# hamptus/mlx-swift-qwen3-tts

Hardware: NVIDIA B200
Metric: audio-sec generated per sec (RTFx) (higher is better)
Workload: dtype u4 g64 weights dequantised at load to f16 operands x f32 accumulate, f32 residual stream

## Files before the change

### mlx-swift-qwen3-tts_b200/csrc/engine.h

```cpp
#pragma once
#include <map>
#include <memory>
#include <mutex>
#include <string>
#include <vector>

#include "frame_kernel.h"
#include "kernels.h"

namespace q3 {

class CodecDecoder;
class AudioEncoder;
class SpeakerEncoderDev;

struct EngineOptions {
  int device = 0;
  cudaStream_t stream = nullptr;
  int max_batch = 1, kv_capacity = 512, max_frames = 2400, use_cuda_graph = 1;
  int load_codec = 1, load_talker = 1, codec_max_frames = 2400, codec_max_batch = 8;
  int lanes = 1;
  int max_trailing = 1024;
  int packed_gemm = 0;
  int runtime_quantization = 0;
};

struct Admission {
  bool too_short = false;
  int prefill_len = 0;
};

struct TalkerShared {
  DeviceArena arena;
  TalkerWeights w;
  int weight_dtype = Q3TTS_BF16, eff_bits = 0, eff_group = 64;
  std::mutex mu;
};

class TalkerEngine {
 public:
  TalkerEngine(const std::string& model_dir, const TalkerConfig& cfg, const EngineOptions& opt, cudaStream_t stream,
               LaunchCounter* counter, std::shared_ptr<TalkerShared> shared = nullptr);
  ~TalkerEngine();

  Admission admit(int slot, const q3tts_request& req);
  struct AdmitItem { int slot; const q3tts_request* req; };
  void admit_batch(const std::vector<AdmitItem>& items, std::vector<Admission>& out);
  int max_prefill_rows() const { return max_rows_; }
  int step_slots(int hi) const {
    if (!handle_tc_) return hi;
    int b = hi <= 32 ? 32 : (hi <= 64 ? 64 : (hi + 127) / 128 * 128);
    return b < opt_.max_batch ? b : opt_.max_batch;
  }
  void run_frames(int n_slots, int n);
  void fetch_states(int n_slots, std::vector<SlotState>& out);
  void fetch_frames(int slot, int first, int count, int32_t* dst);
  void fetch_logits(int frames, float* code0_out, float* cp_out);
  int dump_slot() const { return dump_enabled_ ? dump_slot_ : -1; }
  void release(int slot);
  void drop_graphs();

  const TalkerConfig& config() const { return cfg_; }
  const TalkerWeights& weights() const { return w_; }
  int max_batch() const { return opt_.max_batch; }
  int kv_capacity() const { return opt_.kv_capacity; }
  int max_frames() const { return opt_.max_frames; }
  int weight_dtype() const { return shared_->weight_dtype; }
  int quant_bits() const { return shared_->eff_bits; }
  int checkpoint_quant_bits() const { return w_.checkpoint_bits; }
  int quant_group() const { return shared_->eff_group; }
  size_t device_bytes() const { return arena_.total() + (owns_weights_ ? shared_->arena.total() : 0); }
  const std::shared_ptr<TalkerShared>& shared() const { return shared_; }
  size_t weight_bytes_per_frame() const { return w_.talker_step_bytes + 15 * w_.cp_pass_bytes; }
  int64_t graph_replays = 0, graph_nodes_replayed = 0, mega_launches = 0;
  bool megakernel_enabled() const { return mega_.ok; }
  double last_prefill_ms = 0;

  double profile_linears(int which, int m, int iters, int64_t& launches, int64_t& bytes_per_iter);
  int sample_probe(const float* logits, int vocab, float temperature, int top_k, float top_p, float rep_penalty,
                   const int32_t* token_set, int n_set, uint64_t seed, uint64_t counter);

 private:
  void forward_stack(const StackWeights& S, float* x, int m, const int* row_slot, const int* row_pos, const int* win_start,
                     const float* inv_freq, void* kbase, void* vbase, int kv_f16, size_t slot_stride, size_t layer_stride, int capacity,
                     bool one_row_per_slot, bool decode_step, bool x16_ready);
  void issue_frame(int n_slots);
  void build_tc_weights();
  void build_mega_plan();
  TcLinear make_tc(const Linear& L, bool interleave_halves, const float* fold = nullptr);
  bool use_tc(int) const { return handle_tc_; }
  bool use_tc_step(int) const { return handle_tc_; }
  bool use_mega(int n_slots) const { return mega_.ok && !handle_tc_ && opt_.max_batch <= mega_.max_slots && n_slots <= mega_.max_slots; }
  void linear_tc(const TcLinear& L, const void* x16, int m, float* out32, int ld32, void* out16, int ld16, const float* res, int act, int swiglu, bool row_count_invariant = false);
  LaunchCtx ctx() { return LaunchCtx{stream_, counter_}; }

  TalkerConfig cfg_;
  EngineOptions opt_;
  cudaStream_t stream_;
  LaunchCounter* counter_;
  DeviceArena arena_;
  std::shared_ptr<TalkerShared> shared_;
  bool owns_weights_ = false;
  TalkerWeights& w_;

  int max_rows_ = 0, max_tp_rows_ = 0, set_words_ = 0;
  int tc_min_rows_ = 3;
  bool step_tc_ = false;
  bool handle_tc_ = false;
  bool packed_gemm_ = false;
  void attach_packed(struct TcGemm& g, const TcLinear& L) const;
  float* d_rs_ = nullptr;
  static constexpr float kX16Div = 16.0f;
  void *d_h16_ = nullptr, *d_attn16_ = nullptr, *d_act16_ = nullptr, *d_tpe16_ = nullptr, *d_tph16_ = nullptr;
  void *kcache_ = nullptr, *vcache_ = nullptr;
  int kv_f16_ = 0;
  float *cp_k_ = nullptr, *cp_v_ = nullptr;
  size_t kv_slot_stride_ = 0, kv_layer_stride_ = 0, cpkv_slot_stride_ = 0, cpkv_layer_stride_ = 0;
  static constexpr int kCpCapacity = 32;
  SlotState* d_state_ = nullptr;
  int *d_step_slot_ = nullptr, *d_step_pos_ = nullptr, *d_win_ = nullptr;
  int *d_cp_slot2_ = nullptr, *d_cp_pos2_ = nullptr, *d_iota_ = nullptr, *d_cp_pos_ = nullptr;
  int *d_pf_slot_ = nullptr, *d_pf_pos_ = nullptr, *d_pf_win_ = nullptr;
  float *d_x_ = nullptr, *d_qkv_ = nullptr, *d_attn_ = nullptr, *d_act_ = nullptr;
  float *d_hlast_ = nullptr, *d_logits0_ = nullptr, *d_cplogits_ = nullptr, *d_cpin_ = nullptr, *d_cpx_ = nullptr, *d_xstep_ = nullptr;
  int *d_cur_codes_ = nullptr, *d_frames_ = nullptr, *d_forced_ = nullptr;
  unsigned* d_sets_ = nullptr;
  float *d_trailing_ = nullptr, *d_tts_ = nullptr;
  float *d_tpe_ = nullptr, *d_tph_ = nullptr, *d_tp_ = nullptr, *d_spk_ = nullptr;
  int *d_ids_ = nullptr, *d_desc_ = nullptr;
  Embedding* d_cp_emb_ = nullptr;
  float *d_inv_freq_ = nullptr, *d_cp_inv_freq_ = nullptr;
  float *d_dump0_ = nullptr, *d_dumpcp_ = nullptr;
  int dump_cap_ = 0, dump_slot_ = 0;
  bool dump_enabled_ = false;
  float* d_probe_logits_ = nullptr;
  unsigned* d_probe_set_ = nullptr;
  int* d_probe_out_ = nullptr;
  int* h_stage_ = nullptr;
  size_t h_stage_ints_ = 0;
  SlotState* h_state_ = nullptr;
  cudaEvent_t ev_a_ = nullptr, ev_b_ = nullptr;

  struct Graph {
    cudaGraphExec_t exec = nullptr;
    int64_t nodes = 0;
  };
  std::map<long long, Graph> graphs_;
  MegaPlan mega_;
};

struct Handle {
  std::mutex mu;
  std::string model_dir;
  std::string last_error;
  bool poisoned = false;
  EngineOptions opt;
  cudaStream_t stream = nullptr;
  bool own_stream = false;
  LaunchCounter counter;
  TalkerConfig cfg;
  bool has_talker = false;
  std::unique_ptr<TalkerEngine> talker;
  std::unique_ptr<CodecDecoder> codec;
  std::unique_ptr<AudioEncoder> audio_encoder;
  std::unique_ptr<SpeakerEncoderDev> speaker_encoder;
  q3tts_timing timing{};
  cudaEvent_t ev_start = nullptr, ev_stop = nullptr;
  float* h_pcm = nullptr;
  size_t h_pcm_floats = 0;
  int32_t* h_codes = nullptr;
  size_t h_codes_ints = 0;
  int32_t* d_codes = nullptr;
  size_t d_codes_ints = 0;
  float* d_pcm = nullptr;
  size_t d_pcm_floats = 0;
  void* open_stream = nullptr;
  std::mutex lanes_mu;
  std::vector<Handle*> lanes;
  ~Handle();
};

}
```

### mlx-swift-qwen3-tts_b200/csrc/gemm_skinny.cu

```cuda
#include <cuda.h>

#include <algorithm>

#include "skinny_common.cuh"

namespace q3 {

namespace {

using namespace skinny;

template <int ACT, bool SWIGLU>
__global__ void __launch_bounds__(kThreads, 1)
tc_skinny_kernel(const __grid_constant__ CUtensorMap tmW, const __grid_constant__ CUtensorMap tmX, const SkParams p) {
  extern __shared__ uint8_t smem_raw[];
  uint8_t* smem = reinterpret_cast<uint8_t*>((reinterpret_cast<uintptr_t>(smem_raw) + 1023) & ~(uintptr_t)1023);
  const int x_bytes = p.m_pad * kBlockK * 2;
  uint8_t* sW = smem;
  uint8_t* sX = smem + (size_t)p.stages * kWBytes;
  float* red = reinterpret_cast<float*>(sX + (size_t)p.stages * x_bytes);
  uint64_t* full = reinterpret_cast<uint64_t*>(red + (size_t)kRowsW * p.m_pad);
  uint64_t* empty = full + p.stages;
  uint64_t* tmem_full = empty + p.stages;
  uint64_t* red_full = tmem_full + 1;
  uint64_t* ack = red_full + 1;
  uint32_t* tmem_slot = reinterpret_cast<uint32_t*>(ack + 1);
  float* rowscale_s = reinterpret_cast<float*>(tmem_slot + 2);

  const int warp = threadIdx.x >> 5, lane = threadIdx.x & 31;
  const uint32_t rank = p.split > 1 ? cluster_ctarank() : 0u;
  const int n0 = blockIdx.x * kRowsW;
  const int kb0 = (int)((rank * (uint32_t)p.num_kb) >> p.split_shift);
  const int kb1 = (int)(((rank + 1u) * (uint32_t)p.num_kb) >> p.split_shift);
  const int nkb = kb1 - kb0;

  pdl_launch_dependents();
  if (threadIdx.x == 32) {
    asm volatile("prefetch.tensormap [%0];" ::"l"(&tmW) : "memory");
    asm volatile("prefetch.tensormap [%0];" ::"l"(&tmX) : "memory");
  }
  if (threadIdx.x == 0) {
    if (p.trace) p.trace[((size_t)blockIdx.y * gridDim.x + blockIdx.x) * 16 + 0] = sk_globaltimer();
    SK_STAMP(1);
    for (int s = 0; s < p.stages; ++s) { mbar_init(&full[s], 1); mbar_init(&empty[s], 1); }
    mbar_init(tmem_full, 1);
    mbar_init(red_full, 1);
    mbar_init(ack, p.split > 1 ? p.split - 1 : 1);
    asm volatile("fence.mbarrier_init.release.cluster;" ::: "memory");
    asm volatile("fence.proxy.async.shared::cta;" ::: "memory");
  }
  if (warp == 1) {
    asm volatile("tcgen05.alloc.cta_group::1.sync.aligned.shared::cta.b32 [%0], %1;" ::"r"(smem_u32(tmem_slot)), "r"(p.tmem_cols) : "memory");
    asm volatile("tcgen05.relinquish_alloc_permit.cta_group::1.sync.aligned;" ::: "memory");
  }
  tc_fence_before();
  __syncthreads();
  tc_fence_after();
  const uint32_t tmem_base = *tmem_slot;
  if (threadIdx.x == 0) SK_STAMP(2);
  if (p.split > 1) cluster_arrive_release();

  if (warp == 0) {
    {
      const bool lead = elect_one();
      const int pre = nkb < p.stages ? nkb : p.stages;
      if (lead) {
        for (int i = 0; i < pre; ++i) {
          mbar_expect_tx(&full[i], (uint32_t)(kWBytes + x_bytes));
          tma_load_2d(sW + (size_t)i * kWBytes, &tmW, &full[i], (kb0 + i) * kBlockK, n0);
        }
        for (int i = pre; i < nkb; ++i) tma_prefetch_2d(&tmW, (kb0 + i) * kBlockK, n0);
      }
      pdl_wait();
      int s = 0;
      uint32_t ph = 0;
      for (int i = 0; i < nkb; ++i) {
        if (i >= pre) mbar_wait(&empty[s], ph ^ 1u);
        if (lead) {
          if (i >= pre) {
            mbar_expect_tx(&full[s], (uint32_t)(kWBytes + x_bytes));
            tma_load_2d(sW + (size_t)s * kWBytes, &tmW, &full[s], (kb0 + i) * kBlockK, n0);
          }
          tma_load_2d(sX + (size_t)s * x_bytes, &tmX, &full[s], (kb0 + i) * kBlockK, 0);
        }
        if (++s == p.stages) { s = 0; ph ^= 1u; }
      }
    }
    __syncwarp();
  } else if (warp == 1) {
    {
      const bool lead = elect_one();
      const uint32_t idesc = (1u << 4) | ((uint32_t)(p.m_pad >> 3) << 17) | ((uint32_t)(kRowsW >> 4) << 24);
      int s = 0;
      uint32_t ph = 0;
      for (int i = 0; i < nkb; ++i) {
        mbar_wait(&full[s], ph);
        tc_fence_after();
        if (lead && i == 0) SK_STAMP(3);
        const uint64_t ad = umma_desc(smem_u32(sW + (size_t)s * kWBytes));
        const uint64_t bd = umma_desc(smem_u32(sX + (size_t)s * x_bytes));
        if (lead) {
#pragma unroll
          for (int k = 0; k < kBlockK / 16; ++k)
            umma_f16(tmem_base, ad + (uint64_t)(2 * k), bd + (uint64_t)(2 * k), idesc, (i | k) != 0 ? 1u : 0u);
          umma_commit(&empty[s]);
        }
        if (++s == p.stages) { s = 0; ph ^= 1u; }
      }
      if (lead) umma_commit(tmem_full);
    }
    __syncwarp();
  } else {
    pdl_wait();
    if (p.rms_x) sk_row_factors(p, rowscale_s, rank);
    if (p.split > 1) cluster_wait_acquire();
    mbar_wait(tmem_full, 0);
    tc_fence_after();
    if (threadIdx.x == 64) SK_STAMP(4);
    sk_reduce_epilogue<ACT, SWIGLU>(p, reinterpret_cast<float*>(smem), red, red_full, ack, rowscale_s, tmem_base, rank, n0);
  }
  if (p.split > 1 && warp < 2) cluster_wait_acquire();
  tc_fence_before();
  __syncthreads();
  if (threadIdx.x == 0 && p.trace) {
    SK_STAMP(8);
    p.trace[((size_t)blockIdx.y * gridDim.x + blockIdx.x) * 16 + 9] = sk_globaltimer();
  }
  if (warp == 1) {
    tc_fence_after();
    asm volatile("tcgen05.dealloc.cta_group::1.sync.aligned.b32 %0, %1;" ::"r"(tmem_base), "r"(p.tmem_cols) : "memory");
  }
}

constexpr int kSmemKB = 108;

struct SkPlan {
  int m_pad, split, stages, num_kb, tiles;
  size_t smem;
};

SkPlan plan(const TcGemm& g) {
  SkPlan s{};
  const int M = g.Bt * g.T;
  s.m_pad = M <= 32 ? 32 : (M <= 64 ? 64 : 128);
  s.tiles = (g.N + kRowsW - 1) / kRowsW;
  s.num_kb = (g.cin + kBlockK - 1) / kBlockK;
  s.split = k_split(s.tiles, s.num_kb, s.m_pad);
  const int stage_bytes = kWBytes + s.m_pad * kBlockK * 2;
  const int red_bytes = kRowsW * s.m_pad * 4;
  const int nkb_max = (s.num_kb + s.split - 1) / s.split;
  s.stages = std::max(2, (kSmemKB * 1024 - red_bytes) / stage_bytes);
  s.stages = std::max(1, std::min(s.stages, nkb_max));
  while (s.stages * stage_bytes < red_bytes) ++s.stages;
  s.smem = (size_t)s.stages * stage_bytes + red_bytes + 1024 + (2 * s.stages + 4) * 8 + 16 + 128 * 4;
  return s;
}

}

bool tc_skinny_supported(const TcGemm& g) {
  const long long M = (long long)g.Bt * g.T;
  return g.allow_skinny && !g.res16 && !g.outr16 && g.ntap == 1 && M >= 1 && M <= 128 && !g.snake_ea && !g.pcm && !(g.swiglu && g.act != TC_ACT_NONE) && tc_gemm_supported(g);
}

using SkKernel = void (*)(const CUtensorMap, const CUtensorMap, const SkParams);
static SkKernel pick_kernel(int act, int swiglu) {
  if (swiglu) return tc_skinny_kernel<TC_ACT_NONE, true>;
  if (act == TC_ACT_GELU) return tc_skinny_kernel<TC_ACT_GELU, false>;
  if (act == TC_ACT_SILU) return tc_skinny_kernel<TC_ACT_SILU, false>;
  return tc_skinny_kernel<TC_ACT_NONE, false>;
}

void init_tc_skinny() {
  tc_resolve_encode();
  for (SkKernel k : {pick_kernel(0, 1), pick_kernel(TC_ACT_GELU, 0), pick_kernel(TC_ACT_SILU, 0), pick_kernel(0, 0)})
    Q3_CUDA(cudaFuncSetAttribute(k, cudaFuncAttributeMaxDynamicSharedMemorySize, 220 * 1024));
  for (SkKernel k : {pick_kernel(0, 1), pick_kernel(TC_ACT_GELU, 0), pick_kernel(TC_ACT_SILU, 0), pick_kernel(0, 0)})
    Q3_CUDA(cudaFuncSetAttribute(k, cudaFuncAttributeNonPortableClusterSizeAllowed, 1));
  init_tc_skinny_q();
}

unsigned long long* g_sk_trace = nullptr;

void tc_skinny_set_trace(unsigned long long* dev_buf) { g_sk_trace = dev_buf; }
unsigned long long* tc_skinny_trace_buf() { return g_sk_trace; }
void tc_skinny_grid(const TcGemm& g, int* tiles, int* split, int* stages) {
  const SkPlan s = plan(g);
  *tiles = s.tiles; *split = s.split; *stages = s.stages;
}

void launch_tc_skinny(const LaunchCtx& c, const TcGemm& g) {
  if (tc_skinny_q_supported(g)) return launch_tc_skinny_q(c, g);
  Q3_CHECK(tc_skinny_supported(g), Q3TTS_ERR_INVALID_ARG, "tc_skinny: unsupported shape (rows %d, cin %d, N %d)", g.Bt * g.T, g.cin, g.N);
  tc_resolve_encode();
  const SkPlan s = plan(g);
  SkParams p{};
  p.M = g.Bt * g.T; p.N = g.N; p.K = g.cin;
  p.m_pad = s.m_pad; p.split = s.split; p.mc = s.m_pad / s.split; p.stages = s.stages; p.num_kb = s.num_kb;
  p.mc_shift = 0;
  while ((1 << p.mc_shift) < p.mc) ++p.mc_shift;
  p.split_shift = 0;
  while ((1 << p.split_shift) < p.split) ++p.split_shift;
  p.tmem_cols = std::max(32, s.m_pad);
  p.bias = g.bias; p.res = g.res; p.ld_res = g.ld_res; p.scale = g.scale; p.act = g.act; p.swiglu = g.swiglu;
  p.out32 = g.out32; p.ld32 = g.ld32; p.out16 = g.out16; p.ld16 = g.ld16;
  p.out16_scale = g.out16_scale;
  p.rms_x = g.rms_in ? g.a : nullptr;
  p.rms_a = 1.0f / (g.in_scale * g.in_scale * (float)g.cin); p.rms_eps = g.rms_eps; p.rms_mult = 1.0f / g.in_scale;
  Q3_CHECK(!g.row_scale, Q3TTS_ERR_INVALID_ARG, "tc_skinny: pass rms_in instead of precomputed row factors");
  p.trace = g_sk_trace;

  const uint64_t wdims[2] = {(uint64_t)g.cin, (uint64_t)g.N};
  const uint64_t wstr[1] = {(uint64_t)g.cin * 2};
  const uint32_t wbox[2] = {(uint32_t)kBlockK, (uint32_t)kRowsW};
  const CUtensorMap mw = tc_make_map(g.w, 2, wdims, wstr, wbox);
  const uint64_t xdims[2] = {(uint64_t)g.cin, (uint64_t)p.M};
  const uint64_t xstr[1] = {(uint64_t)g.cin * 2};
  const uint32_t xbox[2] = {(uint32_t)kBlockK, (uint32_t)s.m_pad};
  const CUtensorMap mx = tc_make_map(g.a, 2, xdims, xstr, xbox);

  Q3_CHECK(s.smem <= 220 * 1024, Q3TTS_ERR_CAPACITY, "tc_skinny: shared memory request %zu too large", s.smem);
  cudaLaunchConfig_t cfg{};
  cfg.gridDim = dim3((unsigned)s.tiles, (unsigned)s.split);
  cfg.blockDim = dim3(kThreads);
  cfg.dynamicSmemBytes = s.smem;
  cfg.stream = c.stream;
  cudaLaunchAttribute attr[2];
  int na = 0;
  if (s.split > 1) {
    attr[na].id = cudaLaunchAttributeClusterDimension;
    attr[na].val.clusterDim.x = 1; attr[na].val.clusterDim.y = (unsigned)s.split; attr[na].val.clusterDim.z = 1;
    ++na;
  }
  if (pdl_enabled()) {
    attr[na].id = cudaLaunchAttributeProgrammaticStreamSerialization;
    attr[na].val.programmaticStreamSerializationAllowed = 1;
    ++na;
  }
  cfg.attrs = attr;
  cfg.numAttrs = na;
  Q3_CUDA(cudaLaunchKernelEx(&cfg, pick_kernel(g.act, g.swiglu), mw, mx, p));
  c.tick();
}

}
```

### mlx-swift-qwen3-tts_b200/csrc/skinny_common.cuh

```cuda
#pragma once
#include <cuda.h>

#include "gemm_tc.h"
#include "tc_ptx.cuh"

namespace q3 {
namespace skinny {

using namespace tcptx;

constexpr int kRowsW = 128;
constexpr int kBlockK = 64;
constexpr int kWBytes = kRowsW * kBlockK * 2;
constexpr int kThreads = 192;
constexpr int kMaxSplit = 8;
constexpr int kCtaTarget = 200;

inline int k_split(int tiles, int num_kb, int m_pad) {
  int split = 1;
  while (split * 2 <= kMaxSplit && tiles * split * 2 <= kCtaTarget && split * 2 <= num_kb && m_pad / (split * 2) >= 4) split *= 2;
  return split;
}

struct SkParams {
  int M, N, K;
  int m_pad, mc, mc_shift, split, stages, num_kb, tmem_cols;
  const float* bias;
  const float* res;
  int ld_res;
  const float* scale;
  int act, swiglu;
  float* out32;
  int ld32;
  __half* out16;
  int ld16;
  float out16_scale;
  const __half* rms_x;
  float rms_a, rms_eps, rms_mult;
  unsigned long long* trace;
  const void* q_scales;
  const void* q_biases;
  const float* q_fold;
  int q_group, q_sdt;
  int q_pstages;
  int q_xstages, q_xown;
  int q_half_rows;
  int split_shift;
};

__device__ __forceinline__ unsigned long long sk_globaltimer() {
  unsigned long long t;
  asm volatile("mov.u64 %0, %%globaltimer;" : "=l"(t));
  return t;
}
#define SK_STAMP(slot)                                                                                        \
  do {                                                                                                        \
    if (p.trace) p.trace[((size_t)blockIdx.y * gridDim.x + blockIdx.x) * 16 + (slot)] = (unsigned long long)clock64(); \
  } while (0)

__device__ __forceinline__ float sk_gelu_erf(float v) { return 0.5f * v * (1.0f + erff(v * 0.70710678118654752440f)); }
__device__ __forceinline__ float sk_silu(float v) { return v / (1.0f + expf(-v)); }
__device__ __forceinline__ float sk_silu_fast(float v) { return __fdividef(v, 1.0f + __expf(-v)); }

__device__ __forceinline__ float4 lds_f4(uint32_t saddr) {
  float4 v;
  asm volatile("ld.shared.v4.f32 {%0, %1, %2, %3}, [%4];" : "=f"(v.x), "=f"(v.y), "=f"(v.z), "=f"(v.w) : "r"(saddr));
  return v;
}

template <int NC>
__device__ __forceinline__ void sk_load_res(const SkParams& p, float (&r)[NC], int valid, int m0, int ob) {
  if (p.res) {
    const float* rp = p.res + (size_t)m0 * p.ld_res + ob;
#pragma unroll
    for (int e = 0; e < NC; ++e, rp += p.ld_res) r[e] = e < valid ? *rp : 0.f;
  }
}
template <int NC, int ACT, bool SWIGLU>
__device__ __forceinline__ void sk_finish(const SkParams& p, float (&acc)[NC], const float (&r)[NC], int valid, int m0, int ob, float bias,
                                          float scale, const float* rowscale) {
#pragma unroll
  for (int e = 0; e < NC; ++e) {
    float v = acc[e];
    if (rowscale) v *= rowscale[e];
    v += bias;
    if (ACT == TC_ACT_GELU) v = sk_gelu_erf(v);
    else if (ACT == TC_ACT_SILU) v = sk_silu(v);
    if (SWIGLU) {
      const float up = __shfl_xor_sync(0xffffffffu, v, 1);
      v = sk_silu_fast(v) * up;
    }
    if (p.res) v = r[e] + scale * v;
    acc[e] = v;
  }
  if (p.out32) {
    float* op = p.out32 + (size_t)m0 * p.ld32 + ob;
#pragma unroll
    for (int e = 0; e < NC; ++e, op += p.ld32)
      if (e < valid) *op = acc[e];
  }
  if (p.out16) {
    __half* hp = p.out16 + (size_t)m0 * p.ld16 + ob;
#pragma unroll
    for (int e = 0; e < NC; ++e, hp += p.ld16)
      if (e < valid) *hp = __float2half_rn(acc[e] * p.out16_scale);
  }
}

template <int ACT, bool SWIGLU>
__device__ __forceinline__ void sk_reduce_epilogue(const SkParams& p, float* stage_out, float* red, uint64_t* red_full, uint64_t* ack, const float* rowscale_s,
                                                   uint32_t tmem_base, uint32_t rank, int n0) {
  const int warp = threadIdx.x >> 5, lane = threadIdx.x & 31;
  const int q = warp & 3;
  const int row = q * 32 + lane;
  const int n = n0 + row;
  const bool n_ok = n < p.N;
  const uint32_t taddr = tmem_base + ((uint32_t)(q * 32) << 16);
  const float bias = (p.bias && n_ok) ? p.bias[n] : 0.f;
  const int so = SWIGLU ? (n >> 1) : n;
  const float scale = (p.scale && n_ok) ? p.scale[so] : 1.f;
  for (int c0 = 0; c0 < p.m_pad; c0 += 32) {
    uint32_t raw[32];
    tmem_ld32(taddr + (uint32_t)c0, raw);
#pragma unroll
    for (int j = 0; j < 32; j += 4) {
      const int col = c0 + j;
      const int dst = col >> p.mc_shift;
      const int off = col & (p.mc - 1);
      *reinterpret_cast<float4*>(stage_out + (size_t)dst * kRowsW * p.mc + ((size_t)(off >> 2) * kRowsW + row) * 4) =
          make_float4(__uint_as_float(raw[j]), __uint_as_float(raw[j + 1]), __uint_as_float(raw[j + 2]), __uint_as_float(raw[j + 3]));
    }
  }
  asm volatile("fence.proxy.async.shared::cta;" ::: "memory");
  asm volatile("bar.sync 1, 128;" ::: "memory");
  const uint32_t slice_bytes = (uint32_t)(kRowsW * p.mc * 4);
  if (threadIdx.x == 64 && p.split > 1) {
    mbar_expect_tx(red_full, slice_bytes * (uint32_t)(p.split - 1));
    for (int i = 1; i < p.split; ++i) {
      const uint32_t d = (rank + (uint32_t)i) & (uint32_t)(p.split - 1);
      bulk_copy_to_rank(map_to_rank(smem_u32(red + (size_t)rank * kRowsW * p.mc), d), smem_u32(stage_out + (size_t)d * kRowsW * p.mc), slice_bytes,
                        map_to_rank(smem_u32(red_full), d));
    }
  }
  if (threadIdx.x == 64) SK_STAMP(5);
  const int m_base = (int)rank * p.mc;
  const bool lane_out = n_ok && (!SWIGLU || (n & 1) == 0);
  float r16[16];
  {
    int valid0 = p.M - m_base;
    valid0 = valid0 < 16 ? valid0 : 16;
    valid0 = valid0 < p.mc ? valid0 : p.mc;
    sk_load_res<16>(p, r16, lane_out ? valid0 : 0, m_base, so);
  }
  if (p.split > 1) mbar_wait(red_full, 0);
  if (threadIdx.x == 96) SK_STAMP(10);
  if (threadIdx.x == 64) {
    SK_STAMP(6);
    for (int i = 1; i < p.split; ++i) mbar_arrive_remote_relaxed(map_to_rank(smem_u32(ack), (rank + (uint32_t)i) & (uint32_t)(p.split - 1)));
  }
  const uint32_t own_s = smem_u32(stage_out), red_s = smem_u32(red);
  for (int cb = 0; cb < p.mc; cb += 16) {
    const int nc = p.mc - cb < 16 ? p.mc - cb : 16;
    float a16[16];
#pragma unroll
    for (int j = 0; j < 16; ++j) a16[j] = 0.f;
    for (int s = 0; s < p.split; ++s) {
      const uint32_t base = (s == (int)rank ? own_s : red_s) + (uint32_t)s * slice_bytes + (uint32_t)row * 16u;
#pragma unroll
      for (int c = 0; c < 16; c += 4) {
        if (c < nc) {
          const float4 v = lds_f4(base + (uint32_t)((cb + c) >> 2) * (uint32_t)(kRowsW * 16));
          a16[c] += v.x; a16[c + 1] += v.y; a16[c + 2] += v.z; a16[c + 3] += v.w;
        }
      }
    }
    if (threadIdx.x == 96 && cb == 0) SK_STAMP(11);
    int valid = p.M - (m_base + cb);
    valid = valid < nc ? valid : nc;
    if (!lane_out) valid = 0;
    if (cb > 0) sk_load_res<16>(p, r16, valid, m_base + cb, so);
    sk_finish<16, ACT, SWIGLU>(p, a16, r16, valid, m_base + cb, so, bias, scale, p.rms_x ? rowscale_s + cb : nullptr);
    if (threadIdx.x == 96 && cb == 0) SK_STAMP(12);
  }
  if (threadIdx.x == 96) SK_STAMP(13);
  if (threadIdx.x == 64 && p.split > 1) {
    SK_STAMP(7);
    mbar_wait(ack, 0);
  }
}

__device__ __forceinline__ void sk_row_factors(const SkParams& p, float* rowscale_s, uint32_t rank) {
  const int warp = threadIdx.x >> 5, lane = threadIdx.x & 31;
  const int q = warp & 3;
  const int m_lo = (int)rank * p.mc, j = lane & 7;
  for (int r0 = 0; r0 < p.mc; r0 += 16) {
    const int r = r0 + q * 4 + (lane >> 3), m = m_lo + r;
    float ss = (r < p.mc && m < p.M) ? tc_row_sumsq_f16(p.rms_x + (size_t)m * p.K, p.K, j) : 0.f;
    ss = tc_group8_sum(ss);
    if (j == 0 && r < p.mc) rowscale_s[r] = p.rms_mult * rsqrtf(ss * p.rms_a + p.rms_eps);
  }
}

}
}
```

### mlx-swift-qwen3-tts_b200/csrc/talker_engine.cu

```cuda
#include <algorithm>
#include <cmath>

#include "engine.h"
#include "frame_kernel.h"
#include "gemm_tc.h"

namespace q3 {

void init_talker_kernels();
int mega_max_blocks_per_sm(int fmt, int slots, size_t smem);

TalkerEngine::TalkerEngine(const std::string& model_dir, const TalkerConfig& cfg, const EngineOptions& opt, cudaStream_t stream,
                           LaunchCounter* counter, std::shared_ptr<TalkerShared> shared)
    : cfg_(cfg), opt_(opt), stream_(stream), counter_(counter), shared_(shared ? shared : std::make_shared<TalkerShared>()),
      owns_weights_(!shared), w_(shared_->w) {
  init_talker_kernels();
  if (owns_weights_)
    load_talker_weights(model_dir, cfg_, shared_->arena, stream_, w_, shared_->weight_dtype, shared_->eff_bits, shared_->eff_group,
                        opt_.runtime_quantization != 0);
  const int B = opt_.max_batch, C = opt_.kv_capacity, F = opt_.max_frames;
  const int H = cfg_.hidden_size, Hcp = cfg_.cp.hidden_size;
  Q3_CHECK(B >= 1 && C >= 208 && F >= 1, Q3TTS_ERR_INVALID_ARG, "bad options: max_batch %d kv_capacity %d max_frames %d", B, C, F);
  const StackWeights &T = w_.talker, &P = w_.cp;
  max_rows_ = std::max(std::max(2 * B, C), std::min(B * 96, 8192));
  max_tp_rows_ = std::max(C + opt_.max_trailing + 8, std::min(B * 128, 16384));
  set_words_ = (std::max(cfg_.vocab_size, cfg_.cp.vocab_size) + 31) / 32;

  kv_layer_stride_ = (size_t)T.kv_heads * C * 128;
  kv_slot_stride_ = kv_layer_stride_ * T.layers;
  if (const char* e = getenv("Q3TTS_TC_MIN_ROWS")) tc_min_rows_ = atoi(e);
  {
    const char* e16 = getenv("Q3TTS_KV_F16");
    kv_f16_ = (tc_min_rows_ > 0 && B >= tc_min_rows_ && !(e16 && atoi(e16) == 0)) ? 1 : 0;
  }
  const size_t kv_elem = kv_f16_ ? 2 : 4;
  kcache_ = arena_.alloc(kv_slot_stride_ * B * kv_elem);
  vcache_ = arena_.alloc(kv_slot_stride_ * B * kv_elem);
  cpkv_layer_stride_ = (size_t)P.kv_heads * kCpCapacity * 128;
  cpkv_slot_stride_ = cpkv_layer_stride_ * P.layers;
  cp_k_ = arena_.alloc_n<float>(cpkv_slot_stride_ * B);
  cp_v_ = arena_.alloc_n<float>(cpkv_slot_stride_ * B);

  d_state_ = arena_.alloc_n<SlotState>(B);
  Q3_CUDA(cudaMemsetAsync(d_state_, 0, sizeof(SlotState) * B, stream_));
  d_step_slot_ = arena_.alloc_n<int>(B); d_step_pos_ = arena_.alloc_n<int>(B); d_win_ = arena_.alloc_n<int>(B);
  d_cp_slot2_ = arena_.alloc_n<int>(2 * B); d_cp_pos2_ = arena_.alloc_n<int>(2 * B);
  d_iota_ = arena_.alloc_n<int>(B); d_cp_pos_ = arena_.alloc_n<int>(16 * B);
  d_pf_slot_ = arena_.alloc_n<int>(max_rows_); d_pf_pos_ = arena_.alloc_n<int>(max_rows_); d_pf_win_ = arena_.alloc_n<int>(B);
  Q3_CUDA(cudaMemsetAsync(d_pf_win_, 0, sizeof(int) * B, stream_));
  Q3_CUDA(cudaMemsetAsync(d_win_, 0, sizeof(int) * B, stream_));

  const int wide_h = std::max(H, Hcp);
  const int qkv_w = std::max((T.heads + 2 * T.kv_heads) * 128, (P.heads + 2 * P.kv_heads) * 128);
  const int attn_w = std::max(T.heads, P.heads) * 128;
  const int act_w = std::max(T.inter, P.inter);
  d_x_ = arena_.alloc_n<float>((size_t)max_rows_ * wide_h);
  d_qkv_ = arena_.alloc_n<float>((size_t)max_rows_ * qkv_w);
  d_attn_ = arena_.alloc_n<float>((size_t)max_rows_ * attn_w);
  d_act_ = arena_.alloc_n<float>((size_t)max_rows_ * act_w);
  d_hlast_ = arena_.alloc_n<float>((size_t)B * H);
  d_logits0_ = arena_.alloc_n<float>((size_t)B * cfg_.vocab_size);
  d_cplogits_ = arena_.alloc_n<float>((size_t)B * cfg_.cp.vocab_size);
  d_cpin_ = arena_.alloc_n<float>((size_t)2 * B * H);
  d_cpx_ = arena_.alloc_n<float>((size_t)2 * B * Hcp);
  d_xstep_ = arena_.alloc_n<float>((size_t)B * H);
  d_cur_codes_ = arena_.alloc_n<int>((size_t)B * 16);
  Q3_CUDA(cudaMemsetAsync(d_cur_codes_, 0, sizeof(int) * B * 16, stream_));
  d_frames_ = arena_.alloc_n<int>((size_t)B * F * 16);
  d_forced_ = arena_.alloc_n<int>((size_t)B * F * 16);
  d_sets_ = arena_.alloc_n<unsigned>((size_t)B * 16 * set_words_);
  d_trailing_ = arena_.alloc_n<float>((size_t)B * opt_.max_trailing * H);
  d_tts_ = arena_.alloc_n<float>((size_t)3 * H);
  d_tpe_ = arena_.alloc_n<float>((size_t)max_tp_rows_ * cfg_.text_hidden_size);
  d_tph_ = arena_.alloc_n<float>((size_t)max_tp_rows_ * cfg_.text_hidden_size);
  d_tp_ = arena_.alloc_n<float>((size_t)max_tp_rows_ * H);
  d_spk_ = arena_.alloc_n<float>((size_t)B * H);
  d_ids_ = arena_.alloc_n<int>(max_tp_rows_);
  d_desc_ = arena_.alloc_n<int>((size_t)3 * max_rows_);
  if (tc_min_rows_ > 0 && B >= tc_min_rows_) {
    init_tc_gemm();
    {
      std::lock_guard<std::mutex> lk(shared_->mu);
      if (!w_.has_tc) build_tc_weights();
    }
    d_h16_ = arena_.alloc((size_t)max_rows_ * std::max(wide_h, cfg_.text_hidden_size) * 2);
    d_attn16_ = arena_.alloc((size_t)max_rows_ * attn_w * 2);
    d_act16_ = arena_.alloc((size_t)max_rows_ * act_w * 2);
    d_rs_ = arena_.alloc_n<float>((size_t)max_rows_);
    d_tpe16_ = arena_.alloc((size_t)max_tp_rows_ * cfg_.text_hidden_size * 2);
    d_tph16_ = arena_.alloc((size_t)max_tp_rows_ * cfg_.text_hidden_size * 2);
  }
  handle_tc_ = w_.has_tc && tc_min_rows_ > 0 && B >= tc_min_rows_;
  {
    const char* e = getenv("Q3TTS_SKINNY_Q");
    packed_gemm_ = opt_.packed_gemm == 1 || (opt_.packed_gemm == 0 && e && atoi(e) != 0);
  }
  Q3_CHECK(!kv_f16_ || handle_tc_ || !w_.has_tc, Q3TTS_ERR_BAD_CONFIG, "internal: fp16 KV rings on a handle without the tensor-core step");
  d_probe_logits_ = arena_.alloc_n<float>(4096);
  d_probe_set_ = arena_.alloc_n<unsigned>(128);
  d_probe_out_ = arena_.alloc_n<int>(1);

  std::vector<int> slot2(2 * B), pos2(2 * B), iota(B), cpos(16 * B);
  for (int s = 0; s < B; ++s) {
    slot2[2 * s] = slot2[2 * s + 1] = s;
    pos2[2 * s] = 0; pos2[2 * s + 1] = 1;
    iota[s] = s;
    for (int g = 0; g < 16; ++g) cpos[g * B + s] = g + 1;
  }
  Q3_CUDA(cudaMemcpy(d_cp_slot2_, slot2.data(), slot2.size() * 4, cudaMemcpyHostToDevice));
  Q3_CUDA(cudaMemcpy(d_cp_pos2_, pos2.data(), pos2.size() * 4, cudaMemcpyHostToDevice));
  Q3_CUDA(cudaMemcpy(d_iota_, iota.data(), iota.size() * 4, cudaMemcpyHostToDevice));
  Q3_CUDA(cudaMemcpy(d_cp_pos_, cpos.data(), cpos.size() * 4, cudaMemcpyHostToDevice));

  std::vector<float> f(64), fc(64);
  for (int i = 0; i < 64; ++i) {
    f[i] = 1.0f / powf(cfg_.rope_theta, (float)(2 * i) / 128.0f);
    fc[i] = 1.0f / powf(cfg_.cp.rope_theta, (float)(2 * i) / 128.0f);
  }
  d_inv_freq_ = arena_.alloc_n<float>(64); d_cp_inv_freq_ = arena_.alloc_n<float>(64);
  Q3_CUDA(cudaMemcpy(d_inv_freq_, f.data(), 256, cudaMemcpyHostToDevice));
  Q3_CUDA(cudaMemcpy(d_cp_inv_freq_, fc.data(), 256, cudaMemcpyHostToDevice));

  d_cp_emb_ = arena_.alloc_n<Embedding>(15);
  Q3_CUDA(cudaMemcpy(d_cp_emb_, w_.cp_codec_embedding.data(), sizeof(Embedding) * 15, cudaMemcpyHostToDevice));

  h_stage_ints_ = (size_t)max_tp_rows_ + 3 * (size_t)C + 64;
  Q3_CUDA(cudaMallocHost(&h_stage_, h_stage_ints_ * sizeof(int)));
  Q3_CUDA(cudaMallocHost(&h_state_, sizeof(SlotState) * B));
  Q3_CUDA(cudaEventCreate(&ev_a_));
  Q3_CUDA(cudaEventCreate(&ev_b_));

  h_stage_[0] = cfg_.tts_bos_token_id; h_stage_[1] = cfg_.tts_eos_token_id; h_stage_[2] = cfg_.tts_pad_token_id;
  for (int i = 0; i < 3; ++i)
    Q3_CHECK(h_stage_[i] >= 0 && h_stage_[i] < cfg_.text_vocab_size, Q3TTS_ERR_BAD_CONFIG, "tts special token id %d outside text vocab", h_stage_[i]);
  Q3_CUDA(cudaMemcpyAsync(d_ids_, h_stage_, 12, cudaMemcpyHostToDevice, stream_));
  LaunchCtx c{stream_, nullptr};
  launch_gather_rows(c, w_.text_embedding, d_ids_, 3, d_tpe_, cfg_.text_hidden_size, false);
  launch_linear(c, w_.fc1, d_tpe_, cfg_.text_hidden_size, 3, d_tph_, cfg_.text_hidden_size, nullptr, 0.f, EPI_SILU);
  launch_linear(c, w_.fc2, d_tph_, cfg_.text_hidden_size, 3, d_tts_, H, nullptr, 0.f, EPI_STORE);
  Q3_CUDA(cudaStreamSynchronize(stream_));
  build_mega_plan();
}

void TalkerEngine::build_mega_plan() {
  mega_ = MegaPlan{};
  if (const char* e = getenv("Q3TTS_MEGAKERNEL"))
    if (atoi(e) == 0) return;
  if (!opt_.use_cuda_graph) return;
  const StackWeights &T = w_.talker, &P = w_.cp;
  std::vector<const Linear*> order;
  std::vector<int> swiglu;
  struct Norms { const float *norm_w, *q_norm, *k_norm; };
  struct PhaseInfo { int in_kind, pass, epi, out_sel, flags, layer, unit, tkind; };
  std::vector<Norms> norms;
  std::vector<PhaseInfo> phase;
  enum { IN_GX = 0, IN_GX_LAST, IN_CP0, IN_CPG, IN_TALKER, IN_ATTN, IN_ACT };
  enum { E_STORE = 0, E_ADD_RAW = 1, E_SWIGLU = 2 };
  auto push = [&](const Linear& L, bool sw, PhaseInfo ph, const float* nw = nullptr, const float* qn = nullptr, const float* kn = nullptr) {
    order.push_back(&L); swiglu.push_back(sw ? 1 : 0); norms.push_back({nw, qn, kn}); phase.push_back(ph);
  };
  for (int u = 0; u < 16; ++u) {
    const bool talker = (u == 15);
    const StackWeights& S = talker ? T : P;
    const int base = (talker ? MF_TALKER : 0) | (u == 0 ? MF_ROWS2 : 0);
    const int first_kind = talker ? IN_TALKER : (u == 0 ? IN_CP0 : IN_CPG);
    bool first = true;
    auto flags_of = [&](int extra) { const int f = base | extra | (first ? MF_UNIT_START : 0); first = false; return f; };
    const bool mtp = !talker && w_.has_mtp;
    if (mtp) push(w_.small_to_mtp, false, {first_kind, u, E_STORE, 0, flags_of(0), 0, u, 0});
    for (int l = 0; l < S.layers; ++l) {
      const LayerWeights& lw = S.layer[l];
      const int qkv_in = (l == 0 && !mtp) ? first_kind : IN_GX;
      push(lw.qkv, false, {qkv_in, u, E_STORE, 1, flags_of(MF_ATTN | MF_KEEP_RAW | ((talker && l == 0) ? MF_FINALIZE : 0)), l, u, 1}, lw.in_norm, lw.q_norm, lw.k_norm);
      push(lw.o, false, {IN_ATTN, u, E_ADD_RAW, 0, flags_of(0), l, u, 2});
      push(lw.gate_up, true, {IN_GX, u, E_SWIGLU, 2, flags_of(MF_KEEP_RAW), l, u, 3}, lw.post_norm);
      push(lw.down, false, {IN_ACT, u, E_ADD_RAW, 0, flags_of(0), l, u, 4});
    }
    if (talker) push(w_.codec_head, false, {IN_GX, u, E_STORE, 3, flags_of(MF_HEAD | MF_KEEP_RAW), 0, u, 5}, T.final_norm);
    else push(w_.lm_head[u], false, {IN_GX_LAST, u == 0 ? 2 : 1, E_STORE, 3, flags_of(MF_HEAD), 0, u, 5}, P.final_norm);
  }
  const Linear& L0 = *order[0];
  int fmt = -1;
  if (L0.bits == 4) fmt = 0; else if (L0.bits == 8) fmt = 1;
  else if (L0.bits == 0) fmt = L0.sdt == Q3TTS_BF16 ? 2 : (L0.sdt == Q3TTS_F16 ? 3 : 4);
  if (fmt < 0) return;
  const int vpl = fmt == 0 ? 32 : (fmt == 1 ? 16 : (fmt == 4 ? 4 : 8));
  const int kc = 32 * vpl;
  std::vector<MegaLinear> lin;
  int kmax = 0, need_slot = 0;
  for (size_t i = 0; i < order.size(); ++i) {
    const Linear& L = *order[i];
    if (L.bits != L0.bits || (L.bits == 0 && L.sdt != L0.sdt)) return;
    if (L.bits && (L.group % vpl != 0 || L.in % L.group != 0)) return;
    if (L.in % vpl != 0 || L.in % 4 != 0) return;
    MegaLinear m{};
    m.w = L.bits ? (const void*)L.qw : L.w; m.scales = L.scales; m.biases = L.biases; m.bias = L.bias;
    m.nsub = swiglu[i] ? 2 : 1;
    m.out_eff = L.out / m.nsub;
    m.in = L.in;
    m.row_bytes = L.bits ? L.in * L.bits / 8 : L.in * (int)dtype_size(L.sdt);
    m.srow_bytes = L.bits ? (L.in / L.group) * (int)dtype_size(L.sdt) : 0;
    m.sdt = L.sdt; m.group = L.bits ? L.group : 1;
    if (m.group & (m.group - 1)) return;
    m.group_shift = 0;
    while ((1 << m.group_shift) < m.group) ++m.group_shift;
    int u = 1;
    while (u <= 16 && ((u * m.row_bytes) % 16 != 0 || (u * m.srow_bytes) % 16 != 0)) u <<= 1;
    if (u > 16 || m.out_eff % u != 0) return;
    m.unit = u;
    m.norm_w = norms[i].norm_w; m.q_norm = norms[i].q_norm; m.k_norm = norms[i].k_norm;
    m.in_kind = phase[i].in_kind; m.pass = phase[i].pass; m.epi = phase[i].epi; m.out_sel = phase[i].out_sel; m.flags = phase[i].flags;
    m.layer = phase[i].layer; m.uidx = phase[i].unit; m.tkind = phase[i].tkind;
    need_slot = std::max(need_slot, u * m.nsub * (m.row_bytes + 2 * m.srow_bytes));
    kmax = std::max(kmax, L.in);
    lin.push_back(m);
  }
  const int G_tk = T.heads / T.kv_heads, G_cp = P.heads / P.kv_heads;
  auto g_ok = [](int g) { return g == 1 || g == 2 || g == 4; };
  if (!g_ok(G_tk) || !g_ok(G_cp) || T.head_dim != 128 || P.head_dim != 128) return;
  if (T.heads % T.kv_heads || P.heads % P.kv_heads) return;
  if (cfg_.vocab_size > 4096 || cfg_.cp.vocab_size > 4096) return;
  if (T.hidden % 4 || P.hidden % 4 || T.inter % 4 || P.inter % 4) return;
  int slot_bytes = 32 * 1024;
  while (slot_bytes < need_slot) slot_bytes += 8 * 1024;
  const int nchunk = (kmax + kc - 1) / kc;
  const int hmax = std::max(T.hidden, P.hidden);
  auto up = [](int v, int a) { return (v + a - 1) / a * a; };
  const bool mma = (fmt == 0 || fmt == 1);
  int gmin = 1 << 30, gmax = 0, max_tiles = 0;
  for (const MegaLinear& m : lin) {
    gmin = std::min(gmin, m.group); gmax = std::max(gmax, m.group);
    const int rch = (slot_bytes / (m.nsub * (m.row_bytes + 2 * m.srow_bytes))) / m.unit * m.unit;
    max_tiles = std::max(max_tiles, ((rch + 15) / 16) * m.nsub);
  }
  if (mma && (gmin < 32 || gmax > 128 || kmax % 32 != 0)) return;
  const int budget = 226 * 1024;
  int NS = 0, MT = 0, n_ring = 0, xs_bytes = 0, xsum_bytes = 0, xraw_bytes = 0, red_bytes = 0, hl_bytes = 0, rope_bytes = 0, part_bytes = 0;
  const int scratch = (4096 + 64 + 4096) * 4;
  for (int cand : {kMegaMaxSlots, 1}) {
    if (cand > 1 && (!mma || opt_.max_batch < 2)) continue;
    NS = cand; MT = 2 * NS;
    const bool tc = mma && cand > 1;
    xs_bytes = up(std::max(tc ? 8 * (kmax * 2 + 64) : MT * nchunk * kc * 4, scratch), 128);
    xsum_bytes = up(tc ? MT * (kmax / gmin) * 4 : MT * nchunk * 32 * 4, 128);
    xraw_bytes = up(MT * hmax * 4, 128);
    red_bytes = up(MT * 16 * 4, 128);
    hl_bytes = up(NS * hmax * 4, 128);
    rope_bytes = up(NS * 128 * 2 * 4, 128);
    part_bytes = tc ? up(std::max(32, max_tiles) * 128 * 4, 128) : 0;
    const int fixed = xs_bytes + xsum_bytes + xraw_bytes + red_bytes + 256 + 512 + hl_bytes + rope_bytes + part_bytes + 128;
    n_ring = std::min(8, (budget - fixed) / slot_bytes);
    if (n_ring >= 3 || (cand == 1 && n_ring >= 2)) break;
    NS = 0;
  }
  if (NS == 0) return;
  mega_.max_slots = NS;
  MegaParams& p = mega_.p;
  p.slot_bytes = slot_bytes; p.n_ring = n_ring;
  p.off_xs = n_ring * slot_bytes;
  p.off_xsum = p.off_xs + xs_bytes;
  p.off_xraw = p.off_xsum + xsum_bytes;
  p.off_red = p.off_xraw + xraw_bytes;
  p.off_bar = p.off_red + red_bytes;
  p.off_dsc = p.off_bar + 256;
  static_assert(2 * sizeof(MegaLinear) <= 512, "descriptor slots");
  p.off_hl = p.off_dsc + 512;
  p.raw_ld = hmax;
  p.off_rope = p.off_hl + hl_bytes;
  p.off_part = p.off_rope + rope_bytes;
  p.xh_stride = kmax + 32;
  mega_.smem = (size_t)p.off_part + part_bytes + 128;
  mega_.fmt = fmt; mega_.G_cp = G_cp; mega_.G_tk = G_tk;
  int dev = 0, sms = 0, coop = 0;
  Q3_CUDA(cudaGetDevice(&dev));
  Q3_CUDA(cudaDeviceGetAttribute(&sms, cudaDevAttrMultiProcessorCount, dev));
  Q3_CUDA(cudaDeviceGetAttribute(&coop, cudaDevAttrCooperativeLaunch, dev));
  if (!coop || sms < 1) return;
  init_mega_kernels();
  if (mega_max_blocks_per_sm(fmt, mega_.max_slots, mega_.smem) < 1) return;
  int min_units = 1 << 30;
  for (const MegaLinear& m : lin) min_units = std::min(min_units, m.out_eff / m.unit);
  mega_.grid = std::min(sms, min_units);
  if (mega_.grid < 1 || opt_.kv_capacity > 4 * 128) return;
  for (MegaLinear& m : lin) {
    const int U = m.out_eff / m.unit;
    m.ubase = U / mega_.grid; m.urem = U % mega_.grid;
    m.rch = (slot_bytes / (m.nsub * (m.row_bytes + 2 * m.srow_bytes))) / m.unit * m.unit;
  }
  MegaLinear* d_lin = arena_.alloc_n<MegaLinear>(lin.size());
  Q3_CUDA(cudaMemcpy(d_lin, lin.data(), sizeof(MegaLinear) * lin.size(), cudaMemcpyHostToDevice));
  auto stack_of = [&](const StackWeights& S, const float* inv_freq, float* k, float* v, size_t slot_stride, size_t layer_stride, int cap, int nsplit) {
    MegaStack s{};
    s.hidden = S.hidden; s.layers = S.layers; s.heads = S.heads; s.kv_heads = S.kv_heads; s.inter = S.inter; s.eps = S.eps;
    s.final_norm = S.final_norm; s.inv_freq = inv_freq; s.k = k; s.v = v;
    s.slot_stride = slot_stride; s.layer_stride = layer_stride; s.capacity = cap; s.nsplit = nsplit;
    return s;
  };
  const int nsplit_tk = 4;
  p.lin = d_lin; p.n_lin = (int)lin.size();
  p.cp = stack_of(P, d_cp_inv_freq_, cp_k_, cp_v_, cpkv_slot_stride_, cpkv_layer_stride_, kCpCapacity, 1);
  if (kv_f16_) return;
  p.tk = stack_of(T, d_inv_freq_, (float*)kcache_, (float*)vcache_, kv_slot_stride_, kv_layer_stride_, opt_.kv_capacity, nsplit_tk);
  p.has_mtp = w_.has_mtp ? 1 : 0; p.H = cfg_.hidden_size; p.Hcp = cfg_.cp.hidden_size; p.V = cfg_.vocab_size; p.Vc = cfg_.cp.vocab_size;
  p.codec = w_.codec_embedding; p.cp_emb = d_cp_emb_;
  p.st = d_state_; p.cur_codes = d_cur_codes_; p.frames = d_frames_; p.forced = d_forced_; p.max_frames = opt_.max_frames;
  p.sets = d_sets_; p.set_words = set_words_;
  p.trailing = d_trailing_; p.max_trailing = opt_.max_trailing; p.tts_pad = d_tts_ + (size_t)2 * cfg_.hidden_size;
  p.hlast = d_hlast_; p.logits0 = d_logits0_; p.cplogits = d_cplogits_;
  p.part_stride = up(std::max(T.heads, P.heads) * 130, 4);
  p.ld_x = up(hmax, 4);
  p.ld_qkv = up(std::max((T.heads + 2 * T.kv_heads) * 128, (P.heads + 2 * P.kv_heads) * 128), 4);
  p.ld_act = up(std::max(T.inter, P.inter), 4);
  p.ld_logit = up(std::max(cfg_.vocab_size, cfg_.cp.vocab_size), 4);
  const size_t n_x = (size_t)MT * p.ld_x, n_qkv = (size_t)MT * p.ld_qkv, n_part = (size_t)MT * nsplit_tk * p.part_stride;
  const size_t n_act = (size_t)MT * p.ld_act, n_logit = (size_t)NS * p.ld_logit, n_msg = (size_t)2 * 16 * kMegaMaxSlots * 4;
  p.ex_bytes = (n_x + n_qkv + n_part + n_act + n_logit + n_msg) * sizeof(unsigned long long);
  unsigned long long* ex = arena_.alloc_n<unsigned long long>(n_x + n_qkv + n_part + n_act + n_logit + n_msg);
  p.ex_base = ex;
  p.ex_x = ex; ex += n_x;
  p.ex_qkv = ex; ex += n_qkv;
  p.ex_part = ex; ex += n_part;
  p.ex_act = ex; ex += n_act;
  p.ex_logit = ex; ex += n_logit;
  p.ex_msg = ex;
  p.window = 192;
  p.eos_id = cfg_.codec_eos_token_id; p.pad_id = cfg_.codec_pad_id;
  if (getenv("Q3TTS_MEGA_TRACE")) {
    p.trace_stride = 8 * 1024 * 8;
    p.trace = arena_.alloc_n<long long>((size_t)2 * p.trace_stride);
  }
  mega_.ok = true;
}

TalkerEngine::~TalkerEngine() {
  drop_graphs();
  if (h_stage_) cudaFreeHost(h_stage_);
  if (h_state_) cudaFreeHost(h_state_);
  if (ev_a_) cudaEventDestroy(ev_a_);
  if (ev_b_) cudaEventDestroy(ev_b_);
  if (d_dump0_) cudaFree(d_dump0_);
  if (d_dumpcp_) cudaFree(d_dumpcp_);
}

void TalkerEngine::drop_graphs() {
  for (auto& g : graphs_)
    if (g.second.exec) cudaGraphExecDestroy(g.second.exec);
  graphs_.clear();
}

TcLinear TalkerEngine::make_tc(const Linear& L, bool interleave_halves, const float* fold) {
  const LaunchCtx c{stream_, nullptr};
  TcLinear t;
  t.out = L.out; t.in = L.in; t.bias = L.bias;
  if (L.bits) { t.qw = L.qw; t.qscales = L.scales; t.qbiases = L.biases; t.qbits = L.bits; t.qgroup = L.group; t.qsdt = L.sdt; t.fold = fold; t.halves = interleave_halves; }
  __half* dst = (__half*)shared_->arena.alloc((size_t)L.out * L.in * 2);
  if (L.bits && fold) {
    float* tmp = nullptr;
    Q3_CUDA(cudaMalloc(&tmp, (size_t)L.out * L.in * 4));
    launch_dequantize(c, L.qw, L.scales, L.biases, L.sdt, L.out, L.in, L.group, L.bits, Q3TTS_F32, tmp);
    launch_weight_to_f16(c, tmp, Q3TTS_F32, L.out, L.in, interleave_halves, dst, fold);
    Q3_CUDA(cudaStreamSynchronize(stream_));
    cudaFree(tmp);
  } else if (L.bits) {
    if (!interleave_halves) {
      launch_dequantize(c, L.qw, L.scales, L.biases, L.sdt, L.out, L.in, L.group, L.bits, Q3TTS_F16, dst);
    } else {
      __half* tmp = nullptr;
      Q3_CUDA(cudaMalloc(&tmp, (size_t)L.out * L.in * 2));
      launch_dequantize(c, L.qw, L.scales, L.biases, L.sdt, L.out, L.in, L.group, L.bits, Q3TTS_F16, tmp);
      launch_weight_to_f16(c, tmp, Q3TTS_F16, L.out, L.in, true, dst);
      Q3_CUDA(cudaStreamSynchronize(stream_));
      cudaFree(tmp);
    }
  } else {
    launch_weight_to_f16(c, L.w, L.sdt, L.out, L.in, interleave_halves, dst, fold);
  }
  t.w = dst;
  return t;
}

void TalkerEngine::build_tc_weights() {
  auto ok = [](const Linear& L) { return L.in % 8 == 0 && L.out % 32 == 0; };
  bool all = ok(w_.fc1) && ok(w_.fc2) && ok(w_.codec_head) && (!w_.has_mtp || ok(w_.small_to_mtp));
  for (StackWeights* S : {&w_.talker, &w_.cp})
    for (auto& l : S->layer) all = all && ok(l.qkv) && ok(l.o) && ok(l.gate_up) && ok(l.down) && (l.gate_up.out / 2) % 16 == 0;
  for (auto& h : w_.lm_head) all = all && ok(h);
  if (!all) return;
  for (StackWeights* S : {&w_.talker, &w_.cp}) {
    S->tc.resize(S->layers);
    for (int l = 0; l < S->layers; ++l) {
      S->tc[l].qkv = make_tc(S->layer[l].qkv, false, S->layer[l].in_norm);
      S->tc[l].o = make_tc(S->layer[l].o, false);
      S->tc[l].gate_up_il = make_tc(S->layer[l].gate_up, true, S->layer[l].post_norm);
      S->tc[l].down = make_tc(S->layer[l].down, false);
    }
  }
  w_.fc1_tc = make_tc(w_.fc1, false);
  w_.fc2_tc = make_tc(w_.fc2, false);
  w_.codec_head_tc = make_tc(w_.codec_head, false);
  for (auto& h : w_.lm_head) w_.lm_head_tc.push_back(make_tc(h, false, w_.cp.final_norm));
  if (w_.has_mtp) w_.small_to_mtp_tc = make_tc(w_.small_to_mtp, false);
  Q3_CUDA(cudaStreamSynchronize(stream_));
  w_.has_tc = true;
}

void TalkerEngine::attach_packed(TcGemm& g, const TcLinear& L) const {
  if (!L.qbits || !packed_gemm_) return;
  g.q_w = L.qw; g.q_scales = L.qscales; g.q_biases = L.qbiases; g.q_fold = L.fold;
  g.q_bits = L.qbits; g.q_group = L.qgroup; g.q_sdt = L.qsdt; g.q_halves = L.halves ? 1 : 0;
}

void TalkerEngine::linear_tc(const TcLinear& L, const void* x16, int m, float* out32, int ld32, void* out16, int ld16, const float* res,
                             int act, int swiglu, bool row_count_invariant) {
  TcGemm g;
  if (row_count_invariant) { g.allow_skinny = 0; g.k_rotate = 0; }
  g.a = (const __half*)x16; g.w = (const __half*)L.w; g.Bt = 1; g.T = m; g.cin = L.in; g.N = L.out; g.ntap = 1; g.dil = 1;
  g.bias = L.bias; g.res = res; g.ld_res = ld32; g.act = act; g.swiglu = swiglu;
  g.out32 = out32; g.ld32 = ld32; g.out16 = (__half*)out16; g.ld16 = ld16;
  if (!row_count_invariant) attach_packed(g, L);
  launch_tc_gemm(ctx(), g);
}

void TalkerEngine::forward_stack(const StackWeights& S, float* x, int m, const int* row_slot, const int* row_pos,
                                 const int* win_start, const float* inv_freq, void* kbase, void* vbase, int kv_f16, size_t slot_stride,
                                 size_t layer_stride, int capacity, bool one_row_per_slot, bool decode_step, bool x16_ready) {
  const size_t kv_elem = kv_f16 ? 2 : 4;
  const LaunchCtx c = ctx();
  const int qkv_ld = (S.heads + 2 * S.kv_heads) * 128, attn_ld = S.heads * 128;
  if ((decode_step ? step_tc_ : use_tc(m)) && !S.tc.empty()) {
    const bool fused = decode_step && m <= 128;
    const bool pass0_pairs = decode_step && !one_row_per_slot && win_start == nullptr && row_pos == d_cp_pos2_ && (m % 2) == 0;
    const float inv16 = 1.0f / kX16Div;
    auto consumer = [&](const TcLinear& L, float* out32, int ld32, void* out16, int ld16, int swiglu) {
      TcGemm g;
      g.a = (const __half*)d_h16_; g.w = (const __half*)L.w; g.Bt = 1; g.T = m; g.cin = L.in; g.N = L.out;
      g.bias = L.bias; g.swiglu = swiglu; g.out32 = out32; g.ld32 = ld32; g.out16 = (__half*)out16; g.ld16 = ld16;
      g.rms_eps = S.eps; g.in_scale = inv16; g.allow_skinny = fused; g.k_rotate = fused;
      if (fused) {
        g.rms_in = 1;
        attach_packed(g, L);
      } else {
        launch_row_scale(c, (const __half*)d_h16_, m, S.hidden, inv16, S.eps, d_rs_);
        g.row_scale = d_rs_;
      }
      launch_tc_gemm(c, g);
    };
    auto producer = [&](const TcLinear& L, const void* a16) {
      TcGemm g;
      g.a = (const __half*)a16; g.w = (const __half*)L.w; g.Bt = 1; g.T = m; g.cin = L.in; g.N = L.out;
      g.bias = L.bias; g.res = x; g.ld_res = S.hidden; g.out32 = x; g.ld32 = S.hidden; g.allow_skinny = fused; g.k_rotate = fused;
      if (fused) {
        g.out16 = (__half*)d_h16_; g.ld16 = S.hidden; g.out16_scale = inv16;
        attach_packed(g, L);
        launch_tc_gemm(c, g);
      } else {
        launch_tc_gemm(c, g);
        launch_scale_to_f16(c, x, (size_t)m * S.hidden, inv16, (__half*)d_h16_);
      }
    };
    if (!x16_ready) launch_scale_to_f16(c, x, (size_t)m * S.hidden, inv16, (__half*)d_h16_);
    for (int l = 0; l < S.layers; ++l) {
      const LayerWeights& L = S.layer[l];
      const LayerTc& Tc = S.tc[l];
      KVLayout kv;
      kv.k = static_cast<char*>(kbase) + l * layer_stride * kv_elem; kv.v = static_cast<char*>(vbase) + l * layer_stride * kv_elem;
      kv.slot_stride = slot_stride; kv.capacity = capacity; kv.f16 = kv_f16;
      consumer(Tc.qkv, d_qkv_, qkv_ld, nullptr, 0, 0);
      if (one_row_per_slot) {
        launch_rope_attention_f16(c, d_qkv_, qkv_ld, m, S.heads, S.kv_heads, L.q_norm, L.k_norm, S.eps, inv_freq, row_slot, row_pos, win_start, kv,
                                  (__half*)d_attn16_, attn_ld);
      } else if (pass0_pairs) {
        launch_cp_pass0_attention_f16(c, d_qkv_, qkv_ld, m / 2, S.heads, S.kv_heads, L.q_norm, L.k_norm, S.eps, inv_freq, kv, (__half*)d_attn16_, attn_ld);
      } else {
        launch_qk_norm_rope_append(c, d_qkv_, qkv_ld, m, S.heads, S.kv_heads, S.head_dim, L.q_norm, L.k_norm, S.eps, inv_freq, row_slot,
                                   row_pos, kv);
        launch_attention_f16(c, d_qkv_, qkv_ld, m, S.heads, S.kv_heads, S.head_dim, row_slot, row_pos, win_start, kv, (__half*)d_attn16_, attn_ld);
      }
      producer(Tc.o, d_attn16_);
      consumer(Tc.gate_up_il, nullptr, 0, d_act16_, S.inter, 1);
      producer(Tc.down, d_act16_);
    }
    return;
  }
  for (int l = 0; l < S.layers; ++l) {
    const LayerWeights& L = S.layer[l];
    KVLayout kv;
    kv.k = static_cast<char*>(kbase) + l * layer_stride * kv_elem; kv.v = static_cast<char*>(vbase) + l * layer_stride * kv_elem;
    kv.slot_stride = slot_stride; kv.capacity = capacity; kv.f16 = kv_f16;
    launch_linear(c, L.qkv, x, S.hidden, m, d_qkv_, qkv_ld, L.in_norm, S.eps, EPI_STORE);
    if (one_row_per_slot) {
      launch_rope_attention(c, d_qkv_, qkv_ld, m, S.heads, S.kv_heads, L.q_norm, L.k_norm, S.eps, inv_freq, row_slot, row_pos, win_start, kv,
                            d_attn_, attn_ld);
    } else {
      launch_qk_norm_rope_append(c, d_qkv_, qkv_ld, m, S.heads, S.kv_heads, S.head_dim, L.q_norm, L.k_norm, S.eps, inv_freq, row_slot,
                                 row_pos, kv);
      launch_attention(c, d_qkv_, qkv_ld, m, S.heads, S.kv_heads, S.head_dim, row_slot, row_pos, win_start, kv, d_attn_, attn_ld);
    }
    launch_linear(c, L.o, d_attn_, attn_ld, m, x, S.hidden, nullptr, 0.f, EPI_ADD);
    launch_linear(c, L.gate_up, x, S.hidden, m, d_act_, S.inter, L.post_norm, S.eps, EPI_SWIGLU);
    launch_linear(c, L.down, d_act_, S.inter, m, x, S.hidden, nullptr, 0.f, EPI_ADD);
  }
}

Admission TalkerEngine::admit(int slot, const q3tts_request& r) {
  std::vector<AdmitItem> items{{slot, &r}};
  std::vector<Admission> out;
  admit_batch(items, out);
  return out[0];
}

void TalkerEngine::admit_batch(const std::vector<AdmitItem>& items, std::vector<Admission>& out) {
  const int H = cfg_.hidden_size, C = opt_.kv_capacity, F = opt_.max_frames, TH = cfg_.text_hidden_size;
  out.assign(items.size(), Admission{});
  std::vector<int> ids{cfg_.tts_bos_token_id, cfg_.tts_eos_token_id, cfg_.tts_pad_token_id};
  const int TP_BOS = 0, TP_EOS = 1, TP_PAD = 2;
  std::vector<int> desc, meta_slot, meta_pos;
  std::vector<float> spk_host;
  struct Plan { int slot, row0, P, tp_trailing, n_trailing; const q3tts_request* r; };
  std::vector<Plan> plans;
  auto check_text = [&](const int32_t* p, int n, const char* what) {
    for (int i = 0; i < n; ++i)
      Q3_CHECK(p[i] >= 0 && p[i] < cfg_.text_vocab_size, Q3TTS_ERR_INVALID_ARG, "%s id %d outside the text vocabulary", what, p[i]);
  };
  for (size_t it = 0; it < items.size(); ++it) {
    const int slot = items[it].slot;
    const q3tts_request& r = *items[it].req;
    Q3_CHECK(slot >= 0 && slot < opt_.max_batch, Q3TTS_ERR_INVALID_ARG, "slot %d out of range", slot);
    Q3_CHECK(r.text_ids != nullptr || r.n_text_ids == 0, Q3TTS_ERR_INVALID_ARG, "text_ids is NULL");
    if (r.n_text_ids < 9) {
      out[it].too_short = true;
      continue;
    }
    check_text(r.text_ids, r.n_text_ids, "text");
    const bool has_instruct = r.instruct_ids != nullptr && r.n_instruct_ids > 0;
    const bool use_icl = !has_instruct && r.ref_codes != nullptr && r.ref_text_ids != nullptr && r.n_ref_text_ids > 0;
    if (has_instruct) check_text(r.instruct_ids, r.n_instruct_ids, "instruct");
    if (use_icl) check_text(r.ref_text_ids, r.n_ref_text_ids, "reference transcript");
    const bool spk_by_id = r.speaker_id >= 0;
    const bool spk_by_vec = !spk_by_id && r.speaker_embedding != nullptr;
    if (spk_by_id) Q3_CHECK(r.speaker_id < cfg_.vocab_size, Q3TTS_ERR_INVALID_ARG, "speaker_id %d outside codec vocabulary", r.speaker_id);
    if (spk_by_vec) Q3_CHECK(r.speaker_embedding_dim == H, Q3TTS_ERR_INVALID_ARG, "speaker embedding has %d dims, model hidden size is %d", r.speaker_embedding_dim, H);
    const int n_front_text = has_instruct ? r.n_instruct_ids : (use_icl ? r.n_ref_text_ids : 0);
    const int n_ref_audio = (use_icl && r.ref_frames > 0) ? r.ref_frames : 0;
    const int trailing_len = r.n_text_ids - 4 - 5;
    const int n_trailing = trailing_len > 0 ? trailing_len : 0;
    Q3_CHECK(n_trailing + 1 <= opt_.max_trailing, Q3TTS_ERR_CAPACITY, "text too long: %d trailing tokens > %d", n_trailing + 1, opt_.max_trailing);
    const int n_codec = 5 + ((spk_by_id || spk_by_vec) ? 1 : 0);
    const int P = n_front_text + n_ref_audio + 3 + (n_codec - 1) + 1;
    Q3_CHECK(P <= C - 16, Q3TTS_ERR_CAPACITY, "prefill of %d positions exceeds kv_capacity %d - 16; raise q3tts_options.kv_capacity", P, C);
    Q3_CHECK((int)ids.size() + n_front_text + 4 + n_trailing <= max_tp_rows_ && (int)meta_slot.size() + P <= max_rows_, Q3TTS_ERR_CAPACITY,
             "prompt batch too large for this handle");
    const int tp_front = (int)ids.size();
    for (int i = 0; i < n_front_text; ++i) ids.push_back(has_instruct ? r.instruct_ids[i] : r.ref_text_ids[i]);
    const int tp_role = (int)ids.size();
    for (int i = 0; i < 3; ++i) ids.push_back(r.text_ids[i]);
    const int tp_first = (int)ids.size();
    ids.push_back(r.text_ids[3]);
    const int tp_trailing = (int)ids.size();
    for (int i = 0; i < n_trailing; ++i) ids.push_back(r.text_ids[4 + i]);
    int spk_ref = 0;
    if (spk_by_vec) {
      spk_host.insert(spk_host.end(), r.speaker_embedding, r.speaker_embedding + H);
      spk_ref = (int)(spk_host.size() / H);
    }
    const int row0 = (int)meta_slot.size();
    auto row = [&](int tp, int codec, int spk) {
      desc.push_back(tp); desc.push_back(codec); desc.push_back(spk);
      meta_slot.push_back(slot); meta_pos.push_back((int)meta_slot.size() - 1 - row0);
    };
    for (int i = 0; i < n_front_text; ++i) row(tp_front + i, -1, 0);
    for (int i = 0; i < n_ref_audio; ++i) {
      const int code = r.ref_codes[i];
      Q3_CHECK(code >= 0 && code < cfg_.vocab_size, Q3TTS_ERR_INVALID_ARG, "reference code %d outside codec vocabulary", code);
      row(-1, code, 0);
    }
    for (int i = 0; i < 3; ++i) row(tp_role + i, -1, 0);
    int codec_ids[6], codec_spk[6] = {0, 0, 0, 0, 0, 0};
    int k = 0;
    codec_ids[k++] = cfg_.codec_nothink_id; codec_ids[k++] = cfg_.codec_think_bos_id; codec_ids[k++] = cfg_.codec_think_eos_id;
    if (spk_by_id) codec_ids[k++] = r.speaker_id;
    else if (spk_by_vec) { codec_ids[k] = -1; codec_spk[k] = spk_ref; ++k; }
    codec_ids[k++] = cfg_.codec_pad_id; codec_ids[k++] = cfg_.codec_bos_id;
    for (int i = 0; i < n_codec - 1; ++i) row(i < n_codec - 2 ? TP_PAD : TP_BOS, codec_ids[i], codec_spk[i]);
    row(tp_first, codec_ids[n_codec - 1], 0);
    out[it].prefill_len = P;
    plans.push_back({slot, row0, P, tp_trailing, n_trailing, &r});
  }
  if (plans.empty()) return;
  const int n_tp = (int)ids.size(), R = (int)meta_slot.size();
  Q3_CHECK((int)(spk_host.size() / H) <= opt_.max_batch, Q3TTS_ERR_CAPACITY, "too many speaker embeddings in one admission batch");

  const LaunchCtx c = ctx();
  Q3_CUDA(cudaEventRecord(ev_a_, stream_));
  Q3_CUDA(cudaMemcpyAsync(d_ids_, ids.data(), sizeof(int) * n_tp, cudaMemcpyHostToDevice, stream_));
  Q3_CUDA(cudaMemcpyAsync(d_desc_, desc.data(), sizeof(int) * 3 * R, cudaMemcpyHostToDevice, stream_));
  Q3_CUDA(cudaMemcpyAsync(d_pf_slot_, meta_slot.data(), sizeof(int) * R, cudaMemcpyHostToDevice, stream_));
  Q3_CUDA(cudaMemcpyAsync(d_pf_pos_, meta_pos.data(), sizeof(int) * R, cudaMemcpyHostToDevice, stream_));
  if (!spk_host.empty()) Q3_CUDA(cudaMemcpyAsync(d_spk_, spk_host.data(), sizeof(float) * spk_host.size(), cudaMemcpyHostToDevice, stream_));
  if (use_tc(n_tp)) {
    launch_gather_rows_f16(c, w_.text_embedding, d_ids_, n_tp, (__half*)d_tpe16_, TH);
    linear_tc(w_.fc1_tc, d_tpe16_, n_tp, nullptr, 0, d_tph16_, TH, nullptr, TC_ACT_SILU, 0, true);
    linear_tc(w_.fc2_tc, d_tph16_, n_tp, d_tp_, H, nullptr, 0, nullptr, TC_ACT_NONE, 0, true);
  } else {
    launch_gather_rows(c, w_.text_embedding, d_ids_, n_tp, d_tpe_, TH, false);
    launch_linear(c, w_.fc1, d_tpe_, TH, n_tp, d_tph_, TH, nullptr, 0.f, EPI_SILU);
    launch_linear(c, w_.fc2, d_tph_, TH, n_tp, d_tp_, H, nullptr, 0.f, EPI_STORE);
  }
  launch_assemble_rows(c, d_tp_, H, w_.codec_embedding, d_spk_, d_desc_, R, d_x_);
  for (const Plan& p : plans) {
    float* tr = d_trailing_ + (size_t)p.slot * opt_.max_trailing * H;
    if (p.n_trailing > 0)
      Q3_CUDA(cudaMemcpyAsync(tr, d_tp_ + (size_t)p.tp_trailing * H, sizeof(float) * p.n_trailing * H, cudaMemcpyDeviceToDevice, stream_));
    Q3_CUDA(cudaMemcpyAsync(tr + (size_t)p.n_trailing * H, d_tp_ + (size_t)TP_EOS * H, sizeof(float) * H, cudaMemcpyDeviceToDevice, stream_));
  }
  forward_stack(w_.talker, d_x_, R, d_pf_slot_, d_pf_pos_, d_pf_win_, d_inv_freq_, kcache_, vcache_, kv_f16_, kv_slot_stride_, kv_layer_stride_, C, false, false, false);
  for (const Plan& p : plans) {
    launch_rmsnorm(c, d_x_ + (size_t)(p.row0 + p.P - 1) * H, H, 1, H, w_.talker.final_norm, w_.talker.eps, d_hlast_ + (size_t)p.slot * H, H);
    launch_linear(c, w_.codec_head, d_hlast_ + (size_t)p.slot * H, H, 1, d_logits0_ + (size_t)p.slot * cfg_.vocab_size, cfg_.vocab_size, nullptr, 0.f, EPI_STORE);
  }
  for (const Plan& p : plans) {
    const q3tts_request& r = *p.r;
    const int slot = p.slot;
    const bool forced = r.forced_codes != nullptr && r.n_forced_frames > 0;
    if (forced) {
      Q3_CHECK(r.n_forced_frames <= F, Q3TTS_ERR_CAPACITY, "n_forced_frames %d > max_frames %d", r.n_forced_frames, F);
      Q3_CUDA(cudaMemcpyAsync(d_forced_ + (size_t)slot * F * 16, r.forced_codes, sizeof(int) * 16 * r.n_forced_frames, cudaMemcpyHostToDevice, stream_));
    }
    int logits_cap = 0;
    if ((r.code0_logits_out != nullptr || r.cp_logits_out != nullptr) && r.logits_capacity_frames > 0) {
      Q3_CHECK(slot == 0 || !use_mega(opt_.max_batch), Q3TTS_ERR_INVALID_ARG, "logit dumps on a handle of <= 2 slots are only available for slot 0");
      Q3_CHECK(slot < 4096, Q3TTS_ERR_INVALID_ARG, "logit dumps are limited to slots < 4096");
      logits_cap = std::min(r.logits_capacity_frames, F);
      if (logits_cap > dump_cap_) {
        Q3_CUDA(cudaStreamSynchronize(stream_));
        if (d_dump0_) cudaFree(d_dump0_);
        if (d_dumpcp_) cudaFree(d_dumpcp_);
        Q3_CUDA(cudaMalloc(&d_dump0_, sizeof(float) * (size_t)logits_cap * cfg_.vocab_size));
        Q3_CUDA(cudaMalloc(&d_dumpcp_, sizeof(float) * (size_t)logits_cap * 15 * cfg_.cp.vocab_size));
        dump_cap_ = logits_cap;
        drop_graphs();
      }
      Q3_CUDA(cudaMemsetAsync(d_dump0_, 0, sizeof(float) * (size_t)logits_cap * cfg_.vocab_size, stream_));
      Q3_CUDA(cudaMemsetAsync(d_dumpcp_, 0, sizeof(float) * (size_t)logits_cap * 15 * cfg_.cp.vocab_size, stream_));
    }
    if (logits_cap > 0) { dump_slot_ = slot; dump_enabled_ = true; }
    else if (slot == dump_slot_) dump_enabled_ = false;
    SlotState s{};
    s.active = 1;
    s.pos = p.P;
    s.total_text = p.n_trailing + 1;
    s.max_tokens = forced ? r.n_forced_frames : std::min(std::max(r.max_tokens, 0), F);
    s.n_forced = forced ? r.n_forced_frames : 0;
    s.stream_variant = r.stream_variant ? 1 : 0;
    s.top_k = r.top_k;
    s.logits_cap = logits_cap;
    s.temperature = r.temperature;
    s.top_p = (r.top_p > 0.f) ? r.top_p : 1.0f;
    s.rep_penalty = (r.repetition_penalty > 0.f) ? r.repetition_penalty : 1.0f;
    s.seed = r.seed;
    if (s.max_tokens <= 0) s.finished = 1;
    h_state_[slot] = s;
    Q3_CUDA(cudaMemsetAsync(d_sets_ + (size_t)slot * 16 * set_words_, 0, sizeof(unsigned) * 16 * set_words_, stream_));
  }
  Q3_CUDA(cudaStreamSynchronize(stream_));
  for (const Plan& p : plans)
    Q3_CUDA(cudaMemcpyAsync(d_state_ + p.slot, h_state_ + p.slot, sizeof(SlotState), cudaMemcpyHostToDevice, stream_));
  Q3_CUDA(cudaEventRecord(ev_b_, stream_));
  Q3_CUDA(cudaStreamSynchronize(stream_));
  float ms = 0.f;
  cudaEventElapsedTime(&ms, ev_a_, ev_b_);
  last_prefill_ms += ms;
}

void TalkerEngine::release(int slot) {
  Q3_CUDA(cudaMemsetAsync(d_state_ + slot, 0, sizeof(SlotState), stream_));
}

void TalkerEngine::issue_frame(int n_slots) {
  step_tc_ = use_tc_step(n_slots);
  const LaunchCtx c = ctx();
  const int H = cfg_.hidden_size, Hcp = cfg_.cp.hidden_size, V = cfg_.vocab_size, Vc = cfg_.cp.vocab_size;
  const int B = opt_.max_batch, F = opt_.max_frames;
  SamplerParams p{};
  p.vocab = V; p.group = 0; p.codec_vocab = V; p.eos_id = cfg_.codec_eos_token_id; p.pad_id = cfg_.codec_pad_id;
  p.groups = 16; p.set_words = set_words_;
  float* dump0 = dump_enabled_ ? d_dump0_ : nullptr;
  float* dumpcp = dump_enabled_ ? d_dumpcp_ : nullptr;
  const bool x16_direct = step_tc_ && !w_.has_mtp;
  auto next_input = [&](int mode) {
    NextInput ni;
    ni.mode = mode; ni.H = H; ni.h_last = d_hlast_; ni.codec = w_.codec_embedding; ni.cp_emb = d_cp_emb_; ni.y32 = d_cpin_;
    if (step_tc_) { ni.y16 = (__half*)d_h16_; ni.y16_scale = w_.has_mtp ? 1.0f : 1.0f / kX16Div; }
    return ni;
  };
  launch_sample(c, d_logits0_, V, n_slots, d_state_, p, d_sets_, d_cur_codes_, d_forced_, F, dump0, V, 0, dump_slot_, next_input(1));
  for (int g = 0; g < 15; ++g) {
    const int m = g == 0 ? 2 * n_slots : n_slots;
    float* x = d_cpin_;
    if (w_.has_mtp) {
      if (step_tc_) {
        linear_tc(w_.small_to_mtp_tc, d_h16_, m, d_cpx_, Hcp, nullptr, 0, nullptr, TC_ACT_NONE, 0);
      } else {
        launch_linear(c, w_.small_to_mtp, d_cpin_, H, m, d_cpx_, Hcp, nullptr, 0.f, EPI_STORE);
      }
      x = d_cpx_;
    }
    forward_stack(w_.cp, x, m, g == 0 ? d_cp_slot2_ : d_iota_, g == 0 ? d_cp_pos2_ : d_cp_pos_ + (size_t)g * B, nullptr,
                  d_cp_inv_freq_, cp_k_, cp_v_, 0, cpkv_slot_stride_, cpkv_layer_stride_, kCpCapacity, g != 0, true, x16_direct);
    if (step_tc_ && g != 0 && n_slots <= 128) {
      TcGemm hg;
      hg.a = (const __half*)d_h16_; hg.w = (const __half*)w_.lm_head_tc[g].w; hg.Bt = 1; hg.T = n_slots; hg.cin = Hcp; hg.N = Vc;
      hg.bias = w_.lm_head_tc[g].bias; hg.out32 = d_cplogits_; hg.ld32 = Vc;
      hg.rms_in = 1; hg.rms_eps = w_.cp.eps; hg.in_scale = 1.0f / kX16Div;
      attach_packed(hg, w_.lm_head_tc[g]);
      launch_tc_gemm(c, hg);
    } else if (step_tc_) {
      launch_rmsnorm_f16(c, g == 0 ? x + Hcp : x, g == 0 ? 2 * Hcp : Hcp, n_slots, Hcp, nullptr, w_.cp.eps, (__half*)d_h16_, Hcp);
      linear_tc(w_.lm_head_tc[g], d_h16_, n_slots, d_cplogits_, Vc, nullptr, 0, nullptr, TC_ACT_NONE, 0);
    } else if (g == 0) {
      launch_linear(c, w_.lm_head[0], x + Hcp, 2 * Hcp, n_slots, d_cplogits_, Vc, w_.cp.final_norm, w_.cp.eps, EPI_STORE);
    } else {
      launch_linear(c, w_.lm_head[g], x, Hcp, n_slots, d_cplogits_, Vc, w_.cp.final_norm, w_.cp.eps, EPI_STORE);
    }
    SamplerParams pg = p;
    pg.vocab = Vc; pg.group = g + 1;
    launch_sample(c, d_cplogits_, Vc, n_slots, d_state_, pg, d_sets_, d_cur_codes_, d_forced_, F, dumpcp, 15 * Vc, g * Vc, dump_slot_,
                  g < 14 ? next_input(2) : NextInput());
  }
  launch_frame_finalize(c, n_slots, d_state_, d_cur_codes_, d_frames_, F, d_sets_, set_words_, d_trailing_, opt_.max_trailing,
                        d_tts_ + (size_t)2 * H, w_.codec_embedding, d_cp_emb_, H, d_xstep_, step_tc_ ? (__half*)d_h16_ : nullptr, 1.0f / kX16Div);
  launch_step_rows(c, n_slots, d_state_, d_step_slot_, d_step_pos_, d_win_);
  forward_stack(w_.talker, d_xstep_, n_slots, d_step_slot_, d_step_pos_, d_win_, d_inv_freq_, kcache_, vcache_, kv_f16_, kv_slot_stride_,
                kv_layer_stride_, opt_.kv_capacity, true, true, step_tc_);
  launch_rmsnorm(c, d_xstep_, H, n_slots, H, w_.talker.final_norm, w_.talker.eps, d_hlast_, H);
  if (step_tc_) {
    launch_f32_to_f16(c, d_hlast_, (size_t)n_slots * H, (__half*)d_h16_);
    linear_tc(w_.codec_head_tc, d_h16_, n_slots, d_logits0_, V, nullptr, 0, nullptr, TC_ACT_NONE, 0);
  } else {
    launch_linear(c, w_.codec_head, d_hlast_, H, n_slots, d_logits0_, V, nullptr, 0.f, EPI_STORE);
  }
  launch_step_advance(c, n_slots, d_state_, 192);
}

void TalkerEngine::run_frames(int n_slots, int n) {
  if (n <= 0 || n_slots <= 0) return;
  if (!opt_.use_cuda_graph) {
    for (int i = 0; i < n; ++i) issue_frame(n_slots);
    return;
  }
  if (use_mega(n_slots)) {
    if (mega_.p.trace) Q3_CUDA(cudaMemsetAsync(mega_.p.trace, 0, sizeof(long long) * 2 * mega_.p.trace_stride, stream_));
    launch_frame_megakernel(ctx(), mega_, n_slots, n, dump_enabled_ ? d_dump0_ : nullptr, dump_enabled_ ? d_dumpcp_ : nullptr);
    ++mega_launches;
    if (mega_.p.trace) {
      std::vector<long long> t((size_t)2 * mega_.p.trace_stride);
      Q3_CUDA(cudaMemcpyAsync(t.data(), mega_.p.trace, sizeof(long long) * t.size(), cudaMemcpyDeviceToHost, stream_));
      Q3_CUDA(cudaStreamSynchronize(stream_));
      if (FILE* f = fopen(getenv("Q3TTS_MEGA_TRACE"), "wb")) { fwrite(t.data(), sizeof(long long), t.size(), f); fclose(f); }
    }
    return;
  }
  const long long key = (long long)n_slots * 8192 + (dump_enabled_ ? 1 + dump_slot_ : 0);
  auto it = graphs_.find(key);
  if (it == graphs_.end()) {
    cudaGraph_t g = nullptr;
    if (counter_) { counter_->capturing = true; counter_->captured = 0; }
    Q3_CUDA(cudaStreamBeginCapture(stream_, cudaStreamCaptureModeThreadLocal));
    try {
      issue_frame(n_slots);
    } catch (...) {
      cudaStreamEndCapture(stream_, &g);
      if (g) cudaGraphDestroy(g);
      if (counter_) counter_->capturing = false;
      throw;
    }
    cudaError_t e = cudaStreamEndCapture(stream_, &g);
    if (counter_) counter_->capturing = false;
    if (e != cudaSuccess) fail(Q3TTS_ERR_CUDA, "graph capture failed: %s", cudaGetErrorString(e));
    Graph gr;
    gr.nodes = counter_ ? counter_->captured : 0;
    e = cudaGraphInstantiate(&gr.exec, g, 0);
    cudaGraphDestroy(g);
    if (e != cudaSuccess) fail(Q3TTS_ERR_CUDA, "graph instantiate failed: %s", cudaGetErrorString(e));
    it = graphs_.emplace(key, gr).first;
  }
  for (int i = 0; i < n; ++i) {
    Q3_CUDA(cudaGraphLaunch(it->second.exec, stream_));
    if (counter_) counter_->n += it->second.nodes;
    ++graph_replays;
  }
}

void TalkerEngine::fetch_states(int n_slots, std::vector<SlotState>& out) {
  Q3_CUDA(cudaMemcpyAsync(h_state_, d_state_, sizeof(SlotState) * n_slots, cudaMemcpyDeviceToHost, stream_));
  Q3_CUDA(cudaStreamSynchronize(stream_));
  out.assign(h_state_, h_state_ + n_slots);
}

void TalkerEngine::fetch_frames(int slot, int first, int count, int32_t* dst) {
  if (count <= 0) return;
  Q3_CUDA(cudaMemcpyAsync(dst, d_frames_ + ((size_t)slot * opt_.max_frames + first) * 16, sizeof(int) * 16 * count,
                          cudaMemcpyDeviceToHost, stream_));
  Q3_CUDA(cudaStreamSynchronize(stream_));
}

void TalkerEngine::fetch_logits(int frames, float* code0_out, float* cp_out) {
  frames = std::min(frames, dump_cap_);
  if (frames <= 0) return;
  if (code0_out) Q3_CUDA(cudaMemcpyAsync(code0_out, d_dump0_, sizeof(float) * (size_t)frames * cfg_.vocab_size, cudaMemcpyDeviceToHost, stream_));
  if (cp_out) Q3_CUDA(cudaMemcpyAsync(cp_out, d_dumpcp_, sizeof(float) * (size_t)frames * 15 * cfg_.cp.vocab_size, cudaMemcpyDeviceToHost, stream_));
  Q3_CUDA(cudaStreamSynchronize(stream_));
}

double TalkerEngine::profile_linears(int which, int m, int iters, int64_t& launches, int64_t& bytes_per_iter) {
  const StackWeights& S = which == 0 ? w_.talker : w_.cp;
  Q3_CHECK(m >= 1 && m <= max_rows_, Q3TTS_ERR_INVALID_ARG, "m %d out of range (1..%d)", m, max_rows_);
  const LaunchCtx c{stream_, nullptr};
  const int qkv_ld = (S.heads + 2 * S.kv_heads) * 128, attn_ld = S.heads * 128;
  Q3_CUDA(cudaMemsetAsync(d_x_, 0, sizeof(float) * (size_t)m * S.hidden, stream_));
  Q3_CUDA(cudaMemsetAsync(d_attn_, 0, sizeof(float) * (size_t)m * attn_ld, stream_));
  if (d_h16_) {
    Q3_CUDA(cudaMemsetAsync(d_h16_, 0, (size_t)m * S.hidden * 2, stream_));
    Q3_CUDA(cudaMemsetAsync(d_attn16_, 0, (size_t)m * attn_ld * 2, stream_));
    Q3_CUDA(cudaMemsetAsync(d_act16_, 0, (size_t)m * S.inter * 2, stream_));
  }
  launches = 0;
  bytes_per_iter = 0;
  const bool tc = handle_tc_ && m >= tc_min_rows_ && !S.tc.empty();
  auto pass = [&](bool count) {
    for (int l = 0; l < S.layers; ++l) {
      const LayerWeights& L = S.layer[l];
      if (tc) {
        const LayerTc& T = S.tc[l];
        linear_tc(T.qkv, d_h16_, m, d_qkv_, qkv_ld, nullptr, 0, nullptr, TC_ACT_NONE, 0);
        linear_tc(T.o, d_attn16_, m, d_x_, S.hidden, nullptr, 0, nullptr, TC_ACT_NONE, 0);
        linear_tc(T.gate_up_il, d_h16_, m, nullptr, 0, d_act16_, S.inter, nullptr, TC_ACT_NONE, 1);
        linear_tc(T.down, d_act16_, m, d_x_, S.hidden, nullptr, 0, nullptr, TC_ACT_NONE, 0);
        if (count) { launches += 4; bytes_per_iter += (int64_t)(L.qkv.weight_bytes() + L.o.weight_bytes() + L.gate_up.weight_bytes() + L.down.weight_bytes()); }
        continue;
      }
      launch_linear(c, L.qkv, d_x_, S.hidden, m, d_qkv_, qkv_ld, L.in_norm, S.eps, EPI_STORE);
      launch_linear(c, L.o, d_attn_, attn_ld, m, d_x_, S.hidden, nullptr, 0.f, EPI_ADD);
      launch_linear(c, L.gate_up, d_x_, S.hidden, m, d_act_, S.inter, L.post_norm, S.eps, EPI_SWIGLU);
      launch_linear(c, L.down, d_act_, S.inter, m, d_x_, S.hidden, nullptr, 0.f, EPI_ADD);
      if (count) { launches += 4; bytes_per_iter += (int64_t)(L.qkv.weight_bytes() + L.o.weight_bytes() + L.gate_up.weight_bytes() + L.down.weight_bytes()); }
    }
    if (tc) {
      const TcLinear& head = which == 0 ? w_.codec_head_tc : w_.lm_head_tc[0];
      linear_tc(head, d_h16_, m, which == 0 ? d_logits0_ : d_cplogits_, head.out, nullptr, 0, nullptr, TC_ACT_NONE, 0);
      if (count) { launches += 1; bytes_per_iter += (int64_t)(which == 0 ? w_.codec_head : w_.lm_head[0]).weight_bytes(); }
      return;
    }
    const Linear& head = which == 0 ? w_.codec_head : w_.lm_head[0];
    launch_linear(c, head, d_x_, S.hidden, m, which == 0 ? d_logits0_ : d_cplogits_, head.out, S.final_norm, S.eps, EPI_STORE);
    if (count) { launches += 1; bytes_per_iter += (int64_t)head.weight_bytes(); }
  };
  pass(true);
  cudaGraph_t graph = nullptr;
  cudaGraphExec_t exec = nullptr;
  Q3_CUDA(cudaStreamBeginCapture(stream_, cudaStreamCaptureModeThreadLocal));
  pass(false);
  Q3_CUDA(cudaStreamEndCapture(stream_, &graph));
  Q3_CUDA(cudaGraphInstantiate(&exec, graph, 0));
  Q3_CUDA(cudaGraphLaunch(exec, stream_));
  Q3_CUDA(cudaEventRecord(ev_a_, stream_));
  for (int i = 0; i < iters; ++i) Q3_CUDA(cudaGraphLaunch(exec, stream_));
  Q3_CUDA(cudaEventRecord(ev_b_, stream_));
  Q3_CUDA(cudaStreamSynchronize(stream_));
  float ms = 0.f;
  cudaEventElapsedTime(&ms, ev_a_, ev_b_);
  cudaGraphExecDestroy(exec);
  cudaGraphDestroy(graph);
  launches *= iters;
  return ms;
}

int TalkerEngine::sample_probe(const float* logits, int vocab, float temperature, int top_k, float top_p, float rep_penalty,
                               const int32_t* token_set, int n_set, uint64_t seed, uint64_t counter) {
  Q3_CHECK(vocab > 0 && vocab <= 4096, Q3TTS_ERR_INVALID_ARG, "vocab %d out of range", vocab);
  std::vector<unsigned> bm(128, 0u);
  for (int i = 0; i < n_set; ++i)
    if (token_set[i] >= 0 && token_set[i] < vocab) bm[token_set[i] >> 5] |= 1u << (token_set[i] & 31);
  Q3_CUDA(cudaMemcpyAsync(d_probe_logits_, logits, sizeof(float) * vocab, cudaMemcpyHostToDevice, stream_));
  Q3_CUDA(cudaMemcpyAsync(d_probe_set_, bm.data(), sizeof(unsigned) * 128, cudaMemcpyHostToDevice, stream_));
  launch_sample_probe(ctx(), d_probe_logits_, vocab, cfg_.vocab_size, temperature, top_k, top_p > 0.f ? top_p : 1.f,
                      rep_penalty > 0.f ? rep_penalty : 1.f, n_set > 0 ? d_probe_set_ : nullptr, seed, counter, d_probe_out_);
  int id = -1;
  Q3_CUDA(cudaMemcpyAsync(&id, d_probe_out_, sizeof(int), cudaMemcpyDeviceToHost, stream_));
  Q3_CUDA(cudaStreamSynchronize(stream_));
  return id;
}

}
```

### mlx-swift-qwen3-tts_b200/csrc/talker_kernels.cu

```cuda
#include <cuda_bf16.h>
#include <cuda_fp16.h>

#include "kernels.h"
#include "device_utils.cuh"
#include "sampler.cuh"

namespace q3 {

__global__ void dequantize_kernel(const uint32_t* __restrict__ qw, const void* __restrict__ scales,
                                  const void* __restrict__ biases, int sdt, int out, int in, int group, int bits,
                                  int out_dt, void* __restrict__ dst) {
  const int per = 32 / bits;
  const size_t words = (size_t)out * (in / per);
  const uint32_t mask = (1u << bits) - 1u;
  for (size_t wi = (size_t)blockIdx.x * blockDim.x + threadIdx.x; wi < words; wi += (size_t)gridDim.x * blockDim.x) {
    const size_t row = wi / (in / per);
    const int col0 = (int)(wi % (in / per)) * per;
    const uint32_t w = qw[wi];
    const size_t gi = row * (in / group) + col0 / group;
    const float s = load_as_f32(scales, gi, sdt), b = load_as_f32(biases, gi, sdt);
    for (int j = 0; j < per; ++j) {
      const float q = (float)((w >> (j * bits)) & mask);
      const float v = __fadd_rn(__fmul_rn(s, q), b);
      const size_t o = row * in + col0 + j;
      if (out_dt == Q3TTS_F32) reinterpret_cast<float*>(dst)[o] = v;
      else if (out_dt == Q3TTS_F16) reinterpret_cast<__half*>(dst)[o] = __float2half_rn(v);
      else reinterpret_cast<__nv_bfloat16*>(dst)[o] = __float2bfloat16_rn(v);
    }
  }
}

void launch_dequantize(const LaunchCtx& c, const uint32_t* qw, const void* scales, const void* biases, int sdt, int out,
                       int in, int group, int bits, int out_dt, void* dst) {
  const size_t words = (size_t)out * in * bits / 32;
  int blocks = (int)std::min<size_t>((words + 255) / 256, 148 * 16);
  if (blocks < 1) blocks = 1;
  dequantize_kernel<<<blocks, 256, 0, c.stream>>>(qw, scales, biases, sdt, out, in, group, bits, out_dt, dst);
  c.tick();
}

__global__ void widen_bits_kernel(const uint32_t* __restrict__ src, size_t rows, int in, int bits, int cbits, uint32_t* __restrict__ dst) {
  const int per = 32 / cbits;
  const int src_words = in / 32 * bits, dst_words = in / per;
  const uint32_t mask = (1u << bits) - 1u;
  const size_t total = rows * (size_t)dst_words;
  for (size_t wi = (size_t)blockIdx.x * blockDim.x + threadIdx.x; wi < total; wi += (size_t)gridDim.x * blockDim.x) {
    const size_t row = wi / dst_words;
    const int col0 = (int)(wi - row * dst_words) * per;
    const uint32_t* s = src + row * src_words;
    const int bit0 = col0 * bits, w0 = bit0 >> 5;
    uint64_t v = s[w0];
    if (w0 + 1 < src_words) v |= (uint64_t)s[w0 + 1] << 32;
    v >>= bit0 & 31;
    uint32_t out = 0;
    for (int j = 0; j < per; ++j) out |= (uint32_t)((v >> (j * bits)) & mask) << (j * cbits);
    dst[wi] = out;
  }
}

void launch_widen_bits(const LaunchCtx& c, const uint32_t* src, int rows, int in, int bits, uint32_t* dst) {
  const int cbits = container_bits(bits);
  Q3_CHECK((bits == 2 || bits == 3 || bits == 5 || bits == 6) && in > 0 && in % 32 == 0 && rows > 0, Q3TTS_ERR_INVALID_ARG,
           "widen_bits: bits %d / in %d unsupported (bits 2, 3, 5 or 6, in a multiple of 32)", bits, in);
  const size_t words = (size_t)rows * in * cbits / 32;
  const int blocks = (int)std::max<size_t>(1, std::min<size_t>((words + 255) / 256, 148 * 16));
  widen_bits_kernel<<<blocks, 256, 0, c.stream>>>(src, (size_t)rows, in, bits, cbits, dst);
  c.tick();
}

__global__ void mlx_quantize_kernel(const void* __restrict__ w, int wdt, size_t groups, int in, int bits, uint32_t* __restrict__ qw8,
                                    void* __restrict__ scales, void* __restrict__ biases, void* __restrict__ fake) {
  const size_t g = (size_t)blockIdx.x * blockDim.x + threadIdx.x;
  if (g >= groups) return;
  const int gpr = in / 64;
  const size_t row = g / gpr;
  const size_t e0 = row * (size_t)in + (size_t)(g - row * gpr) * 64;
  float v[64];
  float mx = -INFINITY, mn = INFINITY;
#pragma unroll 8
  for (int j = 0; j < 64; ++j) {
    v[j] = load_as_f32(w, e0 + j, wdt);
    mx = fmaxf(mx, v[j]);
    mn = fminf(mn, v[j]);
  }
  const float n_bins = (float)((1 << bits) - 1);
  const bool side = fabsf(mn) > fabsf(mx);
  float s = fmaxf(__fdiv_rn(__fsub_rn(mx, mn), n_bins), 1e-7f);
  s = side ? s : -s;
  const float edge = side ? mn : mx;
  const float q0 = rintf(__fdiv_rn(edge, s));
  if (q0 != 0.f) s = __fdiv_rn(edge, q0);
  float b = q0 == 0.f ? 0.f : edge;
  if (wdt == Q3TTS_BF16) { s = __bfloat162float(__float2bfloat16_rn(s)); b = __bfloat162float(__float2bfloat16_rn(b)); }
  else if (wdt == Q3TTS_F16) { s = __half2float(__float2half_rn(s)); b = __half2float(__float2half_rn(b)); }
  const float s_safe = s == 0.f ? 1e-7f : s;
  if (wdt == Q3TTS_F32) { reinterpret_cast<float*>(scales)[g] = s; reinterpret_cast<float*>(biases)[g] = b; }
  else if (wdt == Q3TTS_F16) { reinterpret_cast<__half*>(scales)[g] = __float2half_rn(s); reinterpret_cast<__half*>(biases)[g] = __float2half_rn(b); }
  else { reinterpret_cast<__nv_bfloat16*>(scales)[g] = __float2bfloat16_rn(s); reinterpret_cast<__nv_bfloat16*>(biases)[g] = __float2bfloat16_rn(b); }
#pragma unroll 4
  for (int j = 0; j < 64; j += 4) {
    uint32_t word = 0;
#pragma unroll
    for (int u = 0; u < 4; ++u) {
      const float q = fminf(fmaxf(rintf(__fdiv_rn(__fsub_rn(v[j + u], b), s_safe)), 0.f), n_bins);
      word |= (uint32_t)q << (8 * u);
      if (fake) {
        const float d = __fadd_rn(__fmul_rn(s, q), b);
        const size_t o = e0 + j + u;
        if (wdt == Q3TTS_F32) reinterpret_cast<float*>(fake)[o] = d;
        else if (wdt == Q3TTS_F16) reinterpret_cast<__half*>(fake)[o] = __float2half_rn(d);
        else reinterpret_cast<__nv_bfloat16*>(fake)[o] = __float2bfloat16_rn(d);
      }
    }
    if (qw8) qw8[(e0 + j) >> 2] = word;
  }
}

void launch_mlx_quantize(const LaunchCtx& c, const void* w, int wdt, int out, int in, int bits, uint32_t* qw8, void* scales, void* biases,
                         void* fake) {
  Q3_CHECK(in % 64 == 0 && (bits == 4 || bits == 6 || bits == 8), Q3TTS_ERR_INVALID_ARG, "mlx_quantize: in %d / bits %d unsupported", in, bits);
  const size_t groups = (size_t)out * (in / 64);
  mlx_quantize_kernel<<<(unsigned)((groups + 127) / 128), 128, 0, c.stream>>>(w, wdt, groups, in, bits, qw8, scales, biases, fake);
  c.tick();
}

struct LinearKArgs {
  const void* w;
  const void* scales;
  const void* biases;
  const float* bias;
  const float* x;
  float* y;
  const float* norm_w;
  float eps;
  int out, in, group, sdt, m, ldx, ldy, epi;
};

template <int FMT, int MT>
__global__ void __launch_bounds__(256, (MT <= 2 ? 3 : 1)) linear_kernel(const LinearKArgs a) {
  constexpr int VPL = FmtTraits<FMT>::VPL;
  constexpr int KC = 32 * VPL;
  constexpr bool QUANT = (FMT == W_Q4 || FMT == W_Q8);
  constexpr int LPG = VPL / 4;
  extern __shared__ __align__(16) unsigned char smem_raw[];
  const int nchunk = (a.in + KC - 1) / KC;
  const int xstride = nchunk * (KC / 4);
  float4* xs = reinterpret_cast<float4*>(smem_raw);
  float* xsum = reinterpret_cast<float*>(smem_raw + (size_t)MT * xstride * sizeof(float4));
  __shared__ float red[MT][8];

  const int tid = threadIdx.x, lane = tid & 31, warp = tid >> 5;
  const int m0 = blockIdx.y * MT;
  const int in4 = a.in >> 2;
  const int out_eff = (a.epi == EPI_SWIGLU) ? (a.out >> 1) : a.out;
  const int nsub = (a.epi == EPI_SWIGLU) ? 2 : 1;
  const size_t row_bytes = QUANT ? (size_t)a.in * (FMT == W_Q4 ? 4 : 8) / 8 : (size_t)a.in * (FMT == W_F32 ? 4 : 2);
  const int ngroups = QUANT ? a.in / a.group : 0;
  const int r_first = blockIdx.x * 8 + warp;

  if (r_first < out_eff) {
    for (int s = 0; s < nsub; ++s) {
      const int row = r_first + s * out_eff;
      const unsigned char* wr = reinterpret_cast<const unsigned char*>(a.w) + (size_t)row * row_bytes;
      for (size_t off = (size_t)lane * 128; off < row_bytes; off += 32 * 128) prefetch_l2(wr + off);
      if constexpr (QUANT) {
        if (lane == 0) prefetch_l2(reinterpret_cast<const unsigned char*>(a.scales) + (size_t)row * ngroups * (a.sdt == Q3TTS_F32 ? 4 : 2));
        if (lane == 1) prefetch_l2(reinterpret_cast<const unsigned char*>(a.biases) + (size_t)row * ngroups * (a.sdt == Q3TTS_F32 ? 4 : 2));
      }
    }
  }

  const int iters = (in4 + 255) / 256;
#pragma unroll
  for (int mi = 0; mi < MT; ++mi) {
    const bool valid = (m0 + mi) < a.m;
    const float4* xr = reinterpret_cast<const float4*>(a.x + (size_t)(valid ? m0 + mi : 0) * a.ldx);
    float ss = 0.f;
    for (int it = 0; it < iters; ++it) {
      const int f = tid + it * 256;
      float4 v = make_float4(0.f, 0.f, 0.f, 0.f);
      if (valid && f < in4) v = xr[f];
      ss += v.x * v.x + v.y * v.y + v.z * v.z + v.w * v.w;
      if (a.norm_w != nullptr && f < in4) {
        const float4 nw = reinterpret_cast<const float4*>(a.norm_w)[f];
        v.x *= nw.x; v.y *= nw.y; v.z *= nw.z; v.w *= nw.w;
      }
      const int e = f << 2;
      const int ch = e / KC, ec = e - ch * KC;
      const int l = ec / VPL, j = (ec - l * VPL) >> 2;
      if (f < in4) xs[(size_t)mi * xstride + ch * (KC / 4) + j * 32 + l] = v;
      if constexpr (QUANT) {
        float s4 = (v.x + v.y) + (v.z + v.w);
#pragma unroll
        for (int o = 1; o < LPG; o <<= 1) s4 += __shfl_xor_sync(0xffffffffu, s4, o);
        if ((tid & (LPG - 1)) == 0 && f < in4) xsum[mi * (nchunk * 32) + ch * 32 + l] = s4;
      }
    }
    if (a.norm_w != nullptr) {
      ss = warp_sum(ss);
      if (lane == 0) red[mi][warp] = ss;
    }
  }
  __syncthreads();
  float inv_rms[MT];
#pragma unroll
  for (int mi = 0; mi < MT; ++mi) {
    inv_rms[mi] = 1.0f;
    if (a.norm_w != nullptr) {
      float s = 0.f;
#pragma unroll
      for (int w = 0; w < 8; ++w) s += red[mi][w];
      inv_rms[mi] = rsqrtf(s / (float)a.in + a.eps);
    }
  }

  for (int r = r_first; r < out_eff; r += gridDim.x * 8) {
    float yold[MT];
#pragma unroll
    for (int mi = 0; mi < MT; ++mi) yold[mi] = (a.epi == EPI_ADD && lane == 0 && m0 + mi < a.m) ? a.y[(size_t)(m0 + mi) * a.ldy + r] : 0.f;
    float res[2][MT];
#pragma unroll
    for (int s = 0; s < 2; ++s) {
#pragma unroll
      for (int mi = 0; mi < MT; ++mi) res[s][mi] = 0.f;
    }
#pragma unroll
    for (int s = 0; s < 2; ++s) {
      if (s >= nsub) break;
      const int row = r + s * out_eff;
      const uint4* wr = reinterpret_cast<const uint4*>(reinterpret_cast<const unsigned char*>(a.w) + (size_t)row * row_bytes);
      float acc[MT];
#pragma unroll
      for (int mi = 0; mi < MT; ++mi) acc[mi] = 0.f;
      for (int c0 = 0; c0 < nchunk; c0 += 4) {
        uint4 wv[4];
        float scv[4], biv[4];
#pragma unroll
        for (int u = 0; u < 4; ++u) {
          if ((c0 + u) * KC + lane * VPL < a.in) {
            wv[u] = ldg_stream(wr + (size_t)(c0 + u) * 32 + lane);
            if constexpr (QUANT) {
              const size_t gi = (size_t)row * ngroups + ((c0 + u) * KC + lane * VPL) / a.group;
              scv[u] = load_as_f32(a.scales, gi, a.sdt);
              biv[u] = load_as_f32(a.biases, gi, a.sdt);
            }
          }
        }
#pragma unroll
        for (int u = 0; u < 4; ++u) {
          if ((c0 + u) * KC + lane * VPL < a.in) {
            const int ch = c0 + u;
            float wf[VPL];
            lane_expand<FMT>(wv[u], wf);
#pragma unroll
            for (int mi = 0; mi < MT; ++mi) {
              const float d = lane_dot<FMT>(wf, xs + (size_t)mi * xstride + ch * (KC / 4) + lane);
              if constexpr (QUANT) acc[mi] += scv[u] * d + biv[u] * xsum[mi * (nchunk * 32) + ch * 32 + lane];
              else acc[mi] += d;
            }
          }
        }
      }
#pragma unroll
      for (int mi = 0; mi < MT; ++mi) res[s][mi] = warp_sum(acc[mi]) * inv_rms[mi];
    }
    if (lane == 0) {
#pragma unroll
      for (int mi = 0; mi < MT; ++mi) {
        if (m0 + mi >= a.m) break;
        float v = res[0][mi];
        float* yp = a.y + (size_t)(m0 + mi) * a.ldy + r;
        if (a.epi == EPI_SWIGLU) {
          float g = v, u = res[1][mi];
          if (a.bias) { g += a.bias[r]; u += a.bias[r + out_eff]; }
          *yp = silu_f(g) * u;
        } else {
          if (a.bias) v += a.bias[r];
          if (a.epi == EPI_SILU) v = silu_f(v);
          if (a.epi == EPI_ADD) v += yold[mi];
          *yp = v;
        }
      }
    }
  }
}

template <int FMT, int MT>
static void launch_linear_t(const LaunchCtx& c, const LinearKArgs& a, int num_sms) {
  constexpr int VPL = FmtTraits<FMT>::VPL;
  constexpr bool QUANT = (FMT == W_Q4 || FMT == W_Q8);
  constexpr int KC = 32 * VPL;
  const int nchunk = (a.in + KC - 1) / KC;
  size_t smem = (size_t)MT * nchunk * KC * sizeof(float) + (QUANT ? (size_t)MT * nchunk * 32 * sizeof(float) : 0);
  const int out_eff = (a.epi == EPI_SWIGLU) ? a.out / 2 : a.out;
  int bx = (out_eff + 7) / 8;
  const int cap = num_sms * 8;
  if (bx > cap) bx = cap;
  dim3 grid(bx, (a.m + MT - 1) / MT);
  linear_kernel<FMT, MT><<<grid, 256, smem, c.stream>>>(a);
  c.tick();
}

template <int FMT>
static void launch_linear_f(const LaunchCtx& c, LinearKArgs a) {
  int mt = 8;
  while (mt > 1 && (mt > a.m * 2 - 1 || (size_t)mt * a.in * 5 > 96 * 1024)) mt >>= 1;
  if (a.m == 1) mt = 1;
  switch (mt) {
    case 8: launch_linear_t<FMT, 8>(c, a, 148); break;
    case 4: launch_linear_t<FMT, 4>(c, a, 148); break;
    case 2: launch_linear_t<FMT, 2>(c, a, 148); break;
    default: launch_linear_t<FMT, 1>(c, a, 148); break;
  }
}

void launch_linear(const LaunchCtx& c, const Linear& L, const float* x, int ldx, int m, float* y, int ldy,
                   const float* norm_w, float eps, int epilogue) {
  if (m <= 0) return;
  LinearKArgs a;
  a.w = L.bits ? (const void*)L.qw : L.w;
  a.scales = L.scales; a.biases = L.biases; a.bias = L.bias;
  a.x = x; a.y = y; a.norm_w = norm_w; a.eps = eps;
  a.out = L.out; a.in = L.in; a.group = L.group; a.sdt = L.sdt; a.m = m; a.ldx = ldx; a.ldy = ldy; a.epi = epilogue;
  Q3_CHECK((ldx % 4) == 0, Q3TTS_ERR_INVALID_ARG, "linear: activation stride %d not 16-byte aligned", ldx);
  if (L.bits == 4) {
    Q3_CHECK(L.in % 32 == 0 && L.group % 32 == 0, Q3TTS_ERR_BAD_CONFIG, "4-bit linear needs in %% 32 == 0 and group %% 32 == 0 (in=%d, group=%d)", L.in, L.group);
    launch_linear_f<W_Q4>(c, a);
  } else if (L.bits == 8) {
    Q3_CHECK(L.in % 16 == 0 && L.group % 16 == 0, Q3TTS_ERR_BAD_CONFIG, "8-bit linear needs in %% 16 == 0 (in=%d)", L.in);
    launch_linear_f<W_Q8>(c, a);
  } else if (L.bits == 0) {
    if (L.sdt == Q3TTS_BF16) { Q3_CHECK(L.in % 8 == 0, Q3TTS_ERR_BAD_CONFIG, "bf16 linear needs in %% 8 == 0 (in=%d)", L.in); launch_linear_f<W_BF16>(c, a); }
    else if (L.sdt == Q3TTS_F16) { Q3_CHECK(L.in % 8 == 0, Q3TTS_ERR_BAD_CONFIG, "f16 linear needs in %% 8 == 0 (in=%d)", L.in); launch_linear_f<W_F16>(c, a); }
    else { Q3_CHECK(L.in % 4 == 0, Q3TTS_ERR_BAD_CONFIG, "f32 linear needs in %% 4 == 0 (in=%d)", L.in); launch_linear_f<W_F32>(c, a); }
  } else {
    fail(Q3TTS_ERR_BAD_CONFIG, "unsupported quantisation bits %d (4 and 8 are in scope; 6-bit runtime quantisation is not)", L.bits);
  }
}

__global__ void __launch_bounds__(256) rmsnorm_kernel(const float* __restrict__ x, int ldx, int dim, const float* __restrict__ w,
                                                      float eps, float* __restrict__ y, int ldy) {
  __shared__ float red[8];
  const float* xr = x + (size_t)blockIdx.x * ldx;
  float ss = 0.f;
  for (int i = threadIdx.x; i < dim; i += 256) { const float v = xr[i]; ss += v * v; }
  ss = warp_sum(ss);
  if ((threadIdx.x & 31) == 0) red[threadIdx.x >> 5] = ss;
  __syncthreads();
  float tot = 0.f;
#pragma unroll
  for (int i = 0; i < 8; ++i) tot += red[i];
  const float inv = rsqrtf(tot / (float)dim + eps);
  float* yr = y + (size_t)blockIdx.x * ldy;
  for (int i = threadIdx.x; i < dim; i += 256) yr[i] = xr[i] * inv * w[i];
}
void launch_rmsnorm(const LaunchCtx& c, const float* x, int ldx, int m, int dim, const float* w, float eps, float* y, int ldy) {
  if (m <= 0) return;
  rmsnorm_kernel<<<m, 256, 0, c.stream>>>(x, ldx, dim, w, eps, y, ldy);
  c.tick();
}

__device__ __forceinline__ float4 kv_ld4(const float* p) { return *reinterpret_cast<const float4*>(p); }
__device__ __forceinline__ float4 kv_ld4(const __half* p) {
  const uint2 u = *reinterpret_cast<const uint2*>(p);
  const float2 a = __half22float2(*reinterpret_cast<const __half2*>(&u.x)), b = __half22float2(*reinterpret_cast<const __half2*>(&u.y));
  return make_float4(a.x, a.y, b.x, b.y);
}
__device__ __forceinline__ float kv_ld(const float* p) { return *p; }
__device__ __forceinline__ float kv_ld(const __half* p) { return __half2float(*p); }
__device__ __forceinline__ void kv_st(float* p, float v) { *p = v; }
__device__ __forceinline__ void kv_st(__half* p, float v) { *p = __float2half_rn(v); }
template <typename KvT>
__global__ void __launch_bounds__(128) qk_norm_rope_append_kernel(float* __restrict__ qkv, int ld, int m, int heads, int kv_heads,
                                                                  const float* __restrict__ q_norm, const float* __restrict__ k_norm,
                                                                  float eps, const float* __restrict__ inv_freq,
                                                                  const int* __restrict__ row_slot, const int* __restrict__ row_pos,
                                                                  KVLayout kv) {
  const int total_heads = heads + 2 * kv_heads;
  const int gw = blockIdx.x * 4 + (threadIdx.x >> 5);
  if (gw >= m * total_heads) return;
  const int row = gw / total_heads, head = gw - row * total_heads;
  const int lane = threadIdx.x & 31;
  float* p = qkv + (size_t)row * ld + (size_t)head * 128;
  const int slot = row_slot[row], pos = row_pos[row];
  const int ring = pos % kv.capacity;
  if (head >= heads + kv_heads) {
    KvT* dst = static_cast<KvT*>(kv.v) + (size_t)slot * kv.slot_stride + ((size_t)(head - heads - kv_heads) * kv.capacity + ring) * 128;
    const float4 v4 = reinterpret_cast<const float4*>(p)[lane];
    kv_st(dst + 4 * lane, v4.x); kv_st(dst + 4 * lane + 1, v4.y); kv_st(dst + 4 * lane + 2, v4.z); kv_st(dst + 4 * lane + 3, v4.w);
    return;
  }
  const float a0 = p[lane], a1 = p[lane + 32], b0 = p[lane + 64], b1 = p[lane + 96];
  const float ss = warp_sum(a0 * a0 + a1 * a1 + b0 * b0 + b1 * b1);
  const float inv = rsqrtf(ss * (1.0f / 128.0f) + eps);
  const float* nw = head < heads ? q_norm : k_norm;
  const float x0 = a0 * inv * nw[lane], x1 = a1 * inv * nw[lane + 32];
  const float y0 = b0 * inv * nw[lane + 64], y1 = b1 * inv * nw[lane + 96];
  const float fp = (float)pos;
  float s0, c0, s1, c1;
  sincosf(fp * inv_freq[lane], &s0, &c0);
  sincosf(fp * inv_freq[lane + 32], &s1, &c1);
  const float o0 = x0 * c0 - y0 * s0, o1 = x1 * c1 - y1 * s1;
  const float o2 = y0 * c0 + x0 * s0, o3 = y1 * c1 + x1 * s1;
  if (head >= heads) {
    KvT* dst = static_cast<KvT*>(kv.k) + (size_t)slot * kv.slot_stride + ((size_t)(head - heads) * kv.capacity + ring) * 128;
    kv_st(dst + lane, o0); kv_st(dst + lane + 32, o1); kv_st(dst + lane + 64, o2); kv_st(dst + lane + 96, o3);
  } else {
    p[lane] = o0; p[lane + 32] = o1; p[lane + 64] = o2; p[lane + 96] = o3;
  }
}
void launch_qk_norm_rope_append(const LaunchCtx& c, float* qkv, int ld, int m, int heads, int kv_heads, int head_dim,
                                const float* q_norm, const float* k_norm, float eps, const float* inv_freq,
                                const int* row_slot, const int* row_pos, const KVLayout& kv) {
  Q3_CHECK(head_dim == 128, Q3TTS_ERR_BAD_CONFIG, "talker kernels are specialised for head_dim 128 (got %d)", head_dim);
  const int warps = m * (heads + 2 * kv_heads);
  if (warps <= 0) return;
  if (kv.f16)
    qk_norm_rope_append_kernel<__half><<<(warps + 3) / 4, 128, 0, c.stream>>>(qkv, ld, m, heads, kv_heads, q_norm, k_norm, eps, inv_freq, row_slot, row_pos, kv);
  else
    qk_norm_rope_append_kernel<float><<<(warps + 3) / 4, 128, 0, c.stream>>>(qkv, ld, m, heads, kv_heads, q_norm, k_norm, eps, inv_freq, row_slot, row_pos, kv);
  c.tick();
}

__device__ __forceinline__ void store_act(float* p, float v) { *p = v; }
__device__ __forceinline__ void store_act(__half* p, float v) { *p = __float2half_rn(v); }

template <int G, typename OutT, typename KvT>
__global__ void __launch_bounds__(128) attention_kernel(const float* __restrict__ qkv, int ld, int heads, int kv_heads,
                                                        const int* __restrict__ row_slot, const int* __restrict__ row_pos,
                                                        const int* __restrict__ win_start, KVLayout kv, OutT* __restrict__ out,
                                                        int ldo, float scale) {
  extern __shared__ __align__(16) float sm[];
  float* q = sm;
  float* sc = sm + G * 128;
  __shared__ float red_max[G], red_sum[G];
  const int row = blockIdx.x, kvh = blockIdx.y, tid = threadIdx.x, lane = tid & 31, warp = tid >> 5;
  const int slot = row_slot[row], pos = row_pos[row];
  const int w0 = win_start ? win_start[slot] : 0;
  const int S = pos - w0 + 1;
  const int cap = kv.capacity;
  const int r0 = w0 % cap;
  const KvT* kb = static_cast<const KvT*>(kv.k) + (size_t)slot * kv.slot_stride + (size_t)kvh * cap * 128;
  const KvT* vb = static_cast<const KvT*>(kv.v) + (size_t)slot * kv.slot_stride + (size_t)kvh * cap * 128;
#pragma unroll
  for (int g = 0; g < G; ++g) q[g * 128 + tid] = qkv[(size_t)row * ld + (size_t)(kvh * G + g) * 128 + tid];
  __syncthreads();
  for (int j = tid; j < S; j += 128) {
    const int rj = r0 + j;
    const KvT* kr = kb + (size_t)(rj >= cap ? rj - cap : rj) * 128;
    float acc[G];
#pragma unroll
    for (int g = 0; g < G; ++g) acc[g] = 0.f;
#pragma unroll 8
    for (int d = 0; d < 32; ++d) {
      const float4 kk = kv_ld4(kr + 4 * d);
#pragma unroll
      for (int g = 0; g < G; ++g) {
        const float4 qq = reinterpret_cast<const float4*>(q + g * 128)[d];
        acc[g] += kk.x * qq.x + kk.y * qq.y + kk.z * qq.z + kk.w * qq.w;
      }
    }
#pragma unroll
    for (int g = 0; g < G; ++g) sc[g * S + j] = acc[g] * scale;
  }
  __syncthreads();
  for (int g = warp; g < G; g += 4) {
    float mx = -INFINITY;
    for (int j = lane; j < S; j += 32) mx = fmaxf(mx, sc[g * S + j]);
    mx = warp_max(mx);
    float sum = 0.f;
    for (int j = lane; j < S; j += 32) { const float e = expf(sc[g * S + j] - mx); sc[g * S + j] = e; sum += e; }
    sum = warp_sum(sum);
    if (lane == 0) { red_max[g] = mx; red_sum[g] = sum; }
  }
  __syncthreads();
  float o[G];
#pragma unroll
  for (int g = 0; g < G; ++g) o[g] = 0.f;
  for (int j = 0; j < S; ++j) {
    const int rj = r0 + j;
    const float vv = kv_ld(vb + (size_t)(rj >= cap ? rj - cap : rj) * 128 + tid);
#pragma unroll
    for (int g = 0; g < G; ++g) o[g] = fmaf(sc[g * S + j], vv, o[g]);
  }
#pragma unroll
  for (int g = 0; g < G; ++g) store_act(out + (size_t)row * ldo + (size_t)(kvh * G + g) * 128 + tid, o[g] / red_sum[g]);
}
template <int G, typename OutT, typename KvT>
__global__ void __launch_bounds__(128, 4) rope_attention_kernel(const float* __restrict__ qkv, int ld, int heads, int kv_heads,
                                                             const float* __restrict__ q_norm, const float* __restrict__ k_norm, float eps,
                                                             const float* __restrict__ inv_freq, const int* __restrict__ row_slot,
                                                             const int* __restrict__ row_pos, const int* __restrict__ win_start, KVLayout kv,
                                                             OutT* __restrict__ out, int ldo, float scale) {
  __shared__ __align__(16) float q[G * 128];
  __shared__ __align__(16) float part_o[4][G][128];
  __shared__ float part_m[4][G], part_l[4][G];
  pdl_launch_dependents();
  pdl_wait();
  const int row = blockIdx.x, kvh = blockIdx.y, tid = threadIdx.x, lane = tid & 31, warp = tid >> 5;
  const int slot = row_slot[row], pos = row_pos[row];
  const int w0 = win_start ? win_start[slot] : 0;
  const int S = pos - w0 + 1;
  const int cap = kv.capacity;
  const int r0 = w0 % cap;
  const int ring = (r0 + S - 1 >= cap) ? r0 + S - 1 - cap : r0 + S - 1;
  KvT* kb = static_cast<KvT*>(kv.k) + (size_t)slot * kv.slot_stride + (size_t)kvh * cap * 128;
  KvT* vb = static_cast<KvT*>(kv.v) + (size_t)slot * kv.slot_stride + (size_t)kvh * cap * 128;
  const float* rowp = qkv + (size_t)row * ld;
  for (int hh = warp; hh <= G; hh += 4) {
    const float* src = rowp + (size_t)(hh < G ? (kvh * G + hh) : (heads + kvh)) * 128;
    const float a0 = src[lane], a1 = src[lane + 32], b0 = src[lane + 64], b1 = src[lane + 96];
    const float ss = warp_sum(a0 * a0 + a1 * a1 + b0 * b0 + b1 * b1);
    const float inv = rsqrtf(ss * (1.0f / 128.0f) + eps);
    const float* nw = hh < G ? q_norm : k_norm;
    const float x0 = a0 * inv * nw[lane], x1 = a1 * inv * nw[lane + 32], y0 = b0 * inv * nw[lane + 64], y1 = b1 * inv * nw[lane + 96];
    float s0, c0, s1, c1;
    sincosf((float)pos * inv_freq[lane], &s0, &c0);
    sincosf((float)pos * inv_freq[lane + 32], &s1, &c1);
    const float o0 = x0 * c0 - y0 * s0, o1 = x1 * c1 - y1 * s1, o2 = y0 * c0 + x0 * s0, o3 = y1 * c1 + x1 * s1;
    if (hh < G) {
      float* dst = q + hh * 128;
      dst[lane] = o0; dst[lane + 32] = o1; dst[lane + 64] = o2; dst[lane + 96] = o3;
    } else {
      KvT* dst = kb + (size_t)ring * 128;
      kv_st(dst + lane, o0); kv_st(dst + lane + 32, o1); kv_st(dst + lane + 64, o2); kv_st(dst + lane + 96, o3);
    }
  }
  kv_st(vb + (size_t)ring * 128 + tid, rowp[(size_t)(heads + kv_heads + kvh) * 128 + tid]);
  __syncthreads();
  const int seg = lane & 7, grp = warp * 4 + (lane >> 3);
  float qf[G][16];
#pragma unroll
  for (int g = 0; g < G; ++g)
#pragma unroll
    for (int i = 0; i < 4; ++i) {
      const float4 t = *reinterpret_cast<const float4*>(q + g * 128 + i * 32 + seg * 4);
      qf[g][4 * i] = t.x * scale; qf[g][4 * i + 1] = t.y * scale; qf[g][4 * i + 2] = t.z * scale; qf[g][4 * i + 3] = t.w * scale;
    }
  float mx[G], l[G], o[G][16];
#pragma unroll
  for (int g = 0; g < G; ++g) {
    mx[g] = -INFINITY; l[g] = 0.f;
#pragma unroll
    for (int d = 0; d < 16; ++d) o[g][d] = 0.f;
  }
  for (int jb = 0; jb < S; jb += 32) {
    const int j0 = jb + grp;
    float4 kk[2][4], vv[2][4];
#pragma unroll
    for (int u = 0; u < 2; ++u) {
      const int j = j0 + 16 * u;
      const int rj = r0 + (j < S ? j : 0);
      const size_t base = (size_t)(rj >= cap ? rj - cap : rj) * 128 + seg * 4;
#pragma unroll
      for (int i = 0; i < 4; ++i) {
        kk[u][i] = kv_ld4(kb + base + i * 32);
        vv[u][i] = kv_ld4(vb + base + i * 32);
      }
    }
#pragma unroll
    for (int u = 0; u < 2; ++u) {
      const bool valid = j0 + 16 * u < S;
#pragma unroll
      for (int g = 0; g < G; ++g) {
        float sdot = 0.f;
#pragma unroll
        for (int i = 0; i < 4; ++i)
          sdot += kk[u][i].x * qf[g][4 * i] + kk[u][i].y * qf[g][4 * i + 1] + kk[u][i].z * qf[g][4 * i + 2] + kk[u][i].w * qf[g][4 * i + 3];
        sdot += __shfl_xor_sync(0xffffffffu, sdot, 1);
        sdot += __shfl_xor_sync(0xffffffffu, sdot, 2);
        sdot += __shfl_xor_sync(0xffffffffu, sdot, 4);
        if (!valid) sdot = -INFINITY;
        const float mn = fmaxf(mx[g], sdot);
        const bool none = mn == -INFINITY;
        const float corr = none ? 1.f : expf(mx[g] - mn), pr = none ? 0.f : expf(sdot - mn);
        mx[g] = mn;
        l[g] = l[g] * corr + pr;
#pragma unroll
        for (int i = 0; i < 4; ++i) {
          o[g][4 * i] = o[g][4 * i] * corr + pr * vv[u][i].x;
          o[g][4 * i + 1] = o[g][4 * i + 1] * corr + pr * vv[u][i].y;
          o[g][4 * i + 2] = o[g][4 * i + 2] * corr + pr * vv[u][i].z;
          o[g][4 * i + 3] = o[g][4 * i + 3] * corr + pr * vv[u][i].w;
        }
      }
    }
  }
#pragma unroll
  for (int g = 0; g < G; ++g) {
    float m_all = fmaxf(mx[g], __shfl_xor_sync(0xffffffffu, mx[g], 8));
    m_all = fmaxf(m_all, __shfl_xor_sync(0xffffffffu, m_all, 16));
    const float f = (mx[g] == -INFINITY) ? 0.f : expf(mx[g] - m_all);
    float lw = l[g] * f;
    lw += __shfl_xor_sync(0xffffffffu, lw, 8);
    lw += __shfl_xor_sync(0xffffffffu, lw, 16);
#pragma unroll
    for (int d = 0; d < 16; ++d) {
      float t = o[g][d] * f;
      t += __shfl_xor_sync(0xffffffffu, t, 8);
      t += __shfl_xor_sync(0xffffffffu, t, 16);
      o[g][d] = t;
    }
    if (lane < 8) {
#pragma unroll
      for (int i = 0; i < 4; ++i)
        *reinterpret_cast<float4*>(&part_o[warp][g][i * 32 + seg * 4]) = make_float4(o[g][4 * i], o[g][4 * i + 1], o[g][4 * i + 2], o[g][4 * i + 3]);
      if (lane == 0) { part_m[warp][g] = m_all; part_l[warp][g] = lw; }
    }
  }
  __syncthreads();
#pragma unroll
  for (int g = 0; g < G; ++g) {
    float m_all = fmaxf(fmaxf(part_m[0][g], part_m[1][g]), fmaxf(part_m[2][g], part_m[3][g]));
    float num = 0.f, den = 0.f;
#pragma unroll
    for (int w = 0; w < 4; ++w) {
      const float f = (part_m[w][g] == -INFINITY) ? 0.f : expf(part_m[w][g] - m_all);
      num += part_o[w][g][tid] * f;
      den += part_l[w][g] * f;
    }
    store_act(out + (size_t)row * ldo + (size_t)(kvh * G + g) * 128 + tid, num / den);
  }
}
template <int G>
__global__ void __launch_bounds__(128) cp_pass0_attention_kernel(const float* __restrict__ qkv, int ld, int heads, int kv_heads,
                                                                 const float* __restrict__ q_norm, const float* __restrict__ k_norm, float eps,
                                                                 const float* __restrict__ inv_freq, KVLayout kv, __half* __restrict__ out,
                                                                 int ldo, float scale) {
  __shared__ __align__(16) float q1[G * 128];
  __shared__ __align__(16) float kk[2][128];
  __shared__ __align__(16) float vv[2][128];
  __shared__ float w0[G], w1[G];
  pdl_launch_dependents();
  pdl_wait();
  const int slot = blockIdx.x, kvh = blockIdx.y, tid = threadIdx.x, lane = tid & 31, warp = tid >> 5;
  float* kb = static_cast<float*>(kv.k) + (size_t)slot * kv.slot_stride + (size_t)kvh * kv.capacity * 128;
  float* vb = static_cast<float*>(kv.v) + (size_t)slot * kv.slot_stride + (size_t)kvh * kv.capacity * 128;
  for (int item = warp; item < G + 2; item += 4) {
    const int pos = item < G ? 1 : item - G;
    const float* rowp = qkv + (size_t)(2 * slot + pos) * ld;
    const float* src = rowp + (size_t)(item < G ? (kvh * G + item) : (heads + kvh)) * 128;
    const float a0 = src[lane], a1 = src[lane + 32], b0 = src[lane + 64], b1 = src[lane + 96];
    const float ss = warp_sum(a0 * a0 + a1 * a1 + b0 * b0 + b1 * b1);
    const float inv = rsqrtf(ss * (1.0f / 128.0f) + eps);
    const float* nw = item < G ? q_norm : k_norm;
    const float x0 = a0 * inv * nw[lane], x1 = a1 * inv * nw[lane + 32], y0 = b0 * inv * nw[lane + 64], y1 = b1 * inv * nw[lane + 96];
    float s0 = 0.f, c0 = 1.f, s1 = 0.f, c1 = 1.f;
    if (pos == 1) {
      sincosf(inv_freq[lane], &s0, &c0);
      sincosf(inv_freq[lane + 32], &s1, &c1);
    }
    const float o0 = x0 * c0 - y0 * s0, o1 = x1 * c1 - y1 * s1, o2 = y0 * c0 + x0 * s0, o3 = y1 * c1 + x1 * s1;
    float* dst = item < G ? q1 + item * 128 : kk[pos];
    dst[lane] = o0; dst[lane + 32] = o1; dst[lane + 64] = o2; dst[lane + 96] = o3;
    if (item >= G) {
      float* kd = kb + (size_t)pos * 128;
      kd[lane] = o0; kd[lane + 32] = o1; kd[lane + 64] = o2; kd[lane + 96] = o3;
    }
  }
#pragma unroll
  for (int pos = 0; pos < 2; ++pos) {
    const float v = qkv[(size_t)(2 * slot + pos) * ld + (size_t)(heads + kv_heads + kvh) * 128 + tid];
    vv[pos][tid] = v;
    vb[(size_t)pos * 128 + tid] = v;
  }
  __syncthreads();
  for (int g = warp; g < G; g += 4) {
    float d0 = 0.f, d1 = 0.f;
#pragma unroll
    for (int i = 0; i < 4; ++i) {
      const float qv = q1[g * 128 + lane + 32 * i];
      d0 = fmaf(qv, kk[0][lane + 32 * i], d0);
      d1 = fmaf(qv, kk[1][lane + 32 * i], d1);
    }
    d0 = warp_sum(d0) * scale;
    d1 = warp_sum(d1) * scale;
    const float mx = fmaxf(d0, d1);
    const float e0 = expf(d0 - mx), e1 = expf(d1 - mx);
    if (lane == 0) { w0[g] = e0 / (e0 + e1); w1[g] = e1 / (e0 + e1); }
  }
  __syncthreads();
#pragma unroll
  for (int g = 0; g < G; ++g) {
    out[(size_t)(2 * slot) * ldo + (size_t)(kvh * G + g) * 128 + tid] = __float2half_rn(vv[0][tid]);
    out[(size_t)(2 * slot + 1) * ldo + (size_t)(kvh * G + g) * 128 + tid] = __float2half_rn(w0[g] * vv[0][tid] + w1[g] * vv[1][tid]);
  }
}
void launch_cp_pass0_attention_f16(const LaunchCtx& c, const float* qkv, int ld, int n_slots, int heads, int kv_heads, const float* q_norm,
                                   const float* k_norm, float eps, const float* inv_freq, const KVLayout& kv, __half* out, int ldo) {
  if (n_slots <= 0) return;
  const int G = heads / kv_heads;
  const float scale = 1.0f / sqrtf(128.0f);
  dim3 grid(n_slots, kv_heads);
  const bool pdl = pdl_enabled();
  Q3_CHECK(G == 1 || G == 2 || G == 4, Q3TTS_ERR_BAD_CONFIG, "unsupported GQA group size %d", G);
  if (G == 1) launch_kernel_pdl(cp_pass0_attention_kernel<1>, grid, dim3(128), 0, c.stream, pdl, qkv, ld, heads, kv_heads, q_norm, k_norm, eps, inv_freq, kv, out, ldo, scale);
  else if (G == 2) launch_kernel_pdl(cp_pass0_attention_kernel<2>, grid, dim3(128), 0, c.stream, pdl, qkv, ld, heads, kv_heads, q_norm, k_norm, eps, inv_freq, kv, out, ldo, scale);
  else launch_kernel_pdl(cp_pass0_attention_kernel<4>, grid, dim3(128), 0, c.stream, pdl, qkv, ld, heads, kv_heads, q_norm, k_norm, eps, inv_freq, kv, out, ldo, scale);
  c.tick();
}

template <typename OutT>
static void launch_rope_attention_t(const LaunchCtx& c, const float* qkv, int ld, int m, int heads, int kv_heads, const float* q_norm,
                                    const float* k_norm, float eps, const float* inv_freq, const int* row_slot, const int* row_pos,
                                    const int* win_start, const KVLayout& kv, OutT* out, int ldo) {
  if (m <= 0) return;
  const int G = heads / kv_heads;
  const float scale = 1.0f / sqrtf(128.0f);
  const size_t smem = 0;
  dim3 grid(m, kv_heads);
  const bool pdl = pdl_enabled();
  Q3_CHECK(G == 1 || G == 2 || G == 4, Q3TTS_ERR_BAD_CONFIG, "unsupported GQA group size %d", G);
#define RA_LAUNCH(GV)                                                                                                                              \
  {                                                                                                                                                \
    if (kv.f16) launch_kernel_pdl(rope_attention_kernel<GV, OutT, __half>, grid, dim3(128), smem, c.stream, pdl, qkv, ld, heads, kv_heads, q_norm, k_norm, eps, \
                                  inv_freq, row_slot, row_pos, win_start, kv, out, ldo, scale);                                                    \
    else launch_kernel_pdl(rope_attention_kernel<GV, OutT, float>, grid, dim3(128), smem, c.stream, pdl, qkv, ld, heads, kv_heads, q_norm, k_norm, eps,         \
                           inv_freq, row_slot, row_pos, win_start, kv, out, ldo, scale);                                                           \
  }
  if (G == 1) RA_LAUNCH(1)
  else if (G == 2) RA_LAUNCH(2)
  else RA_LAUNCH(4)
#undef RA_LAUNCH
  c.tick();
}
void launch_rope_attention(const LaunchCtx& c, const float* qkv, int ld, int m, int heads, int kv_heads, const float* q_norm,
                           const float* k_norm, float eps, const float* inv_freq, const int* row_slot, const int* row_pos,
                           const int* win_start, const KVLayout& kv, float* out, int ldo) {
  launch_rope_attention_t<float>(c, qkv, ld, m, heads, kv_heads, q_norm, k_norm, eps, inv_freq, row_slot, row_pos, win_start, kv, out, ldo);
}
void launch_rope_attention_f16(const LaunchCtx& c, const float* qkv, int ld, int m, int heads, int kv_heads, const float* q_norm,
                               const float* k_norm, float eps, const float* inv_freq, const int* row_slot, const int* row_pos,
                               const int* win_start, const KVLayout& kv, __half* out, int ldo) {
  launch_rope_attention_t<__half>(c, qkv, ld, m, heads, kv_heads, q_norm, k_norm, eps, inv_freq, row_slot, row_pos, win_start, kv, out, ldo);
}

template <typename OutT>
static void launch_attention_t(const LaunchCtx& c, const float* qkv, int ld, int m, int heads, int kv_heads, int head_dim,
                               const int* row_slot, const int* row_pos, const int* win_start, const KVLayout& kv, OutT* out, int ldo) {
  Q3_CHECK(head_dim == 128, Q3TTS_ERR_BAD_CONFIG, "talker kernels are specialised for head_dim 128 (got %d)", head_dim);
  if (m <= 0) return;
  const int G = heads / kv_heads;
  const float scale = 1.0f / sqrtf((float)head_dim);
  const size_t smem = (size_t)G * (128 + kv.capacity) * sizeof(float);
  dim3 grid(m, kv_heads);
#define Q3_ATT(GV)                                                                                                     \
  {                                                                                                                    \
    if (kv.f16) attention_kernel<GV, OutT, __half><<<grid, 128, smem, c.stream>>>(qkv, ld, heads, kv_heads, row_slot, row_pos, win_start, kv, out, ldo, scale); \
    else attention_kernel<GV, OutT, float><<<grid, 128, smem, c.stream>>>(qkv, ld, heads, kv_heads, row_slot, row_pos, win_start, kv, out, ldo, scale); \
  }
  Q3_CHECK(smem <= 160 * 1024, Q3TTS_ERR_CAPACITY, "kv_capacity %d too large for the attention kernel", kv.capacity);
  if (G == 1) Q3_ATT(1) else if (G == 2) Q3_ATT(2) else if (G == 4) Q3_ATT(4)
  else fail(Q3TTS_ERR_BAD_CONFIG, "unsupported GQA group size %d", G);
#undef Q3_ATT
  c.tick();
}
void launch_attention(const LaunchCtx& c, const float* qkv, int ld, int m, int heads, int kv_heads, int head_dim,
                      const int* row_slot, const int* row_pos, const int* win_start, const KVLayout& kv, float* out, int ldo) {
  launch_attention_t<float>(c, qkv, ld, m, heads, kv_heads, head_dim, row_slot, row_pos, win_start, kv, out, ldo);
}
void launch_attention_f16(const LaunchCtx& c, const float* qkv, int ld, int m, int heads, int kv_heads, int head_dim,
                          const int* row_slot, const int* row_pos, const int* win_start, const KVLayout& kv, __half* out, int ldo) {
  launch_attention_t<__half>(c, qkv, ld, m, heads, kv_heads, head_dim, row_slot, row_pos, win_start, kv, out, ldo);
}

__global__ void weight_to_f16_kernel(const void* __restrict__ w, int dt, int rows, int cols, int interleave, const float* __restrict__ col_scale,
                                     __half* __restrict__ dst) {
  const size_t total = (size_t)rows * cols;
  for (size_t i = (size_t)blockIdx.x * blockDim.x + threadIdx.x; i < total; i += (size_t)gridDim.x * blockDim.x) {
    const int r = (int)(i / cols), cidx = (int)(i - (size_t)r * cols);
    int dr = r;
    if (interleave) dr = r < rows / 2 ? 2 * r : 2 * (r - rows / 2) + 1;
    const float v = load_as_f32(w, i, dt);
    dst[(size_t)dr * cols + cidx] = __float2half_rn(col_scale ? v * col_scale[cidx] : v);
  }
}
void launch_weight_to_f16(const LaunchCtx& c, const void* w, int dt, int rows, int cols, bool interleave_halves, __half* dst,
                          const float* col_scale) {
  const size_t total = (size_t)rows * cols;
  if (total == 0) return;
  const int blocks = (int)std::min<size_t>((total + 255) / 256, 148 * 32);
  weight_to_f16_kernel<<<blocks, 256, 0, c.stream>>>(w, dt, rows, cols, interleave_halves ? 1 : 0, col_scale, dst);
  c.tick();
}

__global__ void gather_rows_f16_kernel(Embedding e, const int* __restrict__ ids, __half* __restrict__ y, int ldy) {
  const int row = blockIdx.x;
  const int id = ids[row];
  for (int d = threadIdx.x; d < e.dim; d += blockDim.x)
    y[(size_t)row * ldy + d] = (id >= 0 && id < e.rows) ? __float2half_rn(load_as_f32(e.w, (size_t)id * e.dim + d, e.dt)) : __float2half_rn(0.f);
}
void launch_gather_rows_f16(const LaunchCtx& c, const Embedding& e, const int* ids, int n, __half* y, int ldy) {
  if (n <= 0) return;
  gather_rows_f16_kernel<<<n, 256, 0, c.stream>>>(e, ids, y, ldy);
  c.tick();
}

__global__ void gather_rows_kernel(Embedding e, const int* __restrict__ ids, int n, float* __restrict__ y, int ldy, int accumulate) {
  const int row = blockIdx.x;
  const int id = ids[row];
  if (id < 0 || id >= e.rows) return;
  for (int d = threadIdx.x; d < e.dim; d += blockDim.x) {
    const float v = load_as_f32(e.w, (size_t)id * e.dim + d, e.dt);
    float* p = y + (size_t)row * ldy + d;
    *p = accumulate ? (*p + v) : v;
  }
}
void launch_gather_rows(const LaunchCtx& c, const Embedding& e, const int* ids, int n, float* y, int ldy, bool accumulate) {
  if (n <= 0) return;
  gather_rows_kernel<<<n, 256, 0, c.stream>>>(e, ids, n, y, ldy, accumulate ? 1 : 0);
  c.tick();
}

__global__ void assemble_rows_kernel(const float* __restrict__ tp_rows, int H, Embedding codec, const float* __restrict__ spk,
                                     const int* __restrict__ desc, float* __restrict__ y) {
  const int row = blockIdx.x;
  const int tp = desc[row * 3 + 0], cd = desc[row * 3 + 1], sp = desc[row * 3 + 2];
  for (int d = threadIdx.x; d < H; d += blockDim.x) {
    float v = 0.f;
    if (tp >= 0) v += tp_rows[(size_t)tp * H + d];
    if (cd >= 0) v += load_as_f32(codec.w, (size_t)cd * H + d, codec.dt);
    if (sp > 0) v += spk[(size_t)(sp - 1) * H + d];
    y[(size_t)row * H + d] = v;
  }
}
void launch_assemble_rows(const LaunchCtx& c, const float* tp_rows, int H, const Embedding& codec, const float* spk,
                          const int* desc, int n, float* y) {
  if (n <= 0) return;
  assemble_rows_kernel<<<n, 256, 0, c.stream>>>(tp_rows, H, codec, spk, desc, y);
  c.tick();
}

__global__ void __launch_bounds__(kSampleThreads) sample_kernel(const float* __restrict__ logits, int ld, SlotState* __restrict__ st,
                                                               SamplerParams p, unsigned* __restrict__ token_sets,
                                                               int* __restrict__ cur_codes, const int* __restrict__ forced,
                                                               int max_frames, float* __restrict__ dump, int dump_stride_frame,
                                                               int dump_offset, int dump_slot, NextInput ni) {
  __shared__ float sl[kMaxVocab];
  __shared__ BlockRed br;
  sample_slot<0, kSampleThreads>(blockIdx.x, logits, ld, st, p, token_sets, cur_codes, forced, max_frames, dump, dump_stride_frame, dump_offset, dump_slot, sl, br);
  if (ni.mode == 0) return;
  __syncthreads();
  const int slot = blockIdx.x, H = ni.H;
  const int code = cur_codes[slot * p.groups + p.group];
  if (ni.mode == 1) {
    const bool ok = code >= 0 && code < ni.codec.rows;
    for (int d = threadIdx.x; d < H; d += kSampleThreads) {
      const float a = ni.h_last[(size_t)slot * H + d];
      const float b = ok ? load_as_f32(ni.codec.w, (size_t)code * H + d, ni.codec.dt) : 0.f;
      ni.y32[(size_t)(2 * slot) * H + d] = a;
      ni.y32[(size_t)(2 * slot + 1) * H + d] = b;
      if (ni.y16) {
        ni.y16[(size_t)(2 * slot) * H + d] = __float2half_rn(a * ni.y16_scale);
        ni.y16[(size_t)(2 * slot + 1) * H + d] = __float2half_rn(b * ni.y16_scale);
      }
    }
  } else {
    const Embedding e = ni.cp_emb[p.group - 1];
    const bool ok = code >= 0 && code < e.rows;
    for (int d = threadIdx.x; d < H; d += kSampleThreads) {
      const float v = ok ? load_as_f32(e.w, (size_t)code * H + d, e.dt) : 0.f;
      ni.y32[(size_t)slot * H + d] = v;
      if (ni.y16) ni.y16[(size_t)slot * H + d] = __float2half_rn(v * ni.y16_scale);
    }
  }
}
void launch_sample(const LaunchCtx& c, const float* logits, int ld, int n_slots, SlotState* st, const SamplerParams& p,
                   unsigned* token_sets, int* cur_codes, const int* forced, int max_frames, float* logits_dump,
                   int dump_stride_frame, int dump_offset, int dump_slot, const NextInput& ni) {
  Q3_CHECK(p.vocab <= kMaxVocab, Q3TTS_ERR_BAD_CONFIG, "sampler supports vocab <= %d (got %d)", kMaxVocab, p.vocab);
  sample_kernel<<<n_slots, kSampleThreads, 0, c.stream>>>(logits, ld, st, p, token_sets, cur_codes, forced, max_frames, logits_dump,
                                                          dump_stride_frame, dump_offset, dump_slot, ni);
  c.tick();
}

__global__ void __launch_bounds__(kSampleThreads) sample_probe_kernel(const float* __restrict__ logits, int V, int codec_vocab,
                                                                     float temperature, int top_k, float top_p, float rep_penalty,
                                                                     const unsigned* __restrict__ set_bitmap, unsigned long long seed,
                                                                     unsigned long long counter, int* __restrict__ id_out) {
  __shared__ float sl[kMaxVocab];
  __shared__ BlockRed br;
  for (int i = threadIdx.x; i < V; i += kSampleThreads) sl[i] = logits[i];
  __syncthreads();
  const int tok = sample_block<0, kSampleThreads>(sl, V, codec_vocab, temperature, top_k, top_p, rep_penalty, set_bitmap, seed, counter, br);
  if (threadIdx.x == 0) *id_out = tok;
}
void launch_sample_probe(const LaunchCtx& c, const float* logits, int vocab, int codec_vocab, float temperature, int top_k,
                         float top_p, float rep_penalty, const unsigned* set_bitmap, unsigned long long seed,
                         unsigned long long counter, int* id_out) {
  Q3_CHECK(vocab <= kMaxVocab, Q3TTS_ERR_INVALID_ARG, "sampler supports vocab <= %d (got %d)", kMaxVocab, vocab);
  sample_probe_kernel<<<1, kSampleThreads, 0, c.stream>>>(logits, vocab, codec_vocab, temperature, top_k, top_p, rep_penalty,
                                                          set_bitmap, seed, counter, id_out);
  c.tick();
}

template <int FORM>
constexpr int probe_threads() { return FORM == 0 ? kSampleThreads : kFrameSampleThreads; }

template <int FORM, bool DUMP>
__global__ void __launch_bounds__(kSampleThreads) sampler_probe_kernel(const float* __restrict__ logits, int ld, int V, int codec_vocab,
                                                                      SamplerProbeRows rows, int* __restrict__ ids,
                                                                      float* __restrict__ processed) {
  constexpr int NT = probe_threads<FORM>();
  __shared__ float sl[kMaxVocab];
  __shared__ BlockRed br;
  if (threadIdx.x >= NT) return;
  const int r = blockIdx.x;
  for (int i = threadIdx.x; i < V; i += NT) sl[i] = logits[(size_t)r * ld + i];
  block_sync<FORM, NT>();
  const int tok = sample_block<FORM, NT, DUMP>(sl, V, codec_vocab, rows.temperature[r], rows.top_k[r], rows.top_p[r], rows.rep_penalty[r],
                                               rows.sets ? rows.sets + (size_t)r * (kMaxVocab / 32) : nullptr, rows.seed[r], rows.counter[r],
                                               br, DUMP ? processed + (size_t)r * V : nullptr);
  if (threadIdx.x == 0) ids[r] = tok;
}
void launch_sampler_probe(const LaunchCtx& c, int form, const float* logits, int ld, int n_rows, int V, int codec_vocab,
                          const SamplerProbeRows& rows, int* ids, float* processed) {
  Q3_CHECK(V >= 1 && V <= kMaxVocab && n_rows >= 1 && (form == 0 || form == 1), Q3TTS_ERR_INVALID_ARG, "sampler probe: bad V %d / rows %d / form %d",
           V, n_rows, form);
  auto k = form == 0 ? (processed ? sampler_probe_kernel<0, true> : sampler_probe_kernel<0, false>)
                     : (processed ? sampler_probe_kernel<1, true> : sampler_probe_kernel<1, false>);
  k<<<n_rows, kSampleThreads, 0, c.stream>>>(logits, ld, V, codec_vocab, rows, ids, processed);
  c.tick();
}

__global__ void __launch_bounds__(kSampleThreads) sample_slot_frame_form_kernel(const float* __restrict__ logits, int ld, SlotState* __restrict__ st,
                                                                               SamplerParams p, unsigned* __restrict__ token_sets,
                                                                               int* __restrict__ cur_codes, const int* __restrict__ forced,
                                                                               int max_frames, float* __restrict__ dump, int dump_stride_frame,
                                                                               int dump_offset, int dump_slot) {
  __shared__ float sl[kMaxVocab];
  __shared__ BlockRed br;
  if (threadIdx.x >= kFrameSampleThreads) return;
  sample_slot<1, kFrameSampleThreads>(blockIdx.x, logits, ld, st, p, token_sets, cur_codes, forced, max_frames, dump, dump_stride_frame,
                                      dump_offset, dump_slot, sl, br);
}
void launch_sample_frame_form(const LaunchCtx& c, const float* logits, int ld, int n_slots, SlotState* st, const SamplerParams& p,
                              unsigned* token_sets, int* cur_codes, const int* forced, int max_frames, float* logits_dump,
                              int dump_stride_frame, int dump_offset, int dump_slot) {
  Q3_CHECK(p.vocab <= kMaxVocab, Q3TTS_ERR_BAD_CONFIG, "sampler supports vocab <= %d (got %d)", kMaxVocab, p.vocab);
  sample_slot_frame_form_kernel<<<n_slots, kSampleThreads, 0, c.stream>>>(logits, ld, st, p, token_sets, cur_codes, forced, max_frames,
                                                                          logits_dump, dump_stride_frame, dump_offset, dump_slot);
  c.tick();
}

__global__ void cp_input_kernel(int pass, const float* __restrict__ h_last, int H, Embedding codec, const Embedding* __restrict__ cp_emb,
                                const int* __restrict__ cur_codes, float* __restrict__ y, int groups) {
  const int slot = blockIdx.x;
  if (pass == 0) {
    const int code0 = cur_codes[slot * groups];
    const bool ok = code0 >= 0 && code0 < codec.rows;
    for (int d = threadIdx.x; d < H; d += blockDim.x) {
      y[(size_t)(2 * slot) * H + d] = h_last[(size_t)slot * H + d];
      y[(size_t)(2 * slot + 1) * H + d] = ok ? load_as_f32(codec.w, (size_t)code0 * H + d, codec.dt) : 0.f;
    }
  } else {
    const Embedding e = cp_emb[pass - 1];
    const int code = cur_codes[slot * groups + pass];
    const bool ok = code >= 0 && code < e.rows;
    for (int d = threadIdx.x; d < H; d += blockDim.x)
      y[(size_t)slot * H + d] = ok ? load_as_f32(e.w, (size_t)code * H + d, e.dt) : 0.f;
  }
}
void launch_cp_input(const LaunchCtx& c, int pass, int n_slots, const float* h_last, int H, const Embedding& codec,
                     const Embedding* cp_emb_dev, const int* cur_codes, float* y) {
  cp_input_kernel<<<n_slots, 256, 0, c.stream>>>(pass, h_last, H, codec, cp_emb_dev, cur_codes, y, 16);
  c.tick();
}

__global__ void frame_finalize_kernel(SlotState* __restrict__ st, const int* __restrict__ cur_codes, int* __restrict__ frames_out,
                                      int max_frames, unsigned* __restrict__ token_sets, int set_words,
                                      const float* __restrict__ trailing, int max_trailing, const float* __restrict__ tts_pad,
                                      Embedding codec, const Embedding* __restrict__ cp_emb, int H, float* __restrict__ x_next,
                                      __half* __restrict__ x16_next, float x16_scale) {
  const int slot = blockIdx.x;
  SlotState& s = st[slot];
  if (!s.frame_alive) return;
  constexpr int G = 16;
  __shared__ int codes[G];
  __shared__ const void* rowp[G];
  __shared__ int rowdt[G];
  if (threadIdx.x < G) {
    const int g = threadIdx.x, code = cur_codes[slot * G + g];
    codes[g] = code;
    const Embedding e = g == 0 ? codec : cp_emb[g - 1];
    const bool ok = code >= 0 && code < e.rows;
    rowp[g] = ok ? static_cast<const char*>(e.w) + (size_t)code * H * (e.dt == Q3TTS_F32 ? 4 : 2) : nullptr;
    rowdt[g] = e.dt;
  }
  __syncthreads();
  const int ti = s.trailing_idx;
  const float* text = (ti < s.total_text) ? trailing + ((size_t)slot * max_trailing + ti) * H : tts_pad;
  for (int d = threadIdx.x; d < H; d += blockDim.x) {
    float v[G];
#pragma unroll
    for (int g = 0; g < G; ++g) v[g] = rowp[g] ? load_as_f32(rowp[g], (size_t)d, rowdt[g]) : 0.f;
    float sum = v[0];
#pragma unroll
    for (int g = 1; g < G; ++g) sum += v[g];
    const float x = text[d] + sum;
    x_next[(size_t)slot * H + d] = x;
    if (x16_next) x16_next[(size_t)slot * H + d] = __float2half_rn(x * x16_scale);
  }
  __syncthreads();
  if (threadIdx.x == 0) {
    if (s.n_frames < max_frames) {
      for (int g = 0; g < G; ++g) frames_out[((size_t)slot * max_frames + s.n_frames) * G + g] = codes[g];
      s.n_frames += 1;
    }
    if (codes[0] >= 0 && codes[0] < set_words * 32) {
      unsigned* set0 = token_sets + (size_t)slot * G * set_words;
      set0[codes[0] >> 5] |= 1u << (codes[0] & 31);
    }
    if (ti < s.total_text) s.trailing_idx = ti + 1;
  }
}
void launch_frame_finalize(const LaunchCtx& c, int n_slots, SlotState* st, const int* cur_codes, int* frames_out,
                           int max_frames, unsigned* token_sets, int set_words, const float* trailing, int max_trailing,
                           const float* tts_pad, const Embedding& codec, const Embedding* cp_emb_dev, int H, float* x_next,
                           __half* x16_next, float x16_scale) {
  frame_finalize_kernel<<<n_slots, 256, 0, c.stream>>>(st, cur_codes, frames_out, max_frames, token_sets, set_words, trailing,
                                                       max_trailing, tts_pad, codec, cp_emb_dev, H, x_next, x16_next, x16_scale);
  c.tick();
}

__global__ void step_advance_kernel(int n_slots, SlotState* __restrict__ st, int window) {
  const int slot = blockIdx.x * blockDim.x + threadIdx.x;
  if (slot >= n_slots) return;
  SlotState& s = st[slot];
  if (!s.frame_alive) return;
  s.pos += 1;
  s.step += 1;
  if (s.step % 15 == 0 && s.pos - s.win_start > window) s.win_start = s.pos - window;
  if (s.step >= s.max_tokens) s.finished = 1;
  s.frame_alive = 0;
}
void launch_step_advance(const LaunchCtx& c, int n_slots, SlotState* st, int window) {
  step_advance_kernel<<<(n_slots + 63) / 64, 64, 0, c.stream>>>(n_slots, st, window);
  c.tick();
}

__global__ void step_rows_kernel(int n_slots, const SlotState* __restrict__ st, int* __restrict__ row_slot, int* __restrict__ row_pos,
                                 int* __restrict__ win_start) {
  const int slot = blockIdx.x * blockDim.x + threadIdx.x;
  if (slot >= n_slots) return;
  row_slot[slot] = slot;
  row_pos[slot] = st[slot].pos;
  win_start[slot] = st[slot].win_start;
}
void launch_step_rows(const LaunchCtx& c, int n_slots, const SlotState* st, int* row_slot, int* row_pos, int* win_start) {
  step_rows_kernel<<<(n_slots + 63) / 64, 64, 0, c.stream>>>(n_slots, st, row_slot, row_pos, win_start);
  c.tick();
}

template <int FMT>
static void init_linear_fmt() {
  Q3_CUDA(cudaFuncSetAttribute(linear_kernel<FMT, 1>, cudaFuncAttributeMaxDynamicSharedMemorySize, 200 * 1024));
  Q3_CUDA(cudaFuncSetAttribute(linear_kernel<FMT, 2>, cudaFuncAttributeMaxDynamicSharedMemorySize, 200 * 1024));
  Q3_CUDA(cudaFuncSetAttribute(linear_kernel<FMT, 4>, cudaFuncAttributeMaxDynamicSharedMemorySize, 200 * 1024));
  Q3_CUDA(cudaFuncSetAttribute(linear_kernel<FMT, 8>, cudaFuncAttributeMaxDynamicSharedMemorySize, 200 * 1024));
}
void init_talker_kernels() {
  init_linear_fmt<W_Q4>();
  init_linear_fmt<W_Q8>();
  init_linear_fmt<W_BF16>();
  init_linear_fmt<W_F16>();
  init_linear_fmt<W_F32>();
#define Q3_ATT_ATTR(GV, OT, KT) Q3_CUDA(cudaFuncSetAttribute(attention_kernel<GV, OT, KT>, cudaFuncAttributeMaxDynamicSharedMemorySize, 160 * 1024));
#define Q3_ATT_ATTR_G(OT, KT) Q3_ATT_ATTR(1, OT, KT) Q3_ATT_ATTR(2, OT, KT) Q3_ATT_ATTR(4, OT, KT)
  Q3_ATT_ATTR_G(float, float) Q3_ATT_ATTR_G(float, __half) Q3_ATT_ATTR_G(__half, float) Q3_ATT_ATTR_G(__half, __half)
#undef Q3_ATT_ATTR_G
#undef Q3_ATT_ATTR
}

}
```

Baseline: 1122.

## Fuse code-predictor pass into one persistent cooperative tcgen05 kernel

Adds a persistent cooperative kernel that runs every GEMM and attention phase of a code-predictor pass in a single launch. Warp 0 issues TMA loads, warp 1 issues UMMA into tensor memory, and the consumer warps do the split-K reductions and the RoPE attention, with global counters acting as grid-wide barriers between phases. Weight tiles for the next phase are prefetched before the barrier so loads overlap with the previous phase. The aim is to remove per-kernel launch and drain gaps across the fifteen small passes per frame, at the cost of spin-wait grid synchronisation, timeout error handling and heavy use of shared memory.

```diff
diff --git a/mlx-swift-qwen3-tts_b200/csrc/cp_pass.h b/mlx-swift-qwen3-tts_b200/csrc/cp_pass.h
--- /dev/null
+++ b/mlx-swift-qwen3-tts_b200/csrc/cp_pass.h
@@ -0,0 +1,55 @@
+#pragma once
+#include <cuda.h>
+
+#include "kernels.h"
+#include "skinny_common.cuh"
+
+namespace q3 {
+
+enum CpPhaseKind { CP_GEMM = 0, CP_ATTN = 1 };
+
+struct alignas(64) CpPhase {
+  CUtensorMap tmW;
+  CUtensorMap tmX;
+  skinny::SkParams p;
+  int kind;
+  int items;
+  const float* qkv;
+  int ld, ldo;
+  const float *q_norm, *k_norm;
+  KVLayout kv;
+  __half* out;
+};
+
+struct CpPassParams {
+  const CpPhase* phases;
+  int n_phases;
+  int max_tiles;
+  int heads, kv_heads;
+  float eps, attn_scale;
+  const float* inv_freq;
+  const int* row_slot;
+  const int* row_pos;
+  int row_pos_stride;
+  unsigned* sync;
+  int* error;
+  float* part;
+  int ring_stages, stage_bytes, attn_bytes;
+};
+
+struct CpPassPlan {
+  bool ok = false;
+  int grid = 0, G = 0;
+  size_t smem = 0;
+  CpPassParams p{};
+  CpPhase* d_phases = nullptr;
+};
+
+constexpr int kCpPassThreads = 320;
+constexpr int kCpAttnGroups = 2;
+
+size_t cp_pass_smem(int G, int m_pad, int* stages, int* stage_bytes, int* attn_bytes);
+int cp_pass_max_blocks_per_sm(int G, size_t smem);
+void launch_cp_pass(const LaunchCtx& c, const CpPassPlan& plan, int g);
+
+}
diff --git a/mlx-swift-qwen3-tts_b200/csrc/cp_pass_kernel.cu b/mlx-swift-qwen3-tts_b200/csrc/cp_pass_kernel.cu
--- /dev/null
+++ b/mlx-swift-qwen3-tts_b200/csrc/cp_pass_kernel.cu
@@ -0,0 +1,322 @@
+#include <algorithm>
+
+#include "cp_pass.h"
+#include "rope_attention.cuh"
+
+namespace q3 {
+
+namespace {
+
+using namespace skinny;
+
+constexpr unsigned long long kWaitNs = 2000000000ull;
+
+__device__ __forceinline__ bool cp_failed(const int* err) { return *reinterpret_cast<const volatile int*>(err) != 0; }
+__device__ __forceinline__ unsigned ld_acquire_u32(const unsigned* p) {
+  unsigned v;
+  asm volatile("ld.acquire.gpu.global.u32 %0, [%1];" : "=r"(v) : "l"(p) : "memory");
+  return v;
+}
+
+__device__ bool wait_count(const unsigned* cnt, unsigned target, int* err, int phase) {
+  unsigned long long t0 = 0;
+  for (uint32_t i = 0;; ++i) {
+    if (ld_acquire_u32(cnt) >= target) return true;
+    if ((i & 15) == 15) {
+      if (cp_failed(err)) return false;
+      const unsigned long long t = sk_globaltimer();
+      if (t0 == 0) t0 = t;
+      else if (t - t0 > kWaitNs) { atomicCAS(err, 0, 1 + phase); return false; }
+    }
+  }
+}
+__device__ bool mbar_wait_bounded(uint64_t* bar, uint32_t parity, int* err, int phase) {
+  unsigned long long t0 = 0;
+  for (uint32_t i = 0;; ++i) {
+    if (mbar_try_wait(bar, parity)) return true;
+    if ((i & 15) == 15) {
+      if (cp_failed(err)) return false;
+      const unsigned long long t = sk_globaltimer();
+      if (t0 == 0) t0 = t;
+      else if (t - t0 > kWaitNs) { atomicCAS(err, 0, 1 + phase); return false; }
+    }
+  }
+}
+__device__ __forceinline__ void group_bar(int id) { asm volatile("bar.sync %0, 128;" ::"r"(id) : "memory"); }
+__device__ __forceinline__ void consumer_bar() { asm volatile("bar.sync 5, %0;" ::"n"(kCpPassThreads - 64) : "memory"); }
+
+template <bool SWIGLU>
+__device__ __forceinline__ void reduce_rows(const CpPassParams& P, const SkParams& p, int item, const float* rowscale_s, int row) {
+  const int tile = item >> p.split_shift, r = item & (p.split - 1);
+  const int n = tile * kRowsW + row;
+  const bool n_ok = n < p.N;
+  const float bias = (p.bias && n_ok) ? p.bias[n] : 0.f;
+  const int so = SWIGLU ? (n >> 1) : n;
+  const float scale = (p.scale && n_ok) ? p.scale[so] : 1.f;
+  const bool lane_out = n_ok && (!SWIGLU || (n & 1) == 0);
+  const int m_base = r * p.mc;
+  const float* src0 = P.part + (size_t)tile * p.split * p.m_pad * kRowsW + (size_t)m_base * kRowsW + row;
+  for (int cb = 0; cb < p.mc; cb += 16) {
+    const int nc = p.mc - cb < 16 ? p.mc - cb : 16;
+    int valid = p.M - (m_base + cb);
+    valid = valid < nc ? valid : nc;
+    float a16[16];
+#pragma unroll
+    for (int j = 0; j < 16; ++j) a16[j] = 0.f;
+    for (int s = 0; s < p.split; ++s) {
+      const float* src = src0 + ((size_t)s * p.m_pad + cb) * kRowsW;
+#pragma unroll
+      for (int c = 0; c < 16; ++c)
+        if (c < valid) a16[c] += __ldcg(src + (size_t)c * kRowsW);
+    }
+    if (!lane_out) valid = 0;
+    float r16[16];
+    sk_load_res<16>(p, r16, valid, m_base + cb, so);
+    sk_finish<16, TC_ACT_NONE, SWIGLU>(p, a16, r16, valid, m_base + cb, so, bias, scale, p.rms_x ? rowscale_s + cb : nullptr);
+  }
+}
+
+template <int G>
+__global__ void __launch_bounds__(kCpPassThreads, 1) cp_pass_kernel(const CpPassParams P) {
+  extern __shared__ uint8_t smem_raw[];
+  uint8_t* smem = reinterpret_cast<uint8_t*>((reinterpret_cast<uintptr_t>(smem_raw) + 1023) & ~(uintptr_t)1023);
+  uint8_t* ring = smem;
+  uint8_t* attn = ring + (size_t)P.ring_stages * P.stage_bytes;
+  uint64_t* full = reinterpret_cast<uint64_t*>(attn + (size_t)kCpAttnGroups * P.attn_bytes);
+  uint64_t* empty = full + P.ring_stages;
+  uint64_t* tfull = empty + P.ring_stages;
+  uint64_t* tempty = tfull + 2;
+  uint32_t* tmem_slot = reinterpret_cast<uint32_t*>(tempty + 2);
+  int* flag = reinterpret_cast<int*>(tmem_slot + 1);
+  int* last = flag + 1;
+  float* rowscale_s = reinterpret_cast<float*>(tmem_slot + 4);
+
+  const int warp = threadIdx.x >> 5, lane = threadIdx.x & 31;
+  const int m_pad = P.phases[0].p.m_pad;
+  const uint32_t x_bytes = (uint32_t)m_pad * kBlockK * 2;
+  const int grid = gridDim.x;
+  if (threadIdx.x == 0) {
+    for (int s = 0; s < P.ring_stages; ++s) { mbar_init(&full[s], 1); mbar_init(&empty[s], 1); }
+    for (int i = 0; i < 2; ++i) { mbar_init(&tfull[i], 1); mbar_init(&tempty[i], 128); }
+    asm volatile("fence.mbarrier_init.release.cluster;" ::: "memory");
+    asm volatile("fence.proxy.async.shared::cta;" ::: "memory");
+  }
+  if (warp == 1) {
+    asm volatile("tcgen05.alloc.cta_group::1.sync.aligned.shared::cta.b32 [%0], %1;" ::"r"(smem_u32(tmem_slot)), "r"(256) : "memory");
+    asm volatile("tcgen05.relinquish_alloc_permit.cta_group::1.sync.aligned;" ::: "memory");
+  }
+  tc_fence_before();
+  __syncthreads();
+  tc_fence_after();
+  const uint32_t tmem_base = *tmem_slot;
+
+  if (warp == 0) {
+    const bool lead = elect_one();
+    bool ok = true;
+    int s = 0;
+    uint32_t ph = 0;
+    for (int k = 0; k < P.n_phases; ++k) {
+      const CpPhase& F = P.phases[k];
+      if (F.kind != CP_GEMM) continue;
+      const SkParams& p = F.p;
+      int s1 = s, j = 0;
+      uint32_t ph1 = ph;
+      for (int i = blockIdx.x; i < F.items; i += grid) {
+        const int tile = i >> p.split_shift, sl = i & (p.split - 1);
+        const int kb0 = (sl * p.num_kb) >> p.split_shift, kb1 = ((sl + 1) * p.num_kb) >> p.split_shift;
+        for (int kb = kb0; kb < kb1; ++kb, ++j) {
+          if (j < P.ring_stages) {
+            ok = ok && mbar_wait_bounded(&empty[s1], ph1 ^ 1u, P.error, k);
+            if (lead && ok) {
+              mbar_expect_tx(&full[s1], (uint32_t)kWBytes + x_bytes);
+              tma_load_2d(ring + (size_t)s1 * P.stage_bytes, &F.tmW, &full[s1], kb * kBlockK, tile * kRowsW);
+            }
+            if (++s1 == P.ring_stages) { s1 = 0; ph1 ^= 1u; }
+          } else if (lead) {
+            tma_prefetch_2d(&F.tmW, kb * kBlockK, tile * kRowsW);
+          }
+        }
+      }
+      const int pre = j < P.ring_stages ? j : P.ring_stages;
+      if (k > 0) ok = ok && wait_count(&P.sync[k - 1], (unsigned)grid, P.error, k);
+      asm volatile("fence.proxy.async.global;" ::: "memory");
+      j = 0;
+      for (int i = blockIdx.x; i < F.items; i += grid) {
+        const int tile = i >> p.split_shift, sl = i & (p.split - 1);
+        const int kb0 = (sl * p.num_kb) >> p.split_shift, kb1 = ((sl + 1) * p.num_kb) >> p.split_shift;
+        for (int kb = kb0; kb < kb1; ++kb, ++j) {
+          if (j >= pre) {
+            ok = ok && mbar_wait_bounded(&empty[s], ph ^ 1u, P.error, k);
+            if (lead && ok) {
+              mbar_expect_tx(&full[s], (uint32_t)kWBytes + x_bytes);
+              tma_load_2d(ring + (size_t)s * P.stage_bytes, &F.tmW, &full[s], kb * kBlockK, tile * kRowsW);
+            }
+          }
+          if (lead && ok) tma_load_2d(ring + (size_t)s * P.stage_bytes + kWBytes, &F.tmX, &full[s], kb * kBlockK, 0);
+          if (++s == P.ring_stages) { s = 0; ph ^= 1u; }
+        }
+      }
+    }
+    __syncwarp();
+  } else if (warp == 1) {
+    const bool lead = elect_one();
+    const uint32_t idesc = (1u << 4) | ((uint32_t)(m_pad >> 3) << 17) | ((uint32_t)(kRowsW >> 4) << 24);
+    bool ok = true;
+    int s = 0;
+    uint32_t ph = 0, uses[2] = {0u, 0u};
+    for (int k = 0; k < P.n_phases; ++k) {
+      const CpPhase& F = P.phases[k];
+      if (F.kind != CP_GEMM) continue;
+      const SkParams& p = F.p;
+      int it = 0;
+      for (int i = blockIdx.x; i < F.items; i += grid, ++it) {
+        if (uses[it] > 0) ok = ok && mbar_wait_bounded(&tempty[it], (uses[it] - 1u) & 1u, P.error, k);
+        tc_fence_after();
+        const uint32_t dcol = tmem_base + (uint32_t)(it * m_pad);
+        const int sl = i & (p.split - 1);
+        const int kb0 = (sl * p.num_kb) >> p.split_shift, kb1 = ((sl + 1) * p.num_kb) >> p.split_shift;
+        for (int kb = kb0; kb < kb1; ++kb) {
+          ok = ok && mbar_wait_bounded(&full[s], ph, P.error, k);
+          tc_fence_after();
+          const uint64_t ad = umma_desc(smem_u32(ring + (size_t)s * P.stage_bytes));
+          const uint64_t bd = umma_desc(smem_u32(ring + (size_t)s * P.stage_bytes + kWBytes));
+          if (lead && ok) {
+#pragma unroll
+            for (int kk = 0; kk < kBlockK / 16; ++kk)
+              umma_f16(dcol, ad + (uint64_t)(2 * kk), bd + (uint64_t)(2 * kk), idesc, ((kb - kb0) | kk) != 0 ? 1u : 0u);
+            umma_commit(&empty[s]);
+          }
+          if (++s == P.ring_stages) { s = 0; ph ^= 1u; }
+        }
+        if (lead) umma_commit(&tfull[it]);
+        ++uses[it];
+      }
+    }
+    __syncwarp();
+  } else {
+    const int ctid = threadIdx.x - 64, group = ctid >> 7, gtid = ctid & 127;
+    const int row = (warp & 3) * 32 + lane;
+    float* aq = reinterpret_cast<float*>(attn + (size_t)group * P.attn_bytes);
+    float* apo = aq + G * 128;
+    float* apm = apo + 4 * G * 128;
+    float* apl = apm + 4 * G;
+    uint32_t uses[2] = {0u, 0u};
+    for (int k = 0; k < P.n_phases; ++k) {
+      const CpPhase& F = P.phases[k];
+      if (F.kind == CP_GEMM) {
+        if (group == 0) {
+          const SkParams& p = F.p;
+          int it = 0;
+          for (int i = blockIdx.x; i < F.items; i += grid, ++it) {
+            const bool got = mbar_wait_bounded(&tfull[it], uses[it] & 1u, P.error, k);
+            ++uses[it];
+            tc_fence_after();
+            float* dst = P.part + (size_t)i * m_pad * kRowsW + row;
+            const uint32_t taddr = tmem_base + ((uint32_t)((warp & 3) * 32) << 16) + (uint32_t)(it * m_pad);
+            for (int c0 = 0; c0 < p.M; c0 += 32) {
+              uint32_t raw[32];
+              tmem_ld32(taddr + (uint32_t)c0, raw);
+              if (got) {
+#pragma unroll
+                for (int jj = 0; jj < 32; ++jj)
+                  if (c0 + jj < p.M) __stcg(dst + (size_t)(c0 + jj) * kRowsW, __uint_as_float(raw[jj]));
+              }
+            }
+            tc_fence_before();
+            mbar_arrive(&tempty[it]);
+          }
+          group_bar(1);
+          if (ctid == 0) {
+            __threadfence();
+            for (int i = blockIdx.x; i < F.items; i += grid) atomicAdd(&P.sync[P.n_phases + k * P.max_tiles + (i >> p.split_shift)], 1u);
+          }
+          for (int i = blockIdx.x; i < F.items; i += grid) {
+            if (ctid == 0) {
+              bool ok = k == 0 || wait_count(&P.sync[k - 1], (unsigned)grid, P.error, k);
+              ok = ok && wait_count(&P.sync[P.n_phases + k * P.max_tiles + (i >> p.split_shift)], (unsigned)p.split, P.error, k);
+              *flag = ok ? 1 : 0;
+            }
+            group_bar(1);
+            const bool ok = *flag != 0;
+            if (ok && p.rms_x) sk_row_factors(p, rowscale_s, (uint32_t)(i & (p.split - 1)));
+            group_bar(1);
+            if (ok) {
+              if (p.swiglu) reduce_rows<true>(P, p, i, rowscale_s, row);
+              else reduce_rows<false>(P, p, i, rowscale_s, row);
+            }
+            group_bar(1);
+          }
+        }
+      } else {
+        if (ctid == 0) *flag = wait_count(&P.sync[k - 1], (unsigned)grid, P.error, k) ? 1 : 0;
+        consumer_bar();
+        if (*flag) {
+          const int step = grid * kCpAttnGroups;
+          for (int i = group * grid + blockIdx.x; i < F.items; i += step) {
+            const int r = i / P.kv_heads, kvh = i - r * P.kv_heads;
+            rope_attention_item<G, __half, float>(r, kvh, gtid, aq, apo, apm, apl, [group] { group_bar(1 + group); }, F.qkv, F.ld, P.heads,
+                                                  P.kv_heads, F.q_norm, F.k_norm, P.eps, P.inv_freq, P.row_slot, P.row_pos, nullptr, F.kv,
+                                                  F.out, F.ldo, P.attn_scale);
+          }
+        }
+      }
+      asm volatile("fence.proxy.async.global;" ::: "memory");
+      consumer_bar();
+      if (ctid == 0) {
+        __threadfence();
+        atomicAdd(&P.sync[k], 1u);
+      }
+    }
+  }
+  tc_fence_before();
+  __syncthreads();
+  if (warp == 1) {
+    tc_fence_after();
+    asm volatile("tcgen05.dealloc.cta_group::1.sync.aligned.b32 %0, %1;" ::"r"(tmem_base), "r"(256) : "memory");
+  }
+  const int n_sync = P.n_phases * (1 + P.max_tiles);
+  if (threadIdx.x == 0) {
+    __threadfence();
+    *last = atomicAdd(&P.sync[n_sync], 1u) == (unsigned)grid - 1u ? 1 : 0;
+  }
+  __syncthreads();
+  if (*last) {
+    for (int i = threadIdx.x; i <= n_sync; i += blockDim.x) P.sync[i] = 0u;
+  }
+}
+
+using CpKernel = void (*)(const CpPassParams);
+CpKernel pick(int G) {
+  if (G == 1) return cp_pass_kernel<1>;
+  if (G == 2) return cp_pass_kernel<2>;
+  return cp_pass_kernel<4>;
+}
+
+}
+
+size_t cp_pass_smem(int G, int m_pad, int* stages, int* stage_bytes, int* attn_bytes) {
+  *stage_bytes = kWBytes + m_pad * kBlockK * 2;
+  *attn_bytes = ((G * 128 + 4 * G * 128 + 8 * G) * 4 + 127) / 128 * 128;
+  const int budget = 200 * 1024 - kCpAttnGroups * *attn_bytes;
+  *stages = std::min(8, budget / *stage_bytes);
+  return 1024 + (size_t)*stages * *stage_bytes + (size_t)kCpAttnGroups * *attn_bytes + (2 * *stages + 4) * 8 + 16 + 128 * 4;
+}
+
+int cp_pass_max_blocks_per_sm(int G, size_t smem) {
+  const CpKernel k = pick(G);
+  Q3_CUDA(cudaFuncSetAttribute(k, cudaFuncAttributeMaxDynamicSharedMemorySize, (int)smem));
+  int n = 0;
+  Q3_CUDA(cudaOccupancyMaxActiveBlocksPerMultiprocessor(&n, k, kCpPassThreads, smem));
+  return n;
+}
+
+void launch_cp_pass(const LaunchCtx& c, const CpPassPlan& plan, int g) {
+  CpPassParams p = plan.p;
+  p.phases = plan.d_phases + (size_t)g * p.n_phases;
+  p.row_pos = plan.p.row_pos + (size_t)g * plan.p.row_pos_stride;
+  void* args[] = {&p};
+  Q3_CUDA(cudaLaunchCooperativeKernel(reinterpret_cast<const void*>(pick(plan.G)), dim3(plan.grid), dim3(kCpPassThreads), args, plan.smem, c.stream));
+  c.tick();
+}
+
+}
diff --git a/mlx-swift-qwen3-tts_b200/csrc/engine.h b/mlx-swift-qwen3-tts_b200/csrc/engine.h
--- a/mlx-swift-qwen3-tts_b200/csrc/engine.h
+++ b/mlx-swift-qwen3-tts_b200/csrc/engine.h
@@ -5,6 +5,7 @@
 #include <string>
 #include <vector>
 
+#include "cp_pass.h"
 #include "frame_kernel.h"
 #include "kernels.h"
 
@@ -85,6 +86,8 @@
                      const float* inv_freq, void* kbase, void* vbase, int kv_f16, size_t slot_stride, size_t layer_stride, int capacity,
                      bool one_row_per_slot, bool decode_step, bool x16_ready);
   void issue_frame(int n_slots);
+  const CpPassPlan& cp_pass_plan(int n_slots);
+  void check_cp_pass();
   void build_tc_weights();
   void build_mega_plan();
   TcLinear make_tc(const Linear& L, bool interleave_halves, const float* fold = nullptr);
@@ -147,6 +150,10 @@
   };
   std::map<long long, Graph> graphs_;
   MegaPlan mega_;
+  bool cp_pass_enabled_ = false;
+  std::map<int, CpPassPlan> cp_plans_;
+  int* d_cp_err_ = nullptr;
+  std::vector<std::string> cp_phase_names_;
 };
 
 struct Handle {
diff --git a/mlx-swift-qwen3-tts_b200/csrc/gemm_skinny.cu b/mlx-swift-qwen3-tts_b200/csrc/gemm_skinny.cu
--- a/mlx-swift-qwen3-tts_b200/csrc/gemm_skinny.cu
+++ b/mlx-swift-qwen3-tts_b200/csrc/gemm_skinny.cu
@@ -189,8 +189,7 @@
   *tiles = s.tiles; *split = s.split; *stages = s.stages;
 }
 
-void launch_tc_skinny(const LaunchCtx& c, const TcGemm& g) {
-  if (tc_skinny_q_supported(g)) return launch_tc_skinny_q(c, g);
+skinny::SkParams skinny::tc_skinny_params(const TcGemm& g, CUtensorMap* mw, CUtensorMap* mx) {
   Q3_CHECK(tc_skinny_supported(g), Q3TTS_ERR_INVALID_ARG, "tc_skinny: unsupported shape (rows %d, cin %d, N %d)", g.Bt * g.T, g.cin, g.N);
   tc_resolve_encode();
   const SkPlan s = plan(g);
@@ -213,11 +212,19 @@
   const uint64_t wdims[2] = {(uint64_t)g.cin, (uint64_t)g.N};
   const uint64_t wstr[1] = {(uint64_t)g.cin * 2};
   const uint32_t wbox[2] = {(uint32_t)kBlockK, (uint32_t)kRowsW};
-  const CUtensorMap mw = tc_make_map(g.w, 2, wdims, wstr, wbox);
+  *mw = tc_make_map(g.w, 2, wdims, wstr, wbox);
   const uint64_t xdims[2] = {(uint64_t)g.cin, (uint64_t)p.M};
   const uint64_t xstr[1] = {(uint64_t)g.cin * 2};
   const uint32_t xbox[2] = {(uint32_t)kBlockK, (uint32_t)s.m_pad};
-  const CUtensorMap mx = tc_make_map(g.a, 2, xdims, xstr, xbox);
+  *mx = tc_make_map(g.a, 2, xdims, xstr, xbox);
+  return p;
+}
+
+void launch_tc_skinny(const LaunchCtx& c, const TcGemm& g) {
+  if (tc_skinny_q_supported(g)) return launch_tc_skinny_q(c, g);
+  CUtensorMap mw, mx;
+  const SkParams p = skinny::tc_skinny_params(g, &mw, &mx);
+  const SkPlan s = plan(g);
 
   Q3_CHECK(s.smem <= 220 * 1024, Q3TTS_ERR_CAPACITY, "tc_skinny: shared memory request %zu too large", s.smem);
   cudaLaunchConfig_t cfg{};
diff --git a/mlx-swift-qwen3-tts_b200/csrc/rope_attention.cuh b/mlx-swift-qwen3-tts_b200/csrc/rope_attention.cuh
--- /dev/null
+++ b/mlx-swift-qwen3-tts_b200/csrc/rope_attention.cuh
@@ -0,0 +1,155 @@
+#pragma once
+#include <cuda_fp16.h>
+
+#include "device_utils.cuh"
+#include "kernels.h"
+
+namespace q3 {
+
+__device__ __forceinline__ float4 kv_ld4(const float* p) { return *reinterpret_cast<const float4*>(p); }
+__device__ __forceinline__ float4 kv_ld4(const __half* p) {
+  const uint2 u = *reinterpret_cast<const uint2*>(p);
+  const float2 a = __half22float2(*reinterpret_cast<const __half2*>(&u.x)), b = __half22float2(*reinterpret_cast<const __half2*>(&u.y));
+  return make_float4(a.x, a.y, b.x, b.y);
+}
+__device__ __forceinline__ float kv_ld(const float* p) { return *p; }
+__device__ __forceinline__ float kv_ld(const __half* p) { return __half2float(*p); }
+__device__ __forceinline__ void kv_st(float* p, float v) { *p = v; }
+__device__ __forceinline__ void kv_st(__half* p, float v) { *p = __float2half_rn(v); }
+__device__ __forceinline__ void store_act(float* p, float v) { *p = v; }
+__device__ __forceinline__ void store_act(__half* p, float v) { *p = __float2half_rn(v); }
+
+template <int G, typename OutT, typename KvT, typename Sync>
+__device__ __forceinline__ void rope_attention_item(int row, int kvh, int tid, float* q, float* part_o, float* part_m, float* part_l, Sync sync,
+                                                    const float* __restrict__ qkv, int ld, int heads, int kv_heads,
+                                                    const float* __restrict__ q_norm, const float* __restrict__ k_norm, float eps,
+                                                    const float* __restrict__ inv_freq, const int* __restrict__ row_slot,
+                                                    const int* __restrict__ row_pos, const int* __restrict__ win_start, const KVLayout& kv,
+                                                    OutT* __restrict__ out, int ldo, float scale) {
+  const int lane = tid & 31, warp = tid >> 5;
+  const int slot = row_slot[row], pos = row_pos[row];
+  const int w0 = win_start ? win_start[slot] : 0;
+  const int S = pos - w0 + 1;
+  const int cap = kv.capacity;
+  const int r0 = w0 % cap;
+  const int ring = (r0 + S - 1 >= cap) ? r0 + S - 1 - cap : r0 + S - 1;
+  KvT* kb = static_cast<KvT*>(kv.k) + (size_t)slot * kv.slot_stride + (size_t)kvh * cap * 128;
+  KvT* vb = static_cast<KvT*>(kv.v) + (size_t)slot * kv.slot_stride + (size_t)kvh * cap * 128;
+  const float* rowp = qkv + (size_t)row * ld;
+  for (int hh = warp; hh <= G; hh += 4) {
+    const float* src = rowp + (size_t)(hh < G ? (kvh * G + hh) : (heads + kvh)) * 128;
+    const float a0 = src[lane], a1 = src[lane + 32], b0 = src[lane + 64], b1 = src[lane + 96];
+    const float ss = warp_sum(a0 * a0 + a1 * a1 + b0 * b0 + b1 * b1);
+    const float inv = rsqrtf(ss * (1.0f / 128.0f) + eps);
+    const float* nw = hh < G ? q_norm : k_norm;
+    const float x0 = a0 * inv * nw[lane], x1 = a1 * inv * nw[lane + 32], y0 = b0 * inv * nw[lane + 64], y1 = b1 * inv * nw[lane + 96];
+    float s0, c0, s1, c1;
+    sincosf((float)pos * inv_freq[lane], &s0, &c0);
+    sincosf((float)pos * inv_freq[lane + 32], &s1, &c1);
+    const float o0 = x0 * c0 - y0 * s0, o1 = x1 * c1 - y1 * s1, o2 = y0 * c0 + x0 * s0, o3 = y1 * c1 + x1 * s1;
+    if (hh < G) {
+      float* dst = q + hh * 128;
+      dst[lane] = o0; dst[lane + 32] = o1; dst[lane + 64] = o2; dst[lane + 96] = o3;
+    } else {
+      KvT* dst = kb + (size_t)ring * 128;
+      kv_st(dst + lane, o0); kv_st(dst + lane + 32, o1); kv_st(dst + lane + 64, o2); kv_st(dst + lane + 96, o3);
+    }
+  }
+  kv_st(vb + (size_t)ring * 128 + tid, rowp[(size_t)(heads + kv_heads + kvh) * 128 + tid]);
+  sync();
+  const int seg = lane & 7, grp = warp * 4 + (lane >> 3);
+  float qf[G][16];
+#pragma unroll
+  for (int g = 0; g < G; ++g)
+#pragma unroll
+    for (int i = 0; i < 4; ++i) {
+      const float4 t = *reinterpret_cast<const float4*>(q + g * 128 + i * 32 + seg * 4);
+      qf[g][4 * i] = t.x * scale; qf[g][4 * i + 1] = t.y * scale; qf[g][4 * i + 2] = t.z * scale; qf[g][4 * i + 3] = t.w * scale;
+    }
+  float mx[G], l[G], o[G][16];
+#pragma unroll
+  for (int g = 0; g < G; ++g) {
+    mx[g] = -INFINITY; l[g] = 0.f;
+#pragma unroll
+    for (int d = 0; d < 16; ++d) o[g][d] = 0.f;
+  }
+  for (int jb = 0; jb < S; jb += 32) {
+    const int j0 = jb + grp;
+    float4 kk[2][4], vv[2][4];
+#pragma unroll
+    for (int u = 0; u < 2; ++u) {
+      const int j = j0 + 16 * u;
+      const int rj = r0 + (j < S ? j : 0);
+      const size_t base = (size_t)(rj >= cap ? rj - cap : rj) * 128 + seg * 4;
+#pragma unroll
+      for (int i = 0; i < 4; ++i) {
+        kk[u][i] = kv_ld4(kb + base + i * 32);
+        vv[u][i] = kv_ld4(vb + base + i * 32);
+      }
+    }
+#pragma unroll
+    for (int u = 0; u < 2; ++u) {
+      const bool valid = j0 + 16 * u < S;
+#pragma unroll
+      for (int g = 0; g < G; ++g) {
+        float sdot = 0.f;
+#pragma unroll
+        for (int i = 0; i < 4; ++i)
+          sdot += kk[u][i].x * qf[g][4 * i] + kk[u][i].y * qf[g][4 * i + 1] + kk[u][i].z * qf[g][4 * i + 2] + kk[u][i].w * qf[g][4 * i + 3];
+        sdot += __shfl_xor_sync(0xffffffffu, sdot, 1);
+        sdot += __shfl_xor_sync(0xffffffffu, sdot, 2);
+        sdot += __shfl_xor_sync(0xffffffffu, sdot, 4);
+        if (!valid) sdot = -INFINITY;
+        const float mn = fmaxf(mx[g], sdot);
+        const bool none = mn == -INFINITY;
+        const float corr = none ? 1.f : expf(mx[g] - mn), pr = none ? 0.f : expf(sdot - mn);
+        mx[g] = mn;
+        l[g] = l[g] * corr + pr;
+#pragma unroll
+        for (int i = 0; i < 4; ++i) {
+          o[g][4 * i] = o[g][4 * i] * corr + pr * vv[u][i].x;
+          o[g][4 * i + 1] = o[g][4 * i + 1] * corr + pr * vv[u][i].y;
+          o[g][4 * i + 2] = o[g][4 * i + 2] * corr + pr * vv[u][i].z;
+          o[g][4 * i + 3] = o[g][4 * i + 3] * corr + pr * vv[u][i].w;
+        }
+      }
+    }
+  }
+#pragma unroll
+  for (int g = 0; g < G; ++g) {
+    float m_all = fmaxf(mx[g], __shfl_xor_sync(0xffffffffu, mx[g], 8));
+    m_all = fmaxf(m_all, __shfl_xor_sync(0xffffffffu, m_all, 16));
+    const float f = (mx[g] == -INFINITY) ? 0.f : expf(mx[g] - m_all);
+    float lw = l[g] * f;
+    lw += __shfl_xor_sync(0xffffffffu, lw, 8);
+    lw += __shfl_xor_sync(0xffffffffu, lw, 16);
+#pragma unroll
+    for (int d = 0; d < 16; ++d) {
+      float t = o[g][d] * f;
+      t += __shfl_xor_sync(0xffffffffu, t, 8);
+      t += __shfl_xor_sync(0xffffffffu, t, 16);
+      o[g][d] = t;
+    }
+    if (lane < 8) {
+#pragma unroll
+      for (int i = 0; i < 4; ++i)
+        *reinterpret_cast<float4*>(&part_o[(warp * G + g) * 128 + i * 32 + seg * 4]) = make_float4(o[g][4 * i], o[g][4 * i + 1], o[g][4 * i + 2], o[g][4 * i + 3]);
+      if (lane == 0) { part_m[warp * G + g] = m_all; part_l[warp * G + g] = lw; }
+    }
+  }
+  sync();
+#pragma unroll
+  for (int g = 0; g < G; ++g) {
+    float m_all = fmaxf(fmaxf(part_m[g], part_m[G + g]), fmaxf(part_m[2 * G + g], part_m[3 * G + g]));
+    float num = 0.f, den = 0.f;
+#pragma unroll
+    for (int w = 0; w < 4; ++w) {
+      const float f = (part_m[w * G + g] == -INFINITY) ? 0.f : expf(part_m[w * G + g] - m_all);
+      num += part_o[(w * G + g) * 128 + tid] * f;
+      den += part_l[w * G + g] * f;
+    }
+    store_act(out + (size_t)row * ldo + (size_t)(kvh * G + g) * 128 + tid, num / den);
+  }
+}
+
+}
diff --git a/mlx-swift-qwen3-tts_b200/csrc/skinny_common.cuh b/mlx-swift-qwen3-tts_b200/csrc/skinny_common.cuh
--- a/mlx-swift-qwen3-tts_b200/csrc/skinny_common.cuh
+++ b/mlx-swift-qwen3-tts_b200/csrc/skinny_common.cuh
@@ -48,6 +48,8 @@
   int split_shift;
 };
 
+SkParams tc_skinny_params(const TcGemm& g, CUtensorMap* mw, CUtensorMap* mx);
+
 __device__ __forceinline__ unsigned long long sk_globaltimer() {
   unsigned long long t;
   asm volatile("mov.u64 %0, %%globaltimer;" : "=l"(t));
diff --git a/mlx-swift-qwen3-tts_b200/csrc/talker_engine.cu b/mlx-swift-qwen3-tts_b200/csrc/talker_engine.cu
--- a/mlx-swift-qwen3-tts_b200/csrc/talker_engine.cu
+++ b/mlx-swift-qwen3-tts_b200/csrc/talker_engine.cu
@@ -140,6 +140,125 @@
   launch_linear(c, w_.fc2, d_tph_, cfg_.text_hidden_size, 3, d_tts_, H, nullptr, 0.f, EPI_STORE);
   Q3_CUDA(cudaStreamSynchronize(stream_));
   build_mega_plan();
+  cp_pass_enabled_ = handle_tc_ && !w_.cp.tc.empty() && opt_.use_cuda_graph && opt_.lanes <= 1 && owns_weights_;
+  if (cp_pass_enabled_) {
+    d_cp_err_ = arena_.alloc_n<int>(1);
+    Q3_CUDA(cudaMemsetAsync(d_cp_err_, 0, sizeof(int), stream_));
+    Q3_CUDA(cudaStreamSynchronize(stream_));
+  }
+}
+
+const CpPassPlan& TalkerEngine::cp_pass_plan(int m) {
+  auto found = cp_plans_.find(m);
+  if (found != cp_plans_.end()) return found->second;
+  CpPassPlan& pl = cp_plans_[m];
+  const StackWeights& S = w_.cp;
+  if (!cp_pass_enabled_ || m < 3 || m > 128 || S.head_dim != 128 || S.heads % S.kv_heads) return pl;
+  const int G = S.heads / S.kv_heads;
+  if (G != 1 && G != 2 && G != 4) return pl;
+  const int Hcp = cfg_.cp.hidden_size, Vc = cfg_.cp.vocab_size, B = opt_.max_batch;
+  const int qkv_ld = (S.heads + 2 * S.kv_heads) * 128, attn_ld = S.heads * 128;
+  float* x = w_.has_mtp ? d_cpx_ : d_cpin_;
+  const float inv16 = 1.0f / kX16Div;
+  auto consumer = [&](const TcLinear& L, float* out32, int ld32, void* out16, int ld16, int swiglu) {
+    TcGemm g;
+    g.a = (const __half*)d_h16_; g.w = (const __half*)L.w; g.Bt = 1; g.T = m; g.cin = L.in; g.N = L.out;
+    g.bias = L.bias; g.swiglu = swiglu; g.out32 = out32; g.ld32 = ld32; g.out16 = (__half*)out16; g.ld16 = ld16;
+    g.rms_eps = S.eps; g.in_scale = inv16; g.rms_in = 1;
+    return g;
+  };
+  auto producer = [&](const TcLinear& L, const void* a16) {
+    TcGemm g;
+    g.a = (const __half*)a16; g.w = (const __half*)L.w; g.Bt = 1; g.T = m; g.cin = L.in; g.N = L.out;
+    g.bias = L.bias; g.res = x; g.ld_res = S.hidden; g.out32 = x; g.ld32 = S.hidden;
+    g.out16 = (__half*)d_h16_; g.ld16 = S.hidden; g.out16_scale = inv16;
+    return g;
+  };
+  std::vector<CpPhase> ph;
+  std::vector<std::string> names;
+  int max_tiles = 0, max_items = 0, m_pad = 0;
+  auto gemm = [&](const TcGemm& g, const std::string& name) {
+    if (!tc_skinny_supported(g) || g.act != TC_ACT_NONE) return false;
+    CpPhase f{};
+    f.kind = CP_GEMM;
+    f.p = skinny::tc_skinny_params(g, &f.tmW, &f.tmX);
+    f.p.trace = nullptr;
+    const int tiles = (f.p.N + skinny::kRowsW - 1) / skinny::kRowsW;
+    f.items = tiles * f.p.split;
+    max_tiles = std::max(max_tiles, tiles);
+    max_items = std::max(max_items, f.items);
+    m_pad = f.p.m_pad;
+    ph.push_back(f);
+    names.push_back(name);
+    return true;
+  };
+  std::vector<CpPhase> passes;
+  for (int gi = 0; gi < 15; ++gi) {
+    ph.clear();
+    names.clear();
+    for (int l = 0; l < S.layers; ++l) {
+      const LayerWeights& L = S.layer[l];
+      const LayerTc& Tc = S.tc[l];
+      const std::string lay = "layer " + std::to_string(l) + " ";
+      if (!gemm(consumer(Tc.qkv, d_qkv_, qkv_ld, nullptr, 0, 0), lay + "qkv")) return pl;
+      CpPhase a{};
+      a.kind = CP_ATTN;
+      a.items = m * S.kv_heads;
+      a.qkv = d_qkv_; a.ld = qkv_ld; a.q_norm = L.q_norm; a.k_norm = L.k_norm;
+      a.kv.k = cp_k_ + (size_t)l * cpkv_layer_stride_; a.kv.v = cp_v_ + (size_t)l * cpkv_layer_stride_;
+      a.kv.slot_stride = cpkv_slot_stride_; a.kv.capacity = kCpCapacity; a.kv.f16 = 0;
+      a.out = (__half*)d_attn16_; a.ldo = attn_ld;
+      ph.push_back(a);
+      names.push_back(lay + "attention");
+      if (!gemm(producer(Tc.o, d_attn16_), lay + "o")) return pl;
+      if (!gemm(consumer(Tc.gate_up_il, nullptr, 0, d_act16_, S.inter, 1), lay + "gate_up")) return pl;
+      if (!gemm(producer(Tc.down, d_act16_), lay + "down")) return pl;
+    }
+    TcGemm hg = consumer(w_.lm_head_tc[gi], d_cplogits_, Vc, nullptr, 0, 0);
+    hg.cin = Hcp; hg.N = Vc; hg.rms_eps = w_.cp.eps;
+    if (!gemm(hg, "lm_head")) return pl;
+    passes.insert(passes.end(), ph.begin(), ph.end());
+  }
+  const int n_phases = (int)ph.size();
+  int stages = 0, stage_bytes = 0, attn_bytes = 0;
+  const size_t smem = cp_pass_smem(G, m_pad, &stages, &stage_bytes, &attn_bytes);
+  int dev = 0, sms = 0, coop = 0;
+  Q3_CUDA(cudaGetDevice(&dev));
+  Q3_CUDA(cudaDeviceGetAttribute(&sms, cudaDevAttrMultiProcessorCount, dev));
+  Q3_CUDA(cudaDeviceGetAttribute(&coop, cudaDevAttrCooperativeLaunch, dev));
+  if (!coop || stages < 2 || cp_pass_max_blocks_per_sm(G, smem) < 1) return pl;
+  if (max_items > 2 * sms) return pl;
+  CpPassParams& p = pl.p;
+  p.n_phases = n_phases; p.max_tiles = max_tiles;
+  p.heads = S.heads; p.kv_heads = S.kv_heads; p.eps = S.eps; p.attn_scale = 1.0f / sqrtf(128.0f);
+  p.inv_freq = d_cp_inv_freq_; p.row_slot = d_iota_; p.row_pos = d_cp_pos_; p.row_pos_stride = B;
+  const size_t n_sync = (size_t)n_phases * (1 + max_tiles) + 1;
+  p.sync = arena_.alloc_n<unsigned>(n_sync);
+  Q3_CUDA(cudaMemsetAsync(p.sync, 0, n_sync * sizeof(unsigned), stream_));
+  p.error = d_cp_err_;
+  p.part = arena_.alloc_n<float>((size_t)max_items * m_pad * skinny::kRowsW);
+  p.ring_stages = stages; p.stage_bytes = stage_bytes; p.attn_bytes = attn_bytes;
+  pl.d_phases = arena_.alloc_n<CpPhase>(passes.size());
+  Q3_CUDA(cudaMemcpyAsync(pl.d_phases, passes.data(), sizeof(CpPhase) * passes.size(), cudaMemcpyHostToDevice, stream_));
+  Q3_CUDA(cudaStreamSynchronize(stream_));
+  pl.grid = sms; pl.G = G; pl.smem = smem;
+  cp_phase_names_ = names;
+  pl.ok = true;
+  return pl;
+}
+
+void TalkerEngine::check_cp_pass() {
+  if (!d_cp_err_) return;
+  int e = 0;
+  Q3_CUDA(cudaMemcpyAsync(&e, d_cp_err_, sizeof(int), cudaMemcpyDeviceToHost, stream_));
+  Q3_CUDA(cudaStreamSynchronize(stream_));
+  if (e == 0) return;
+  const std::string what = e - 1 < (int)cp_phase_names_.size() ? cp_phase_names_[e - 1] : "phase " + std::to_string(e - 1);
+  Q3_CUDA(cudaMemsetAsync(d_cp_err_, 0, sizeof(int), stream_));
+  for (auto& kv : cp_plans_)
+    if (kv.second.ok) Q3_CUDA(cudaMemsetAsync(kv.second.p.sync, 0, sizeof(unsigned) * ((size_t)kv.second.p.n_phases * (1 + kv.second.p.max_tiles) + 1), stream_));
+  Q3_CUDA(cudaStreamSynchronize(stream_));
+  fail(Q3TTS_ERR_CUDA, "code-predictor pass kernel: a wait in phase '%s' timed out", what.c_str());
 }
 
 void TalkerEngine::build_mega_plan() {
@@ -694,6 +813,7 @@
     return ni;
   };
   launch_sample(c, d_logits0_, V, n_slots, d_state_, p, d_sets_, d_cur_codes_, d_forced_, F, dump0, V, 0, dump_slot_, next_input(1));
+  const CpPassPlan* cpp = step_tc_ && n_slots >= 3 && n_slots <= 128 ? &cp_pass_plan(n_slots) : nullptr;
   for (int g = 0; g < 15; ++g) {
     const int m = g == 0 ? 2 * n_slots : n_slots;
     float* x = d_cpin_;
@@ -705,9 +825,15 @@
       }
       x = d_cpx_;
     }
+    if (step_tc_ && g != 0 && cpp && cpp->ok) {
+      if (!x16_direct) launch_scale_to_f16(c, x, (size_t)m * Hcp, 1.0f / kX16Div, (__half*)d_h16_);
+      launch_cp_pass(c, *cpp, g);
+    } else {
     forward_stack(w_.cp, x, m, g == 0 ? d_cp_slot2_ : d_iota_, g == 0 ? d_cp_pos2_ : d_cp_pos_ + (size_t)g * B, nullptr,
                   d_cp_inv_freq_, cp_k_, cp_v_, 0, cpkv_slot_stride_, cpkv_layer_stride_, kCpCapacity, g != 0, true, x16_direct);
-    if (step_tc_ && g != 0 && n_slots <= 128) {
+    }
+    if (step_tc_ && g != 0 && cpp && cpp->ok) {
+    } else if (step_tc_ && g != 0 && n_slots <= 128) {
       TcGemm hg;
       hg.a = (const __half*)d_h16_; hg.w = (const __half*)w_.lm_head_tc[g].w; hg.Bt = 1; hg.T = n_slots; hg.cin = Hcp; hg.N = Vc;
       hg.bias = w_.lm_head_tc[g].bias; hg.out32 = d_cplogits_; hg.ld32 = Vc;
@@ -763,6 +889,7 @@
   const long long key = (long long)n_slots * 8192 + (dump_enabled_ ? 1 + dump_slot_ : 0);
   auto it = graphs_.find(key);
   if (it == graphs_.end()) {
+    if (use_tc_step(n_slots) && n_slots >= 3 && n_slots <= 128) cp_pass_plan(n_slots);
     cudaGraph_t g = nullptr;
     if (counter_) { counter_->capturing = true; counter_->captured = 0; }
     Q3_CUDA(cudaStreamBeginCapture(stream_, cudaStreamCaptureModeThreadLocal));
@@ -792,6 +919,7 @@
 }
 
 void TalkerEngine::fetch_states(int n_slots, std::vector<SlotState>& out) {
+  check_cp_pass();
   Q3_CUDA(cudaMemcpyAsync(h_state_, d_state_, sizeof(SlotState) * n_slots, cudaMemcpyDeviceToHost, stream_));
   Q3_CUDA(cudaStreamSynchronize(stream_));
   out.assign(h_state_, h_state_ + n_slots);
diff --git a/mlx-swift-qwen3-tts_b200/csrc/talker_kernels.cu b/mlx-swift-qwen3-tts_b200/csrc/talker_kernels.cu
--- a/mlx-swift-qwen3-tts_b200/csrc/talker_kernels.cu
+++ b/mlx-swift-qwen3-tts_b200/csrc/talker_kernels.cu
@@ -3,6 +3,7 @@
 
 #include "kernels.h"
 #include "device_utils.cuh"
+#include "rope_attention.cuh"
 #include "sampler.cuh"
 
 namespace q3 {
@@ -360,16 +361,6 @@
   c.tick();
 }
 
-__device__ __forceinline__ float4 kv_ld4(const float* p) { return *reinterpret_cast<const float4*>(p); }
-__device__ __forceinline__ float4 kv_ld4(const __half* p) {
-  const uint2 u = *reinterpret_cast<const uint2*>(p);
-  const float2 a = __half22float2(*reinterpret_cast<const __half2*>(&u.x)), b = __half22float2(*reinterpret_cast<const __half2*>(&u.y));
-  return make_float4(a.x, a.y, b.x, b.y);
-}
-__device__ __forceinline__ float kv_ld(const float* p) { return *p; }
-__device__ __forceinline__ float kv_ld(const __half* p) { return __half2float(*p); }
-__device__ __forceinline__ void kv_st(float* p, float v) { *p = v; }
-__device__ __forceinline__ void kv_st(__half* p, float v) { *p = __float2half_rn(v); }
 template <typename KvT>
 __global__ void __launch_bounds__(128) qk_norm_rope_append_kernel(float* __restrict__ qkv, int ld, int m, int heads, int kv_heads,
                                                                   const float* __restrict__ q_norm, const float* __restrict__ k_norm,
@@ -422,8 +413,6 @@
   c.tick();
 }
 
-__device__ __forceinline__ void store_act(float* p, float v) { *p = v; }
-__device__ __forceinline__ void store_act(__half* p, float v) { *p = __float2half_rn(v); }
 
 template <int G, typename OutT, typename KvT>
 __global__ void __launch_bounds__(128) attention_kernel(const float* __restrict__ qkv, int ld, int heads, int kv_heads,
@@ -493,134 +482,12 @@
                                                              const int* __restrict__ row_pos, const int* __restrict__ win_start, KVLayout kv,
                                                              OutT* __restrict__ out, int ldo, float scale) {
   __shared__ __align__(16) float q[G * 128];
-  __shared__ __align__(16) float part_o[4][G][128];
-  __shared__ float part_m[4][G], part_l[4][G];
+  __shared__ __align__(16) float part_o[4 * G * 128];
+  __shared__ float part_m[4 * G], part_l[4 * G];
   pdl_launch_dependents();
   pdl_wait();
-  const int row = blockIdx.x, kvh = blockIdx.y, tid = threadIdx.x, lane = tid & 31, warp = tid >> 5;
-  const int slot = row_slot[row], pos = row_pos[row];
-  const int w0 = win_start ? win_start[slot] : 0;
-  const int S = pos - w0 + 1;
-  const int cap = kv.capacity;
-  const int r0 = w0 % cap;
-  const int ring = (r0 + S - 1 >= cap) ? r0 + S - 1 - cap : r0 + S - 1;
-  KvT* kb = static_cast<KvT*>(kv.k) + (size_t)slot * kv.slot_stride + (size_t)kvh * cap * 128;
-  KvT* vb = static_cast<KvT*>(kv.v) + (size_t)slot * kv.slot_stride + (size_t)kvh * cap * 128;
-  const float* rowp = qkv + (size_t)row * ld;
-  for (int hh = warp; hh <= G; hh += 4) {
-    const float* src = rowp + (size_t)(hh < G ? (kvh * G + hh) : (heads + kvh)) * 128;
-    const float a0 = src[lane], a1 = src[lane + 32], b0 = src[lane + 64], b1 = src[lane + 96];
-    const float ss = warp_sum(a0 * a0 + a1 * a1 + b0 * b0 + b1 * b1);
-    const float inv = rsqrtf(ss * (1.0f / 128.0f) + eps);
-    const float* nw = hh < G ? q_norm : k_norm;
-    const float x0 = a0 * inv * nw[lane], x1 = a1 * inv * nw[lane + 32], y0 = b0 * inv * nw[lane + 64], y1 = b1 * inv * nw[lane + 96];
-    float s0, c0, s1, c1;
-    sincosf((float)pos * inv_freq[lane], &s0, &c0);
-    sincosf((float)pos * inv_freq[lane + 32], &s1, &c1);
-    const float o0 = x0 * c0 - y0 * s0, o1 = x1 * c1 - y1 * s1, o2 = y0 * c0 + x0 * s0, o3 = y1 * c1 + x1 * s1;
-    if (hh < G) {
-      float* dst = q + hh * 128;
-      dst[lane] = o0; dst[lane + 32] = o1; dst[lane + 64] = o2; dst[lane + 96] = o3;
-    } else {
-      KvT* dst = kb + (size_t)ring * 128;
-      kv_st(dst + lane, o0); kv_st(dst + lane + 32, o1); kv_st(dst + lane + 64, o2); kv_st(dst + lane + 96, o3);
-    }
-  }
-  kv_st(vb + (size_t)ring * 128 + tid, rowp[(size_t)(heads + kv_heads + kvh) * 128 + tid]);
-  __syncthreads();
-  const int seg = lane & 7, grp = warp * 4 + (lane >> 3);
-  float qf[G][16];
-#pragma unroll
-  for (int g = 0; g < G; ++g)
-#pragma unroll
-    for (int i = 0; i < 4; ++i) {
-      const float4 t = *reinterpret_cast<const float4*>(q + g * 128 + i * 32 + seg * 4);
-      qf[g][4 * i] = t.x * scale; qf[g][4 * i + 1] = t.y * scale; qf[g][4 * i + 2] = t.z * scale; qf[g][4 * i + 3] = t.w * scale;
-    }
-  float mx[G], l[G], o[G][16];
-#pragma unroll
-  for (int g = 0; g < G; ++g) {
-    mx[g] = -INFINITY; l[g] = 0.f;
-#pragma unroll
-    for (int d = 0; d < 16; ++d) o[g][d] = 0.f;
-  }
-  for (int jb = 0; jb < S; jb += 32) {
-    const int j0 = jb + grp;
-    float4 kk[2][4], vv[2][4];
-#pragma unroll
-    for (int u = 0; u < 2; ++u) {
-      const int j = j0 + 16 * u;
-      const int rj = r0 + (j < S ? j : 0);
-      const size_t base = (size_t)(rj >= cap ? rj - cap : rj) * 128 + seg * 4;
-#pragma unroll
-      for (int i = 0; i < 4; ++i) {
-        kk[u][i] = kv_ld4(kb + base + i * 32);
-        vv[u][i] = kv_ld4(vb + base + i * 32);
-      }
-    }
-#pragma unroll
-    for (int u = 0; u < 2; ++u) {
-      const bool valid = j0 + 16 * u < S;
-#pragma unroll
-      for (int g = 0; g < G; ++g) {
-        float sdot = 0.f;
-#pragma unroll
-        for (int i = 0; i < 4; ++i)
-          sdot += kk[u][i].x * qf[g][4 * i] + kk[u][i].y * qf[g][4 * i + 1] + kk[u][i].z * qf[g][4 * i + 2] + kk[u][i].w * qf[g][4 * i + 3];
-        sdot += __shfl_xor_sync(0xffffffffu, sdot, 1);
-        sdot += __shfl_xor_sync(0xffffffffu, sdot, 2);
-        sdot += __shfl_xor_sync(0xffffffffu, sdot, 4);
-        if (!valid) sdot = -INFINITY;
-        const float mn = fmaxf(mx[g], sdot);
-        const bool none = mn == -INFINITY;
-        const float corr = none ? 1.f : expf(mx[g] - mn), pr = none ? 0.f : expf(sdot - mn);
-        mx[g] = mn;
-        l[g] = l[g] * corr + pr;
-#pragma unroll
-        for (int i = 0; i < 4; ++i) {
-          o[g][4 * i] = o[g][4 * i] * corr + pr * vv[u][i].x;
-          o[g][4 * i + 1] = o[g][4 * i + 1] * corr + pr * vv[u][i].y;
-          o[g][4 * i + 2] = o[g][4 * i + 2] * corr + pr * vv[u][i].z;
-          o[g][4 * i + 3] = o[g][4 * i + 3] * corr + pr * vv[u][i].w;
-        }
-      }
-    }
-  }
-#pragma unroll
-  for (int g = 0; g < G; ++g) {
-    float m_all = fmaxf(mx[g], __shfl_xor_sync(0xffffffffu, mx[g], 8));
-    m_all = fmaxf(m_all, __shfl_xor_sync(0xffffffffu, m_all, 16));
-    const float f = (mx[g] == -INFINITY) ? 0.f : expf(mx[g] - m_all);
-    float lw = l[g] * f;
-    lw += __shfl_xor_sync(0xffffffffu, lw, 8);
-    lw += __shfl_xor_sync(0xffffffffu, lw, 16);
-#pragma unroll
-    for (int d = 0; d < 16; ++d) {
-      float t = o[g][d] * f;
-      t += __shfl_xor_sync(0xffffffffu, t, 8);
-      t += __shfl_xor_sync(0xffffffffu, t, 16);
-      o[g][d] = t;
-    }
-    if (lane < 8) {
-#pragma unroll
-      for (int i = 0; i < 4; ++i)
-        *reinterpret_cast<float4*>(&part_o[warp][g][i * 32 + seg * 4]) = make_float4(o[g][4 * i], o[g][4 * i + 1], o[g][4 * i + 2], o[g][4 * i + 3]);
-      if (lane == 0) { part_m[warp][g] = m_all; part_l[warp][g] = lw; }
-    }
-  }
-  __syncthreads();
-#pragma unroll
-  for (int g = 0; g < G; ++g) {
-    float m_all = fmaxf(fmaxf(part_m[0][g], part_m[1][g]), fmaxf(part_m[2][g], part_m[3][g]));
-    float num = 0.f, den = 0.f;
-#pragma unroll
-    for (int w = 0; w < 4; ++w) {
-      const float f = (part_m[w][g] == -INFINITY) ? 0.f : expf(part_m[w][g] - m_all);
-      num += part_o[w][g][tid] * f;
-      den += part_l[w][g] * f;
-    }
-    store_act(out + (size_t)row * ldo + (size_t)(kvh * G + g) * 128 + tid, num / den);
-  }
+  rope_attention_item<G, OutT, KvT>(blockIdx.x, blockIdx.y, threadIdx.x, q, part_o, part_m, part_l, [] { __syncthreads(); }, qkv, ld, heads, kv_heads,
+                                    q_norm, k_norm, eps, inv_freq, row_slot, row_pos, win_start, kv, out, ldo, scale);
 }
 template <int G>
 __global__ void __launch_bounds__(128) cp_pass0_attention_kernel(const float* __restrict__ qkv, int ld, int heads, int kv_heads,
```

Result: slower. 503.0 (median of 6 runs) (-55.2%).
